# gbordelon/fast_ray_tracer

Measured on AMD Instinct MI355X. Metric: Mrays/s (primary+shadow+secondary) + wall-clock/frame, 1/2/4/8 GPU, higher is better.
Workload: dtype f64

## Files before the change

fast_ray_tracer_amd/csrc/frt_engine.hip:

```cpp
#include <hip/hip_runtime.h>
#include <hipcub/hipcub.hpp>

#include <algorithm>
#include <array>
#include <atomic>
#include <condition_variable>
#include <memory>
#include <mutex>
#include <cmath>
#include <cstdio>
#include <cstdlib>
#include <cstring>
#include <string>
#include <chrono>
#include <functional>
#include <thread>
#include <vector>

#include "frt_device.h"
#include "frt_jit.h"
#include "frt_shade.hpp"
#include "frt_shade32.hpp"
#include "frt_shadow.hpp"
#include "frt_jit_rt.hpp"
// ... 411 lines not shown
            }
        }
    }
    nr.flags = flags;
    PSTAMP(3);
    const bool own = kPat && (M.map_Ka >= 0 || M.map_Kd >= 0 || M.map_Ks >= 0 || M.map_refl >= 0 || M.map_Ns >= 0);
    rec.store(node, nr, own, kPat && M.map_d >= 0);
#pragma unroll
    for (int k = 0; k < 3; ++k) rec.head.op[k * rec.head.cap + node] = c.over_point[k];
    if (rec.head.key != nullptr) rec.head.key[node] = key;
    PSTAMP(4);
    for (int k = 0; k < 3; ++k) op[k] = c.over_point[k];
    };
    if (uniform_ok) {
        const int leaf_u = uniform(hr.node);
        if (__ballot(hr.node != leaf_u) == 0ull) {
            if (B.stats) wave_count(line + 18, (int)(threadIdx.x & 63) == __builtin_ctzll(__ballot(true)));
            prepare_hit(uniform_view(S), leaf_u);
            return true;
        }
    }
    prepare_hit(S, hr.node);
    return true;
}

__device__ __forceinline__ void tile_box(int64_t node, int64_t n, bool hit, const double* op, float* __restrict__ tbox,
                                         int tile_log2, float* __restrict__ stbox, int sub_log2) {
    float lo[3], hi[3];
#pragma unroll
    for (int a = 0; a < 3; ++a) {
        lo[a] = hit ? __double2float_rd(op[a]) : __builtin_huge_valf();
        hi[a] = hit ? __double2float_ru(op[a]) : -__builtin_huge_valf();
    }
    for (int off = 1; off < (1 << tile_log2); off <<= 1) {
        if (stbox != nullptr && off == (1 << sub_log2) && node < n && (node & (off - 1)) == 0) {
            float* b = stbox + 6 * (node >> sub_log2);
#pragma unroll
            for (int a = 0; a < 3; ++a) {
                b[a] = lo[a];
                b[a + 3] = hi[a];
            }
        }
#pragma unroll
        for (int a = 0; a < 3; ++a) {
            lo[a] = fminf(lo[a], __shfl_xor(lo[a], off, 64));
            hi[a] = fmaxf(hi[a], __shfl_xor(hi[a], off, 64));
        }
    }
    if (node < n && (node & ((1 << tile_log2) - 1)) == 0) {
        float* b = tbox + 6 * (node >> tile_log2);
#pragma unroll
        for (int a = 0; a < 3; ++a) {
            b[a] = lo[a];
            b[a + 3] = hi[a];
        }
    }
}

template <bool kPat>
__global__ void __launch_bounds__(kBlock) __attribute__((amdgpu_waves_per_eu(kPat ? 1 : FRT_PREPARE_WAVES, 8)))
k_prepare(DevScene S, Batch B, const QueuedRay* __restrict__ q, int64_t n, const HitRec* __restrict__ hits,
          const double* __restrict__ hn12,
          NodeCols rec, QueuedRay* __restrict__ next_q, unsigned long long* counters,
          unsigned* err, float* __restrict__ tbox, int tile_log2, float* __restrict__ stbox, int sub_log2,
          int32_t* __restrict__ counts, unsigned long long* __restrict__ spawn_masks, int uniform_ok) {
    const int64_t node = (int64_t)blockIdx.x * blockDim.x + threadIdx.x;
    double op[3] = {0.0, 0.0, 0.0};
    bool hit = false;
    if (node < n && counts != nullptr)
        for (int l = 0; l < S.num_lights; ++l) counts[node * S.num_lights + l] = 0;
    int spawned = 0;
    if (node < n)
        hit = prepare_node<kPat>(S, B, q, n, hits, hn12, rec, next_q, counters, err, node, op,
                                 spawn_masks != nullptr ? &spawned : nullptr, uniform_ok);
    if (spawn_masks != nullptr) {
        const unsigned long long mr = __ballot(spawned & 1), mt = __ballot((spawned >> 1) & 1);
        const int64_t g = node >> 6, G = (n + 63) >> 6;
        if ((threadIdx.x & 63) == 0 && g < G) {
            spawn_masks[g] = mr;
            spawn_masks[G + g] = mt;
        }
    }
    if (tbox != nullptr) tile_box(node, n, hit, op, tbox, tile_log2, stbox, sub_log2);
}

#ifdef FRT_SHADOW_WAVES
#define FRT_SHADOW_ATTR __attribute__((amdgpu_waves_per_eu(FRT_SHADOW_WAVES, 8)))
#else
#define FRT_SHADOW_ATTR
#endif
template <int kFeat>
__global__ void __launch_bounds__(kTraceBlock) FRT_SHADOW_ATTR k_shadow(DevScene S, Batch B, const HeadCols shead, int64_t n,
                                                        const int32_t* __restrict__ j_light,
                                                        const int32_t* __restrict__ j_point, int32_t samples_per_node,
                                                        int32_t* __restrict__ counts, unsigned* err) {
    ShadowLane L;
    shadow_lane(S, B, shead, n, j_light, j_point, samples_per_node, (int64_t)blockIdx.x * blockDim.x + threadIdx.x, L);
    unsigned e = 0;
    double unused;
    const bool lit = walk<true, kFeat>(S, L.r, L.distance, L.live, unused, frt_walk_smem, e) == 0 && L.live;
    if (e) atomicOr(err, e);
    shadow_count(S, L, lit, counts);
}

template <int kFeat>
__global__ void __launch_bounds__(kTraceBlock) k_shadow_redo(DevScene S, Batch B, const HeadCols shead, int64_t n,
                                                             const int32_t* __restrict__ j_light,
                                                             const int32_t* __restrict__ j_point, int32_t samples_per_node,
                                                             int32_t* __restrict__ counts, unsigned* err,
                                                             const int64_t* __restrict__ redo,
                                                             const unsigned* __restrict__ redo_count, unsigned redo_cap) {
    const unsigned cnt = min(*redo_count, redo_cap);
    const int64_t wave = ((int64_t)blockIdx.x * blockDim.x + threadIdx.x) >> 6;
    const int64_t nwaves = ((int64_t)gridDim.x * blockDim.x) >> 6;
    unsigned e = 0;
    for (int64_t base = wave * 64; base < (int64_t)cnt; base += nwaves * 64) {
        const int64_t k = base + (threadIdx.x & 63);
        ShadowLane L;
        shadow_lane(S, B, shead, n, j_light, j_point, samples_per_node, k < (int64_t)cnt ? redo[k] : -1, L);
        double unused;
        const bool lit = walk<true, kFeat>(S, L.r, L.distance, L.live, unused, frt_walk_smem, e) == 0 && L.live;
        if (lit) atomicAdd(counts + L.node * S.num_lights + L.light, 1);
    }
    if (e) atomicOr(err, e);
}

#ifndef FRT_SHADE_FACTOR
#define FRT_SHADE_FACTOR 1
#endif
__device__ __forceinline__ double dot3_shade(const double* a, const double* b) {
    return __builtin_fma(a[0], b[0], __builtin_fma(a[1], b[1], a[2] * b[2]));
}
__device__ __forceinline__ void camera_eyev(const DevScene& S, const Batch& B, int64_t i, double* eyev) {
    Ray r;
    uint64_t key;
    unsigned ce = 0;
    camera_ray(S, B, i, r, key, ce);
    for (int k = 0; k < 3; ++k) eyev[k] = r.d[k] * -1.0;
}

__global__ void __launch_bounds__(kBlock) k_view_rays(DevScene S, Batch B, const frt_camera* __restrict__ cams,
                                                      int32_t nviews, int64_t view_pixels, int64_t n,
                                                      QueuedRay* __restrict__ q, unsigned* err) {
    const int64_t i = (int64_t)blockIdx.x * blockDim.x + threadIdx.x;
    if (i >= n) return;
    const int64_t pix = B.pixel_begin + i / B.spp;
    const int view = (int)min((int64_t)(nviews - 1), pix / view_pixels);
    Batch Bv = B;
    Bv.pixel_begin = pix - (int64_t)view * view_pixels - i / B.spp;
    Bv.cam_fast = 0;
    unsigned e = 0;
    auto emit = [&](const frt_camera& cam) {
        DevScene Sv = S;
        Sv.cam = cam;
        Sv.cam_origin_set = 0;
        QueuedRay qr;
        Ray r;
        camera_ray(Sv, Bv, i, r, qr.key, e);
        for (int k = 0; k < 3; ++k) {
            qr.o[k] = r.o[k];
            qr.d[k] = r.d[k];
        }
        qr.parent = -1;
        qr.slot = 0;
        q[i] = qr;
    };
// ... 1364 lines not shown
    if (fgather != nullptr)
        for (int k = 0; k < 3; ++k) a[k] += fgather[3 * i + k];
    for (int k = 0; k < 3; ++k) a[k] += gi_extra[6 * i + 3 + k];
    const double len = a[0] + a[1] + a[2];
    if (len > 1.7320508075688772) {
        for (int k = 0; k < 3; ++k) a[k] *= 1.0 / len;
        for (int k = 0; k < 3; ++k) a[k] *= 1.7320508075688772;
    }
    tri_store(surface, i, a);
}

}


constexpr size_t kJitStatWords = 16384;

template <typename T>
struct PinnedBuf {
    T* p = nullptr;
    size_t n = 0;
    PinnedBuf() = default;
    PinnedBuf(const PinnedBuf&) = delete;
    PinnedBuf& operator=(const PinnedBuf&) = delete;
    ~PinnedBuf() {
        if (p) (void)hipHostFree(p);
    }
    bool resize(size_t m) {
        if (m > n) {
            if (p) (void)hipHostFree(p);
            p = nullptr;
            n = 0;
            if (hipHostMalloc((void**)&p, m * sizeof(T), hipHostMallocDefault) != hipSuccess) {
                p = nullptr;
                return false;
            }
            n = m;
        }
        std::memset(p, 0, n * sizeof(T));
        return true;
    }
    T* data() { return p; }
    const T* data() const { return p; }
    size_t size() const { return n; }
    T& operator[](size_t i) { return p[i]; }
    const T& operator[](size_t i) const { return p[i]; }
};

struct frt_scene_handle {
    int device = 0;
    UploadKnobs up;
    FrameKnobs fk;
    frt::DevScene S{};
    std::vector<void*> owned;
    std::vector<double> host_table;
    hipStream_t stream = nullptr;
    int32_t* j_light = nullptr;
    int32_t* j_point = nullptr;
    int32_t samples_per_node = 0;
    size_t lds_bytes = 0;
    void* jit_shadow = nullptr;
    void* jit_beam = nullptr;
    void* jit_tile = nullptr;
    void* jit_list = nullptr;
    int tile = 0;
    uint64_t scene_key = 0;
    void* jit_sub = nullptr;
    int sub = 0;
    int sub_ps = 0;
    const int32_t* light_psamp2 = nullptr;
    const float* light_sbox = nullptr;
    uint32_t* slist = nullptr;
    int64_t slist_cap = 0;
    uint64_t sub_pairs = 0, sub_mixed = 0;
    void* jit_subtile = nullptr;
    void* jit_trace = nullptr;
    int32_t* tredo = nullptr;
    int64_t tredo_cap = 0;
    int subtile = 0;
    float* stbox = nullptr;
    int64_t stbox_cap = 0;
    uint32_t* s2list = nullptr;
    int64_t s2list_cap = 0;
    uint64_t subtile_pairs = 0, subtile_mixed = 0;
    float* tbox = nullptr;
    int64_t tbox_cap = 0;
    uint32_t* tlist = nullptr;
    int64_t tlist_cap = 0;
    uint64_t tile_pairs = 0, tile_mixed = 0, node_pairs = 0, node_mixed = 0;
    bool jit_beam_on = true;
    const int32_t* light_psamp = nullptr;
    const float* light_aabb = nullptr;
    uint32_t* mixed = nullptr;
    int64_t mixed_cap = 0;
    unsigned* mcount = nullptr;
    uint64_t sync_epoch = 0;
    PinnedBuf<unsigned> host_mcount;
    PinnedBuf<unsigned long long> host_counters;
    PinnedBuf<unsigned> host_lcount;
    int64_t* redo = nullptr;
    unsigned* redo_count = nullptr;
    unsigned redo_cap = 0;
    frt_frame_stats* cur_st = nullptr;
    uint64_t rays_walked = 0;
    uint64_t pairs_walked = 0;
    uint64_t heads_walked = 0;
    unsigned long long uniform_stats[3] = {0, 0, 0};
    uint32_t* shade_lit = nullptr;
    int64_t shade_lit_cap = 0;
    int sort_light = -1;
    int shade_stage = 0;
    uint32_t* lit_row = nullptr;
    int64_t lit_row_cap = 0;
    uint32_t* lit_flat = nullptr;
    int64_t lit_flat_cap = 0;
    frt::LitStage* lit_stage = nullptr;
    int64_t lit_stage_cap = 0;
    bool fast32 = false;
    frt::Light32 light32{nullptr, nullptr};
    uint32_t* qsort = nullptr;
    int64_t qsort_cap = 0;
    unsigned long long* spawn_masks = nullptr;
    int64_t spawn_masks_cap = 0;
    uint32_t* spawn_offs = nullptr;
    int64_t spawn_offs_cap = 0;
    unsigned char* scan_tmp = nullptr;
    int64_t scan_tmp_cap = 0;
    unsigned* shade_lcount = nullptr;
    int64_t shade_lcount_cap = 0;
    unsigned long long* jit_stats = nullptr;
    struct Level {
        frt::NodeCols rec;
        double* head_op = nullptr;
        uint64_t* head_key = nullptr;
        frt::QueuedRay* q = nullptr;
        frt::Cols<frt::Tri9> surface;
        frt::Cols<frt::Tri9> child;
        int64_t* qprefix = nullptr;
        std::vector<int64_t> hprefix = std::vector<int64_t>(frt::kQueueSegs + 1, 0);
        int32_t* counts = nullptr;
        uint32_t* spos = nullptr;
        bool staged = false;
        uint32_t* qperm = nullptr;
        int64_t qperm_cap = 0;
        bool sorted = false;
        int64_t cap = 0;
    };
    std::vector<Level> levels;
    frt::HitRec* hits = nullptr;
    int64_t hits_cap = 0;
    double* hn12 = nullptr;
    int64_t hn12_cap = 0;
    frt::Cols<frt::Tri9> sample_col;
    int64_t sample_cap = 0;
    double* out_dev = nullptr;
    int64_t out_cap = 0;
    double* feat_geom = nullptr;
    int64_t feat_geom_cap = 0;
    int32_t* feat_ids = nullptr;
    int64_t feat_ids_cap = 0;
    frt_camera* view_cams = nullptr;
    int64_t view_cams_cap = 0;
    int32_t strip_views = 0;
    bool cam_origin_ok = false;
    frt::QueuedRay* view_q = nullptr;
    int64_t view_q_cap = 0;
    unsigned long long* counters = nullptr;
// ... 743 lines not shown
    const int kind = (int)(i & 7), pick = (int)((i >> 3) % 7);
    frt::Point64 Q;
    if (kind < 2)
        across(l, eps_list[pick], Q.n);
    else
        unit(Q.n);
    if (kind == 2) {
        across(Q.n, eps_list[pick % 5], Q.e);
    } else {
        unit(Q.e);
        if (kind < 6 && frt::dot3(Q.n, Q.e) < 0.0)
            for (int k = 0; k < 3; ++k) Q.e[k] = -Q.e[k];
    }
    const double ns_list[7] = {0.0, 1.0, 2.5, 10.0, 200.0, 1000.0, 5000.0};
    Q.ns = ns_list[i % 7];
    Q.cdist = (Q.ns + 2) * 0.5 * frt::k1Pi;
    Q.ned = frt::dot3(Q.n, Q.e);
    Q.ee = frt::dot3(Q.e, Q.e);
    for (int k = 0; k < 3; ++k) Q.base[k] = c[k] - o[k];
    const frt::Point32 P = frt::point32_of(Q, __builtin_huge_valf(), true, true);
    frt::ShadeSums s32 = {0.0, 0.0, 0.0}, s64 = {0.0, 0.0, 0.0};
    frt::point_term32(P, Q, off, s32);
    frt::Point64 R = Q;
    for (int k = 0; k < 3; ++k) R.base[k] = lp[k] - o[k];
    const double zero[3] = {0.0, 0.0, 0.0};
    frt::point_term64(R, zero, true, true, s64);
    const bool fin64 = __builtin_isfinite(s64.ldn) && __builtin_isfinite(s64.b) && __builtin_isfinite(s64.fb);
    const bool fin32 = __builtin_isfinite(s32.ldn) && __builtin_isfinite(s32.b) && __builtin_isfinite(s32.fb);
    unsigned long long bad = 0;
    if (fin64 && !fin32) bad++;
    const double dl = fabs(s32.ldn - s64.ldn);
    if (fin64 && fin32 && !(dl <= 32.0 * 0x1p-24)) bad++;
    if (bad) atomicAdd(res, bad);
    auto put_max = [&](int slot, double v) {
        const unsigned long long b = (unsigned long long)__double_as_longlong(v);
        if (b > res[slot]) atomicMax(res + slot, b);
    };
    if (fin64 && fin32) {
        put_max(3, dl);
        if (s64.ldn >= 0x1p-16 && s64.b >= 0x1p-100) {
            const double rel = fabs(s32.b - s64.b) / s64.b;
            put_max(1, rel);
            if (Q.ns <= 200.0) put_max(2, rel);
            atomicAdd(res + 4, 1ull);
        }
    }
}

int64_t frt_shade32_selftest(int64_t n, uint64_t seed, double* out, int nout) {
    n = (std::max<int64_t>(n, 64) + 63) / 64 * 64;
    unsigned long long* res = nullptr;
    unsigned long long h[5] = {0, 0, 0, 0, 0};
    if (hipMalloc((void**)&res, sizeof(h)) != hipSuccess) return -1;
    bool ok = hipMemset(res, 0, sizeof(h)) == hipSuccess;
    if (ok) {
        hipLaunchKernelGGL(k_shade32_selftest, dim3((unsigned)((n + 255) / 256)), dim3(256), 0, 0, n, seed, res);
        ok = hipGetLastError() == hipSuccess && hipMemcpy(h, res, sizeof(h), hipMemcpyDeviceToHost) == hipSuccess;
    }
    hip_ignore(hipFree(res));
    if (!ok) return -1;
    for (int k = 0; k < nout && k < 4 && out != nullptr; ++k) {
        double v;
        std::memcpy(&v, &h[k + 1], sizeof(v));
        out[k] = k == 3 ? (double)h[4] : v;
    }
    return (int64_t)h[0];
}

size_t frt_frame_params_size(void) { return sizeof(frt_frame_params); }

const char* frt_last_error(void) { return g_last_error.c_str(); }

static std::atomic<long long> g_maps_stat[2];

static thread_local double t_upload_phases[8];

int frt_photon_pass_stats(int64_t* out, int n) {
    for (int i = 0; i < n && i < 2; ++i) out[i] = g_maps_stat[i].load();
    return 2;
}

size_t frt_frame_stats_size(void) { return sizeof(frt_frame_stats); }

static std::mutex g_warm_mu;
static hipStream_t g_warm_stream[64] = {};

void* frt_host_pinned_alloc(size_t bytes) {
    void* p = nullptr;
    if (bytes == 0 || hipHostMalloc(&p, bytes, hipHostMallocDefault) != hipSuccess) {
        (void)hipGetLastError();
        return nullptr;
    }
    return p;
}

void frt_host_pinned_free(void* p) {
    if (p) hip_ignore(hipHostFree(p));
}

int frt_device_warmup(int device) {
    const WarmupKnobs K = read_warmup_knobs();
    const bool trace = K.trace;
    auto t0 = std::chrono::steady_clock::now();
    auto mark = [&](const char* what) {
        if (!trace) return;
        const auto t1 = std::chrono::steady_clock::now();
        std::fprintf(stderr, "frt warmup: %s %.2f ms\n", what, std::chrono::duration<double, std::milli>(t1 - t0).count());
        t0 = t1;
    };
    if (hipSetDevice(device) != hipSuccess) {
        (void)hipGetLastError();
        return -1;
    }
    mark("hipSetDevice");
    hip_ignore(hipFree(nullptr));
    mark("context");
    void* p = nullptr;
    if (hipMalloc(&p, 1 << 20) == hipSuccess) {
        mark("hipMalloc");
        hipStream_t s = nullptr;
        if (K.mode == 1 || hipStreamCreate(&s) == hipSuccess) {
            mark("stream");
            unsigned host[64] = {0};
            hip_ignore(hipMemcpyAsync(p, host, sizeof(host), hipMemcpyHostToDevice, s));
            hip_ignore(hipStreamSynchronize(s));
            mark("H2D copy");
            hipLaunchKernelGGL(k_warm, dim3(1), dim3(64), 0, s, (unsigned*)p);
            hip_ignore(hipStreamSynchronize(s));
            mark("first kernel (code object load)");
            hip_ignore(hipMemcpyAsync(host, p, sizeof(host), hipMemcpyDeviceToHost, s));
            hip_ignore(hipStreamSynchronize(s));
            mark("D2H copy");
            if (s) {
                std::lock_guard<std::mutex> lk(g_warm_mu);
                if (device >= 0 && device < 64 && g_warm_stream[device] == nullptr) g_warm_stream[device] = s;
                else hip_ignore(hipStreamDestroy(s));
            }
        }
        hip_ignore(hipFree(p));
    }
    (void)hipGetLastError();
    return 0;
}

int frt_upload_phases(double* out, int n) {
    for (int i = 0; i < n && i < 8; ++i) out[i] = t_upload_phases[i];
    return 8;
}

int frt_scene_upload(const frt_scene* sc, int device, frt_scene_handle** out) {
    const auto up0 = std::chrono::steady_clock::now();
    auto up_last = up0;
    auto phase = [&](int i) {
        const auto t = std::chrono::steady_clock::now();
        t_upload_phases[i] += std::chrono::duration<double, std::milli>(t - up_last).count();
        up_last = t;
    };
    for (double& x : t_upload_phases) x = 0.0;
    if (sc == nullptr || out == nullptr) return fail("frt_scene_upload: null argument");
    if (sc->abi_version != FRT_ABI_VERSION) return fail("frt_scene_upload: ABI version mismatch");
    int ndev = frt_device_count();
    if (ndev <= 0) return fail("frt_scene_upload: no HIP device visible");
    if (device < 0 || device >= ndev) return fail("frt_scene_upload: device index out of range");
    FRT_HIP(hipSetDevice(device));
    frt_scene_handle* h = new frt_scene_handle();
    h->device = device;
// ... 21 lines not shown
        mix(sc->roots, sizeof(int32_t) * (size_t)sc->num_roots);
        mix(sc->xforms, sizeof(double) * 16 * (size_t)sc->num_xforms);
        mix(sc->prim_data, sizeof(double) * (size_t)sc->prim_len);
        mix(sc->materials, sizeof(frt_material) * (size_t)sc->num_materials);
        mix(sc->patterns, sizeof(frt_pattern) * (size_t)sc->num_patterns);
        mix(sc->textures, sizeof(frt_texture) * (size_t)sc->num_textures);
        mix(sc->texels, sizeof(double) * (size_t)sc->texel_len);
        mix(sc->lights, sizeof(frt_light) * (size_t)sc->num_lights);
        mix(sc->light_points, sizeof(double) * (size_t)sc->light_point_len);
        mix(&sc->config, sizeof(frt_config));
        h->scene_key = k;
    }
    phase(0);
    S.nodes = upload(h, sc->nodes, (size_t)sc->num_nodes, rc);
    S.roots = upload(h, sc->roots, (size_t)sc->num_roots, rc);
    S.xforms = upload(h, sc->xforms, (size_t)sc->num_xforms * 16, rc);
    S.prim = upload(h, sc->prim_data, (size_t)sc->prim_len, rc);
    S.materials = upload(h, sc->materials, (size_t)sc->num_materials, rc);
    S.patterns = upload(h, sc->patterns, (size_t)sc->num_patterns, rc);
    S.textures = upload(h, sc->textures, (size_t)sc->num_textures, rc);
    S.texels = upload(h, sc->texels, (size_t)sc->texel_len, rc);
    S.lights = upload(h, sc->lights, (size_t)sc->num_lights, rc);
    S.light_points = upload(h, sc->light_points, (size_t)sc->light_point_len, rc);
    S.sample_table = upload(h, sc->sample_table, (size_t)(2 * sc->camera.usteps * sc->camera.vsteps), rc);
    if (S.sample_table != nullptr)
        h->host_table.assign(sc->sample_table, sc->sample_table + 2 * sc->camera.usteps * sc->camera.vsteps);
    {
        std::vector<uint8_t> casts((size_t)std::max(1, sc->num_nodes), 0);
        for (int i = 0; i < sc->num_nodes; ++i) {
            const int m = sc->nodes[i].material;
            casts[(size_t)i] = (m >= 0 && m < sc->num_materials && sc->materials[m].casts_shadow) ? 1 : 0;
        }
        S.casts = upload(h, casts.data(), casts.size(), rc);
        std::vector<int4> xchain((size_t)std::max(1, sc->num_nodes), make_int4(0, 0, 0, 0));
        for (int i = 0; i < sc->num_nodes; ++i) {
            int ids[64], n = 0;
            for (int x = sc->nodes[i].xform >= 0 ? i : sc->nodes[i].tparent; x >= 0 && n < 64; x = sc->nodes[x].tparent)
                ids[n++] = sc->nodes[x].xform;
            if (n <= 3) xchain[(size_t)i] = make_int4(n, n > 0 ? ids[n - 1] : 0, n > 1 ? ids[n - 2] : 0, n > 2 ? ids[n - 3] : 0);
            else xchain[(size_t)i] = make_int4(-1, 0, 0, 0);
        }
        S.xchain = upload(h, xchain.data(), xchain.size(), rc);
    }
    if (rc) {
        frt_scene_release(h);
        return -1;
    }
    phase(1);
    {
        std::vector<frt::WalkNode> wn;
        build_walk_nodes(sc, wn);
        if (rc == 0 && build_meshes(h, sc, wn)) {
            frt_scene_release(h);
            return -1;
        }
        S.wn = upload(h, wn.data(), wn.size(), rc);
        if (rc == 0 && sc->config.include_direct && K.jit) {
            std::string why, log;
            phase(2);
            const std::string src = frt_jit_shadow_source(wn.data(), sc->num_nodes, sc->roots, sc->num_roots, sc->lights, sc->num_lights, K, why);
            phase(3);
            FrtJitFns fns;
            if (!src.empty() && frt_jit_compile(src, h->device, K, fns, log) != 0) {
                why = "hiprtc: " + log.substr(0, 2000);
                fns = FrtJitFns{};
            }
            if (!src.empty()) {
                double ob = 0.0, ld = 0.0;
                frt_jit_last_phases(&ob, &ld);
                t_upload_phases[4] += ob;
                t_upload_phases[5] += ld;
                up_last = std::chrono::steady_clock::now();
            }
            h->jit_shadow = fns.shadow;
            h->jit_beam = fns.beam;
            h->jit_tile = fns.tile;
            h->jit_list = fns.list;
            h->tile = fns.tile && fns.list ? K.jit_tile : 0;
            h->jit_sub = fns.sub;
            h->sub = fns.sub ? K.jit_sub : 0;
            h->jit_subtile = fns.subtile;
            h->jit_trace = sc->config.all_ni_one ? fns.trace : nullptr;
            h->subtile = fns.subtile ? K.jit_subtile : 0;
            if (h->jit_shadow) {
                h->redo_cap = 1u << 20;
                void* p = nullptr;
                if (hipMalloc(&p, h->redo_cap * sizeof(int64_t) + 64) != hipSuccess) {
                    frt_scene_release(h);
                    return fail("frt_scene_upload: redo queue allocation failed");
                }
                h->owned.push_back(p);
                h->redo = (int64_t*)p;
                h->redo_count = (unsigned*)(h->redo + h->redo_cap);
                h->jit_beam_on = K.jit_beam;
                std::vector<float> box;
                std::vector<int32_t> psamp;
                const int PS = K.jit_part;
                auto push_box = [](std::vector<float>& v, const double* pl, const double* ph) {
                    for (int a = 0; a < 3; ++a) {
                        float f = (float)pl[a];
                        if ((double)f > pl[a]) f = std::nextafter(f, -INFINITY);
                        v.push_back(f);
                    }
                    for (int a = 0; a < 3; ++a) {
                        float f = (float)ph[a];
                        if ((double)f < ph[a]) f = std::nextafter(f, INFINITY);
                        v.push_back(f);
                    }
                };
                auto sample_box = [&](const frt_light& lt, const int32_t* idx, int cnt, int r0, int r1, double* pl, double* ph) {
                    for (int a = 0; a < 3; ++a) {
                        pl[a] = INFINITY;
                        ph[a] = -INFINITY;
                    }
                    for (int r = r0; r < r1; ++r)
                        for (int k = 0; k < cnt; ++k) {
                            const int q = idx[k];
                            if (q < 0) continue;
                            const double* pt = sc->light_points + lt.points + 3 * ((int64_t)r * lt.num_samples + q);
                            for (int a = 0; a < 3; ++a) {
                                pl[a] = std::min(pl[a], pt[a]);
                                ph[a] = std::max(ph[a], pt[a]);
                            }
                        }
                };
                bool multi_row = false;
                std::vector<std::vector<int32_t>> orders((size_t)sc->num_lights);
                for (int l = 0; l < sc->num_lights; ++l) {
                    const frt_light& lt = sc->lights[l];
                    multi_row = multi_row || lt.rows > 1;
                    std::vector<int32_t>& order = orders[(size_t)l];
                    const int np = frt_jit_light_parts(lt, sc->light_points, PS, order);
                    psamp.insert(psamp.end(), order.begin(), order.end());
                    for (int r = 0; r < std::max(1, lt.rows); ++r)
                        for (int p = 0; p < np; ++p) {
                            double pl[3], ph[3];
                            sample_box(lt, order.data() + (size_t)p * PS, PS, r, r + 1, pl, ph);
                            push_box(box, pl, ph);
                        }
                }
                for (int l = 0; multi_row && l < sc->num_lights; ++l) {
                    const frt_light& lt = sc->lights[l];
                    const int np = (int)(orders[(size_t)l].size() / (size_t)PS);
                    for (int p = 0; p < np; ++p) {
                        double pl[3], ph[3];
                        sample_box(lt, orders[(size_t)l].data() + (size_t)p * PS, PS, 0, std::max(1, lt.rows), pl, ph);
                        push_box(box, pl, ph);
                    }
                }
                h->light_psamp = upload(h, psamp.data(), psamp.size(), rc);
                h->light_aabb = upload(h, box.data(), box.size(), rc);
                if (h->sub > 0) {
                    std::vector<int32_t> ps2;
                    std::vector<float> sbox;
                    const int Q = h->sub;
                    for (int l = 0; l < sc->num_lights; ++l) {
                        const frt_light& lt = sc->lights[l];
                        const int np = std::max(1, (lt.num_samples + PS - 1) / PS);
                        std::vector<int32_t> order2;
                        h->sub_ps = frt_jit_light_subparts(lt, sc->light_points, orders[(size_t)l], PS, Q, order2);
                        ps2.insert(ps2.end(), order2.begin(), order2.end());
                        for (int p = 0; p < np * Q; ++p) {
                            double pl[3], ph[3];
                            sample_box(lt, order2.data() + (size_t)p * h->sub_ps, h->sub_ps, 0, std::max(1, lt.rows), pl, ph);
                            push_box(sbox, pl, ph);
                        }
                    }
                    h->light_psamp2 = upload(h, ps2.data(), ps2.size(), rc);
                    h->light_sbox = upload(h, sbox.data(), sbox.size(), rc);
                }
                if (rc || hipMalloc((void**)&h->mcount, 4 * frt::jit::kMixSegs * frt::jit::kMixLine * sizeof(unsigned)) != hipSuccess) {
                    frt_scene_release(h);
                    return fail("frt_scene_upload: light box / pair list allocation failed");
                }
                h->owned.push_back(h->mcount);
                if (!h->host_mcount.resize((size_t)frt::jit::kMixSegs * frt::jit::kMixLine)) {
                    frt_scene_release(h);
                    return fail("frt_scene_upload: pinned host buffer allocation failed");
                }
                if (K.jit_stats) {
                    if (hipMalloc((void**)&h->jit_stats, kJitStatWords * sizeof(unsigned long long)) != hipSuccess) {
                        frt_scene_release(h);
                        return fail("frt_scene_upload: jit stats allocation failed");
                    }
                    h->owned.push_back(h->jit_stats);
                    hip_ignore(hipMemset(h->jit_stats, 0, kJitStatWords * sizeof(unsigned long long)));
                }
            } else if (K.jit_verbose) {
                std::fprintf(stderr, "frt: generic shadow walk (%s)\n", why.c_str());
            }
            if (K.jit_dump && !src.empty()) std::fprintf(stderr, "%s\n", src.c_str());
        }
    }
    {
        static const int kMaxHits[10] = {4, 2, 4, 1, 1, 2, 4, 1, 0, 0};
        const int nn = sc->num_nodes;
        std::vector<int> xf_cnt(nn, 0), comp_cnt(nn, 0), csg_top(nn, -1), list_need(nn, 0);
        int xf_depth = 0, comp_depth = 0, list_cap = 0, features = 0;
        for (int i = 0; i < nn; ++i) {
            const frt_node& nd = sc->nodes[i];
            const int par = nd.parent;
            const bool composite = nd.type == FRT_GROUP || nd.type == FRT_CSG;
            if (nd.type == FRT_CSG) features |= frt::kFeatCsg;
            if (nd.type == FRT_TOROID) features |= frt::kFeatTorus;
            csg_top[i] = par >= 0 && csg_top[par] >= 0 ? csg_top[par] : (nd.type == FRT_CSG ? i : -1);
            xf_cnt[i] = (par >= 0 ? xf_cnt[par] : 0) + (composite && nd.xform >= 0 ? 1 : 0);
            comp_cnt[i] = (par >= 0 && csg_top[par] >= 0 ? comp_cnt[par] : 0) + (composite && csg_top[i] >= 0 ? 1 : 0);
            xf_depth = std::max(xf_depth, xf_cnt[i]);
            comp_depth = std::max(comp_depth, comp_cnt[i]);
            if (!composite && csg_top[i] >= 0 && nd.type >= 0 && nd.type < 10) {
                list_need[csg_top[i]] += kMaxHits[nd.type];
                list_cap = std::max(list_cap, list_need[csg_top[i]]);
            }
        }
        S.list_cap = list_cap;
        S.comp_depth = comp_depth;
        S.xf_depth = xf_depth;
        S.features = features;
        h->lds_bytes = (size_t)frt::walk_lds_bytes(list_cap, comp_depth, xf_depth, S.mesh_stack);
        int lds_max = 64 * 1024;
        if (hipDeviceGetAttribute(&lds_max, hipDeviceAttributeMaxSharedMemoryPerBlock, device) != hipSuccess) {
            (void)hipGetLastError();
            lds_max = 64 * 1024;
        }
        if (h->lds_bytes > (size_t)lds_max) {
            frt_scene_release(h);
            return fail("frt_scene_upload: scene needs " + std::to_string(h->lds_bytes) +
                        " B of LDS per traversal block (CSG lists / nesting too large)");
        }
        if (h->lds_bytes > 64 * 1024) {
            const hipError_t e = walk_lds_opt_in(features, (int)h->lds_bytes);
            if (e != hipSuccess) {
                (void)hipGetLastError();
                frt_scene_release(h);
                return fail("frt_scene_upload: " + std::to_string(h->lds_bytes) +
                            " B of LDS per traversal block refused (" + hipGetErrorString(e) + ")");
            }
        }
    }
    S.walk_flags = K.walk_flags;
    S.num_nodes = sc->num_nodes;
    S.num_roots = sc->num_roots;
    S.num_lights = sc->num_lights;
    S.num_patterns = sc->num_patterns;
    set_scene_camera(h, sc->camera);
    S.cfg = sc->config;
    h->host_lights.assign(sc->lights, sc->lights + sc->num_lights);
    h->sort_light = -1;
    for (int l = 0; l < sc->num_lights && h->sort_light < 0 && K.shade_sort; ++l)
        if (sc->lights[l].rows > 1 && sc->lights[l].num_samples > 0) h->sort_light = l;
    h->shade_stage = h->sort_light >= 0 ? K.shade_stage : 0;
    if (S.cfg.path_length < 0 || S.cfg.path_length > frt::kMaxPathLength) {
        frt_scene_release(h);
        return fail("frt_scene_upload: path-length " + std::to_string(S.cfg.path_length) +
                    " is not supported (0.." + std::to_string(frt::kMaxPathLength) + ")");
    }
    if (S.cfg.use_gi && (S.cfg.gi_path_length >= 255 || S.cfg.photon_count <= 0)) {
        frt_scene_release(h);
        return fail("frt_scene_upload: global illumination needs photon maps (photon_count > 0) and path_length < 255");
    }

    std::vector<int32_t> jl, jp;
    for (int l = 0; l < sc->num_lights; ++l)
        for (int p = 0; p < sc->lights[l].num_samples; ++p) {
            jl.push_back(l);
            jp.push_back(p);
        }
    h->samples_per_node = (int32_t)jl.size();
    if (!jl.empty()) {
        h->j_light = (int32_t*)upload(h, jl.data(), jl.size(), rc);
        h->j_point = (int32_t*)upload(h, jp.data(), jp.size(), rc);
        if (rc) {
            frt_scene_release(h);
            return -1;
        }
    }
#if defined(FRT_WALK_STATS) || defined(FRT_WALK_PROF)
    if (hipMalloc((void**)&h->S.dbg, frt::kDbgSlots * sizeof(unsigned long long)) != hipSuccess ||
        hipMemset(h->S.dbg, 0, frt::kDbgSlots * sizeof(unsigned long long)) != hipSuccess) {
        frt_scene_release(h);
        return fail("frt_scene_upload: debug counters");
    }
#endif
    const auto ts0 = std::chrono::steady_clock::now();
    {
        std::lock_guard<std::mutex> lk(g_warm_mu);
        if (device >= 0 && device < 64 && g_warm_stream[device] != nullptr) {
            h->stream = g_warm_stream[device];
            g_warm_stream[device] = nullptr;
        }
    }
    const bool stream_ok = h->stream != nullptr || hipStreamCreate(&h->stream) == hipSuccess;
    if (K.warmup_trace)
        std::fprintf(stderr, "frt upload: hipStreamCreate %.2f ms\n",
                     std::chrono::duration<double, std::milli>(std::chrono::steady_clock::now() - ts0).count());
    if (!stream_ok || hipMalloc((void**)&h->counters, frt::kQueueSegs * frt::kCounterLine * sizeof(unsigned long long)) != hipSuccess ||
        hipMalloc((void**)&h->err, sizeof(unsigned)) != hipSuccess || hipEventCreate(&h->ev[0]) != hipSuccess ||
        hipEventCreate(&h->ev[1]) != hipSuccess) {
        frt_scene_release(h);
        return fail("frt_scene_upload: stream / counter allocation failed");
    }
    h->levels.resize((size_t)std::max(1, sc->config.path_length + 2));
    *out = h;
    phase(6);
    t_upload_phases[7] = std::chrono::duration<double, std::milli>(std::chrono::steady_clock::now() - up0).count();
    return 0;
}

void frt_scene_release(frt_scene_handle* h) {
    if (!h) return;
    hip_ignore(hipSetDevice(h->device));
    if (h->jit_stats) {
        std::vector<unsigned long long> c(kJitStatWords);
        if (hipMemcpy(c.data(), h->jit_stats, c.size() * sizeof(unsigned long long), hipMemcpyDeviceToHost) == hipSuccess) {
            unsigned long long live = 0, amb = 0, pairs = 0, mixed = 0, tpairs = 0, tmixed = 0, spairs = 0, smixed = 0,
                               upairs = 0, umixed = 0;
            for (int j = 0; j < 64; ++j) {
                live += c[32 * j];
                amb += c[32 * j + 1];
                pairs += c[32 * j + 2];
                mixed += c[32 * j + 3];
                tpairs += c[32 * j + 4];
                tmixed += c[32 * j + 5];
                spairs += c[32 * j + 6];
                smixed += c[32 * j + 7];
                upairs += c[32 * j + 8];
                umixed += c[32 * j + 9];
            }
            if (tpairs)
                std::fprintf(stderr, "frt jit stats: tile pair kernel (%d nodes per tile): live tile pairs %llu, mixed %llu (%.2f%%)\n",
                             h->tile, tpairs, tmixed, 100.0 * (double)tmixed / (double)tpairs);
            std::fprintf(stderr, "frt jit stats: pair kernel: live pairs %llu, mixed %llu (%.2f%%)\n", pairs, mixed,
                         pairs ? 100.0 * (double)mixed / (double)pairs : 0.0);
            if (spairs)
                std::fprintf(stderr, "frt jit stats: sub-part pair kernel (%d sub-parts): live sub-pairs %llu, mixed %llu (%.2f%%)\n",
                             h->sub, spairs, smixed, 100.0 * (double)smixed / (double)spairs);
            if (upairs)
                std::fprintf(stderr, "frt jit stats: sub-tile pair kernel (%d nodes per sub-tile): live sub-tile pairs %llu, mixed %llu (%.2f%%)\n",
                             h->subtile, upairs, umixed, 100.0 * (double)umixed / (double)upairs);
            std::fprintf(stderr, "frt jit stats: live shadow lanes %llu, re-walked in binary64 %llu (%.4f%%)\n", live, amb,
                         live ? 100.0 * (double)amb / (double)live : 0.0);
            std::fprintf(stderr, "frt jit stats: (node, light) pairs: all lit %llu, all shadowed %llu, mixed %llu\n",
                         h->uniform_stats[0], h->uniform_stats[1], h->uniform_stats[2]);
            for (int k = 0; k < std::min(h->S.num_nodes, 512); ++k)
                if (c[2048 + 2 * k])
                    std::fprintf(stderr, "frt jit stats: node %d: %llu waves, %llu lanes tested; composites: %llu waves, %llu lanes entered\n",
                                 k, c[2048 + 2 * k], c[2048 + 2 * k + 1], c[3072 + 2 * k], c[3072 + 2 * k + 1]);
            for (int k = std::max(h->S.num_nodes, 100); k < 2048; ++k)
                if (c[3072 + 2 * k + 1])
                    std::fprintf(stderr, "frt jit stats: beam site %d: %llu waves, %llu lanes\n", k, c[3072 + 2 * k],
                                 c[3072 + 2 * k + 1]);
            for (int k = 0; k < 2048; ++k)
                if (c[9216 + 2 * k + 1])
                    std::fprintf(stderr, "frt jit stats: tile beam site %d: %llu waves, %llu lanes\n", k, c[9216 + 2 * k],
                                 c[9216 + 2 * k + 1]);
        }
    }
    for (void* p : h->owned) hip_ignore(hipFree(p));
    for (auto& L : h->levels) {
        hip_ignore(hipFree(L.rec.core.w));
        hip_ignore(hipFree(L.head_op));
        hip_ignore(hipFree(L.head_key));
        hip_ignore(hipFree(L.q));
        hip_ignore(hipFree(L.surface.w));
        hip_ignore(hipFree(L.child.w));
        hip_ignore(hipFree(L.counts));
        hip_ignore(hipFree(L.spos));
        hip_ignore(hipFree(L.qprefix));
        hip_ignore(hipFree(L.qperm));
    }
    hip_ignore(hipFree(h->hits));
    hip_ignore(hipFree(h->hn12));
    {
        auto& G = h->gi;
        for (int m = 0; m < 2; ++m) {
            hip_ignore(hipFree(G.map_mem[m]));
            hip_ignore(hipFree(G.pq[m]));
            hip_ignore(hipFree(G.ppow[m]));
        }
        hip_ignore(hipFree(G.phits));
        hip_ignore(hipFree(G.pn12));
        hip_ignore(hipFree(G.store));
        hip_ignore(hipFree(G.gq));
        hip_ignore(hipFree(G.ghits));
        hip_ignore(hipFree(G.gcol));
        hip_ignore(hipFree(G.greq));
        hip_ignore(hipFree(G.gwork));
        hip_ignore(hipFree(G.gkeys));
        hip_ignore(hipFree(G.extra));
        hip_ignore(hipFree(G.fgather));
    }
    hip_ignore(hipFree(h->sample_col.w));
    hip_ignore(hipFree(h->out_dev));
    hip_ignore(hipFree(h->feat_geom));
    hip_ignore(hipFree(h->feat_ids));
    hip_ignore(hipFree(h->view_cams));
    hip_ignore(hipFree(h->view_q));
    hip_ignore(hipFree(h->counters));
    hip_ignore(hipFree(h->shade_lit));
    hip_ignore(hipFree(h->shade_lcount));
    hip_ignore(hipFree(h->lit_row));
    hip_ignore(hipFree(h->lit_flat));
    hip_ignore(hipFree(h->qsort));
    hip_ignore(hipFree(h->spawn_masks));
    hip_ignore(hipFree(h->spawn_offs));
    hip_ignore(hipFree(h->lit_stage));
    hip_ignore(hipFree(h->scan_tmp));
    hip_ignore(hipFree(h->mixed));
    hip_ignore(hipFree(h->tlist));
    hip_ignore(hipFree(h->slist));
    hip_ignore(hipFree(h->stbox));
    hip_ignore(hipFree(h->s2list));
    hip_ignore(hipFree(h->tredo));
    hip_ignore(hipFree(h->tbox));
    hip_ignore(hipFree(h->err));
    for (hipEvent_t e : h->ev_pool) hip_ignore(hipEventDestroy(e));
    if (h->ev[0]) hip_ignore(hipEventDestroy(h->ev[0]));
    if (h->ev[1]) hip_ignore(hipEventDestroy(h->ev[1]));
    if (h->stream) hip_ignore(hipStreamDestroy(h->stream));
    delete h;
}

static int32_t level_eye_cam(const frt_scene_handle* h, size_t d) {
    return d == 0 && !h->S.cfg.use_gi && h->fk.eye_cam && h->strip_views == 0 ? 1 : 0;
}

static bool level_keyed(const frt_scene_handle* h, size_t d) {
    bool multi = false;
    for (const auto& L : h->host_lights) multi = multi || L.rows > 1;
    if (!h->fk.head_key0) multi = false;
    return d > 0 || h->S.cfg.use_gi || h->strip_views > 0 || multi;
}

static int set_level_head(frt_scene_handle* h, size_t d) {
    auto& L = h->levels[d];
    if (L.cap <= 0) return 0;
    if (level_keyed(h, d) && L.head_key == nullptr)
        FRT_HIP(hipMalloc((void**)&L.head_key, (size_t)L.cap * sizeof(uint64_t)));
    L.rec.head.op = L.head_op;
    L.rec.head.key = level_keyed(h, d) ? L.head_key : nullptr;
    L.rec.head.mat = L.rec.core.w;
    L.rec.head.cap = L.cap;
    L.rec.head.node0 = 0;
    return 0;
}

static int ensure_level(frt_scene_handle* h, size_t d, int64_t need) {
    auto& L = h->levels[d];
    if (need <= L.cap) return 0;
    int64_t nc = std::max<int64_t>(need, L.cap * 2);
    hip_ignore(hipFree(L.rec.core.w));
    hip_ignore(hipFree(L.head_op));
    hip_ignore(hipFree(L.head_key));
    L.head_op = nullptr;
    L.head_key = nullptr;
    hip_ignore(hipFree(L.q));
    hip_ignore(hipFree(L.surface.w));
    hip_ignore(hipFree(L.child.w));
    hip_ignore(hipFree(L.counts));
    hip_ignore(hipFree(L.spos));
    L.spos = nullptr;
    L.rec = {};
    L.q = nullptr;
    L.surface = {};
    L.child = {};
    L.counts = nullptr;
    {
        void* p = nullptr;
        FRT_HIP(hipMalloc(&p, frt::NodeCols::bytes(nc)));
        L.rec.set((uint64_t*)p, nc);
        L.rec.root = d == 0 ? 1 : 0;
        L.rec.eye_cam = level_eye_cam(h, d);
    }
    FRT_HIP(hipMalloc((void**)&L.head_op, (size_t)nc * 3 * sizeof(double)));
    FRT_HIP(hipMalloc((void**)&L.q, nc * sizeof(frt::QueuedRay)));
    FRT_HIP(hipMalloc((void**)&L.surface.w, frt::Cols<frt::Tri9>::bytes(nc)));
    L.surface.cap = nc;
    FRT_HIP(hipMalloc((void**)&L.child.w, frt::Cols<frt::Tri9>::bytes(2 * nc)));
    L.child.cap = 2 * nc;
    if (!L.qprefix) FRT_HIP(hipMalloc((void**)&L.qprefix, (frt::kQueueSegs + 1) * sizeof(int64_t)));
    FRT_HIP(hipMalloc((void**)&L.counts, nc * std::max(1, h->S.num_lights) * sizeof(int32_t)));
    if (h->shade_stage) FRT_HIP(hipMalloc((void**)&L.spos, nc * sizeof(uint32_t)));
    L.cap = nc;
    return set_level_head(h, d);
}

static inline unsigned grid_for(int64_t n, int block = frt::kBlock) { return (unsigned)((n + block - 1) / block); }

static hipError_t stream_sync(frt_scene_handle* h) {
    const hipError_t e = hipStreamSynchronize(h->stream);
    if (e == hipSuccess) h->sync_epoch++;
    return e;
}

static bool shade_lazy(const frt_scene_handle* h) {
    return h->fk.shade_split && !h->S.cfg.use_gi && h->fk.shade_lazy;
}
// ... 74 lines not shown
                case 0: launch_trace_redo_f<0>(h, B, q, n, hits); break;
                case 1: launch_trace_redo_f<1>(h, B, q, n, hits); break;
                case 2: launch_trace_redo_f<2>(h, B, q, n, hits); break;
                default: launch_trace_redo_f<3>(h, B, q, n, hits); break;
                }
                if (h->fk.jit_trace_stats) {
                    unsigned c = 0;
                    hip_ignore(hipMemcpyAsync(&c, cnt, sizeof(c), hipMemcpyDeviceToHost, h->stream));
                    hip_ignore(hipStreamSynchronize(h->stream));
                    std::fprintf(stderr, "frt: frt_jit_trace level %d: %lld rays, %u to the generic walk\n", B.level,
                                 (long long)n, c);
                    const std::string& dump = h->fk.jit_trace_dump;
                    if (!dump.empty() && B.level == 0 && c > 0) {
                        std::vector<int32_t> v(std::min<size_t>(c, cap));
                        hip_ignore(hipMemcpy(v.data(), h->tredo, v.size() * sizeof(int32_t), hipMemcpyDeviceToHost));
                        if (FILE* f = std::fopen(dump.c_str(), "wb")) {
                            std::fwrite(v.data(), sizeof(int32_t), v.size(), f);
                            std::fclose(f);
                        }
                    }
                }
                return;
            }
            std::fprintf(stderr, "frt: scene-specialised closest-hit kernel launch failed; k_trace\n");
            (void)hipGetLastError();
            h->jit_trace = nullptr;
        } else {
            (void)hipGetLastError();
        }
    }
    switch (h->S.features & 3) {
    case 0: launch_trace_f<0>(h, B, q, n, hits, filter_casts, hn12); break;
    case 1: launch_trace_f<1>(h, B, q, n, hits, filter_casts, hn12); break;
    case 2: launch_trace_f<2>(h, B, q, n, hits, filter_casts, hn12); break;
    default: launch_trace_f<3>(h, B, q, n, hits, filter_casts, hn12); break;
    }
}

template <int F>
static void launch_shadow_f(frt_scene_handle* h, const frt::Batch& B, const frt::HeadCols& rec, int64_t n, int32_t* counts) {
    const int64_t work = n * h->samples_per_node;
    hipLaunchKernelGGL(frt::k_shadow<F>, dim3(grid_for(work, frt::kTraceBlock)), dim3(frt::kTraceBlock), h->lds_bytes,
                       h->stream, h->S, B, rec, n, h->j_light, h->j_point, h->samples_per_node, counts, h->err);
}

template <int F>
static void launch_shadow_redo_f(frt_scene_handle* h, const frt::Batch& B, const frt::HeadCols& rec, int64_t n,
                                 int32_t* counts) {
    hipLaunchKernelGGL(frt::k_shadow_redo<F>, dim3(64), dim3(frt::kTraceBlock), h->lds_bytes, h->stream, h->S, B, rec, n,
                       h->j_light, h->j_point, h->samples_per_node, counts, h->err, h->redo, h->redo_count, h->redo_cap);
}

static uint64_t seg_table(const PinnedBuf<unsigned>& host_mcount, uint32_t segcap, uint64_t lpe,
                          frt::jit::SegTable& seg, uint64_t& total) {
    uint64_t nblk = 0;
    total = 0;
    for (int j = 0; j < frt::jit::kMixSegs; ++j) {
        const uint64_t c = std::min<uint64_t>(host_mcount[(size_t)j * frt::jit::kMixLine], segcap);
        seg.bstart[j] = (uint32_t)nblk;
        seg.count[j] = (uint32_t)c;
        total += c;
        nblk += (c * lpe + frt::kTraceBlock - 1) / frt::kTraceBlock;
    }
    seg.bstart[frt::jit::kMixSegs] = (uint32_t)nblk;
    return nblk;
}

static void launch_shadow(frt_scene_handle* h, const frt::Batch& B, const frt::HeadCols& rec, int64_t n, int32_t* counts,
                          int64_t node0 = 0) {
    if (h->jit_shadow) {
        using frt::jit::kMixLine;
        using frt::jit::kMixSegs;
        const int PS = h->up.jit_part;
        int64_t NP = 0;
        for (const auto& L : h->host_lights) NP += std::max(1, (L.num_samples + PS - 1) / PS);
        const int64_t mp = h->fk.jit_max_pairs;
        int64_t kMaxPairs = mp ? mp : (int64_t)((1ll << 31) - 1);
        const bool beam_on = h->jit_beam_on && n * NP >= h->fk.jit_min_pairs;
        const bool tiled = beam_on && h->tile > 0 && h->jit_tile && h->jit_list && h->tbox;
        const bool subbed = tiled && h->jit_sub && h->sub > 0 && h->light_psamp2 && h->light_sbox;
        if (subbed && h->up.jit_node_beam) {
            kMaxPairs = std::min<int64_t>(kMaxPairs, (int64_t)(0xFFFFFFFFull / (uint64_t)h->sub));
        } else if (subbed) {
            int stl = 0;
            while (h->subtile > 0 && (1 << stl) < h->tile / h->subtile) ++stl;
            const uint64_t per_tile = ((uint64_t)NP * (uint64_t)h->sub) << stl;
            const int64_t tiled_max = (int64_t)(0xFFFFFFFFull / per_tile) * h->tile * NP;
            kMaxPairs = std::min<int64_t>(std::min<int64_t>(tiled_max, (int64_t)0xFFFFFFFFll),
                                          mp ? mp : INT64_MAX);
        }
        if (n * NP > kMaxPairs) {
            int64_t per = std::max<int64_t>(1, kMaxPairs / NP);
            if (h->tile > 0) per = std::max<int64_t>(h->tile, per / h->tile * h->tile);
            for (int64_t off = 0; off < n; off += per)
                launch_shadow(h, B, rec.at(off), std::min(per, n - off), counts + off * h->S.num_lights, node0 + off);
            return;
        }
        const int64_t npairs = n * NP;
        uint32_t nn = (uint32_t)n;
        uint32_t segcap = 0;
        unsigned* mc_tile = h->mcount;
        unsigned* mc_sub = h->mcount + kMixSegs * kMixLine;
        unsigned* mc_subtile = h->mcount + 2 * kMixSegs * kMixLine;
        unsigned* mc_node = h->mcount + 3 * kMixSegs * kMixLine;
        if (beam_on) hip_ignore(hipMemsetAsync(h->mcount, 0, 4 * kMixSegs * kMixLine * sizeof(unsigned), h->stream));
        uint64_t total_mixed = 0;
        const uint32_t* direct_in = nullptr;
        uint32_t direct_subq = 0, direct_nodes = 0;
        if (beam_on) {
            frt::jit::SegTable tseg{};
            uint32_t tsegcap = 0;
            uint64_t list_blocks = 0, listed = 0;
            const uint32_t* list_in = h->tlist;
            uint32_t list_segcap = 0;
            const float* list_boxes = h->light_aabb;
            int tl = 0;
            while ((1 << tl) < h->tile) ++tl;
            if (tiled) {
                const int64_t ntiles = (n + h->tile - 1) >> tl;
                uint32_t ntp = (uint32_t)(ntiles * NP);
                const int64_t tblocks = (ntiles * NP + frt::kTraceBlock - 1) / frt::kTraceBlock;
                tsegcap = (uint32_t)std::max<int64_t>(frt::kTraceBlock, ((tblocks + kMixSegs - 1) / kMixSegs) * frt::kTraceBlock);
                if (grow(&h->tlist, h->tlist_cap, 2 * (int64_t)tsegcap * kMixSegs)) {
                    (void)hipGetLastError();
                    h->jit_shadow = nullptr;
                    launch_shadow(h, B, rec, n, counts, node0);
                    return;
                }
                const float* tb = h->tbox + 6 * (node0 >> tl);
                const uint32_t* no_list = nullptr;
                uint32_t zero = 0;
                void* targs[] = {&h->S, (void*)&B, (void*)&rec, &ntp, &nn, (void*)&tb, (void*)&no_list, &tseg, &zero, &zero,
                                 &h->light_aabb, &counts, &h->tlist, &mc_tile, &tsegcap, &h->err, &h->jit_stats,
                                 &h->light_psamp2};
                hipError_t le;
                {
                    KTimer tt(h, h->cur_st, 12);
                    le = hipModuleLaunchKernel((hipFunction_t)h->jit_tile, grid_for(ntiles * NP, frt::kTraceBlock), 1, 1,
                                               frt::kTraceBlock, 1, 1, 0, h->stream, targs, nullptr);
                }
                if (le != hipSuccess) {
                    std::fprintf(stderr, "frt: scene-specialised tile kernel launch failed (%s); pairs per node\n",
                                 hipGetErrorString(le));
                    (void)hipGetLastError();
                    h->tile = 0;
                    launch_shadow(h, B, rec, n, counts, node0);
                    return;
                }
                if (hipMemcpyAsync(h->host_mcount.data(), mc_tile, h->host_mcount.size() * sizeof(unsigned),
                                   hipMemcpyDeviceToHost, h->stream) != hipSuccess ||
                    stream_sync(h) != hipSuccess)
                    return;
                list_blocks = seg_table(h->host_mcount, tsegcap, subbed ? (uint64_t)h->sub : (uint64_t)h->tile, tseg, listed);
                h->tile_pairs += ntp;
                h->tile_mixed += listed;
                list_in = h->tlist;
                list_segcap = tsegcap;
                if (subbed && listed > 0) {
                    const uint64_t sblocks = list_blocks;
                    const frt::jit::SegTable sseg = tseg;
                    const uint32_t ssegcap = (uint32_t)std::max<uint64_t>(frt::kTraceBlock,
                                                                          ((sblocks + kMixSegs - 1) / kMixSegs) * frt::kTraceBlock);
                    if (grow(&h->slist, h->slist_cap, 2 * (int64_t)ssegcap * kMixSegs)) {
                        (void)hipGetLastError();
                        h->jit_shadow = nullptr;
                        hip_ignore(hipMemsetAsync(counts, 0, (size_t)n * h->S.num_lights * sizeof(int32_t), h->stream));
                        launch_shadow(h, B, rec, n, counts, node0);
                        return;
                    }
                    hipError_t se = hipSuccess;
                    {
                        KTimer ts(h, h->cur_st, 13);
                        const uint64_t max_blocks = ((1ull << 31) - 1) / frt::kTraceBlock;
                        uint32_t zero = 0;
                        for (uint64_t b0 = 0; b0 < sblocks && se == hipSuccess; b0 += max_blocks) {
                            uint32_t b0u = (uint32_t)b0;
                            void* sargs[] = {&h->S, (void*)&B, (void*)&rec, &zero, &nn, (void*)&tb, &h->tlist, (void*)&sseg, &b0u,
                                             &tsegcap, &h->light_sbox, &counts, &h->slist, &mc_sub, (void*)&ssegcap, &h->err,
                                             &h->jit_stats, &h->light_psamp2};
                            se = hipModuleLaunchKernel((hipFunction_t)h->jit_sub, (unsigned)std::min(max_blocks, sblocks - b0), 1, 1,
                                                       frt::kTraceBlock, 1, 1, 0, h->stream, sargs, nullptr);
                        }
                    }
                    if (se != hipSuccess) {
                        std::fprintf(stderr, "frt: scene-specialised sub-part kernel launch failed (%s); no sub-parts\n",
                                     hipGetErrorString(se));
                        (void)hipGetLastError();
                        h->jit_sub = nullptr;
                        h->sub = 0;
                        hip_ignore(hipMemsetAsync(counts, 0, (size_t)n * h->S.num_lights * sizeof(int32_t), h->stream));
                        launch_shadow(h, B, rec, n, counts, node0);
                        return;
                    }
                    if (hipMemcpyAsync(h->host_mcount.data(), mc_sub, h->host_mcount.size() * sizeof(unsigned),
                                       hipMemcpyDeviceToHost, h->stream) != hipSuccess ||
                        stream_sync(h) != hipSuccess)
                        return;
                    uint64_t listed_s = 0;
                    const bool subtiled = h->jit_subtile && h->subtile > 0 && h->subtile < h->tile && h->stbox &&
                                          (B.level == 0 || h->fk.jit_subtile_deep);
                    const uint64_t nst = subtiled ? (uint64_t)(h->tile / h->subtile) : 0;
                    list_blocks = seg_table(h->host_mcount, ssegcap, subtiled ? nst : (uint64_t)h->tile, tseg, listed_s);
                    h->sub_pairs += listed * (uint64_t)h->sub;
                    h->sub_mixed += listed_s;
                    listed = listed_s;
                    list_in = h->slist;
                    list_segcap = ssegcap;
                    list_boxes = h->light_sbox;
                    if (subtiled && listed_s > 0) {
                        const uint64_t tblocks = list_blocks;
                        const frt::jit::SegTable s1seg = tseg;
                        const uint32_t s2segcap = (uint32_t)std::max<uint64_t>(
                            frt::kTraceBlock, ((tblocks + kMixSegs - 1) / kMixSegs) * frt::kTraceBlock);
                        if (grow(&h->s2list, h->s2list_cap, 2 * (int64_t)s2segcap * kMixSegs)) {
                            (void)hipGetLastError();
                            h->jit_shadow = nullptr;
                            hip_ignore(hipMemsetAsync(counts, 0, (size_t)n * h->S.num_lights * sizeof(int32_t), h->stream));
                            launch_shadow(h, B, rec, n, counts, node0);
                            return;
                        }
                        int stl = 0;
                        while ((1 << stl) < h->subtile) ++stl;
                        const float* stb = h->stbox + 6 * (node0 >> stl);
                        hipError_t ue = hipSuccess;
                        {
                            KTimer tu(h, h->cur_st, 14);
                            const uint64_t max_blocks = ((1ull << 31) - 1) / frt::kTraceBlock;
                            uint32_t zero = 0;
                            for (uint64_t b0 = 0; b0 < tblocks && ue == hipSuccess; b0 += max_blocks) {
                                uint32_t b0u = (uint32_t)b0;
                                void* uargs[] = {&h->S, (void*)&B, (void*)&rec, &zero, &nn, (void*)&stb, &h->slist, (void*)&s1seg,
                                                 &b0u, (void*)&ssegcap, &h->light_sbox, &counts, &h->s2list, &mc_subtile,
                                                 (void*)&s2segcap, &h->err, &h->jit_stats, &h->light_psamp2};
                                ue = hipModuleLaunchKernel((hipFunction_t)h->jit_subtile, (unsigned)std::min(max_blocks, tblocks - b0),
                                                           1, 1, frt::kTraceBlock, 1, 1, 0, h->stream, uargs, nullptr);
                            }
                        }
                        if (ue != hipSuccess) {
                            std::fprintf(stderr, "frt: scene-specialised sub-tile kernel launch failed (%s); no sub-tiles\n",
                                         hipGetErrorString(ue));
                            (void)hipGetLastError();
                            h->jit_subtile = nullptr;
                            h->subtile = 0;
                            hip_ignore(hipMemsetAsync(counts, 0, (size_t)n * h->S.num_lights * sizeof(int32_t), h->stream));
                            launch_shadow(h, B, rec, n, counts, node0);
                            return;
                        }
                        if (hipMemcpyAsync(h->host_mcount.data(), mc_subtile, h->host_mcount.size() * sizeof(unsigned),
                                           hipMemcpyDeviceToHost, h->stream) != hipSuccess ||
                            stream_sync(h) != hipSuccess)
                            return;
                        uint64_t listed_u = 0;
                        list_blocks = seg_table(h->host_mcount, s2segcap, (uint64_t)h->subtile, tseg, listed_u);
                        h->subtile_pairs += listed_s * nst;
                        h->subtile_mixed += listed_u;
                        listed = listed_u;
                        list_in = h->s2list;
                        list_segcap = s2segcap;
                    } else if (subtiled) {
                        list_blocks = 0;
                        listed = 0;
                    }
                } else if (subbed) {
                    list_blocks = 0;
                    listed = 0;
                }
            }
            if (subbed && !h->up.jit_node_beam && list_in != h->tlist) {
                direct_in = list_in;
                direct_subq = list_in == h->s2list ? 3u : 2u;
                direct_nodes = (uint32_t)(list_in == h->s2list ? h->subtile : h->tile);
                segcap = list_segcap;
                for (int j = 0; j < kMixSegs; ++j) total_mixed += std::min<uint64_t>(h->host_mcount[(size_t)j * kMixLine], segcap);
                h->node_pairs += total_mixed * direct_nodes;
                h->node_mixed += total_mixed * direct_nodes;
            } else {
            const int64_t pblocks = tiled ? (int64_t)list_blocks : (npairs + frt::kTraceBlock - 1) / frt::kTraceBlock;
            segcap = (uint32_t)std::max<int64_t>(frt::kTraceBlock, ((pblocks + kMixSegs - 1) / kMixSegs) * frt::kTraceBlock);
            uint32_t** nout = &h->mixed;
            int64_t& nout_cap = h->mixed_cap;
            if (grow(nout, nout_cap, 2 * (int64_t)segcap * kMixSegs)) {
                (void)hipGetLastError();
                h->jit_shadow = nullptr;
                hip_ignore(hipMemsetAsync(counts, 0, (size_t)n * h->S.num_lights * sizeof(int32_t), h->stream));
                launch_shadow(h, B, rec, n, counts, node0);
                return;
            }
            hipError_t le = hipSuccess;
            {
                KTimer tb(h, h->cur_st, 8);
                if (tiled) {
                    const uint64_t max_blocks = ((1ull << 31) - 1) / frt::kTraceBlock;
                    const float* no_box = nullptr;
                    uint32_t zero = 0;
                    for (uint64_t b0 = 0; b0 < list_blocks && le == hipSuccess; b0 += max_blocks) {
                        uint32_t b0u = (uint32_t)b0;
                        void* largs[] = {&h->S, (void*)&B, (void*)&rec, &zero, &nn, (void*)&no_box, (void*)&list_in, &tseg, &b0u,
                                         &list_segcap, (void*)&list_boxes, &counts, nout, &mc_node, &segcap, &h->err,
                                         &h->jit_stats, &h->light_psamp2};
                        le = hipModuleLaunchKernel((hipFunction_t)h->jit_list, (unsigned)std::min(max_blocks, list_blocks - b0), 1, 1,
                                                   frt::kTraceBlock, 1, 1, 0, h->stream, largs, nullptr);
                    }
                    h->node_pairs += listed * (uint64_t)(list_in == h->s2list ? h->subtile : h->tile);
                } else {
                    uint32_t np = (uint32_t)npairs;
                    const float* no_box = nullptr;
                    const uint32_t* no_list = nullptr;
                    frt::jit::SegTable no_seg{};
                    uint32_t zero = 0;
                    void* bargs[] = {&h->S, (void*)&B, (void*)&rec, &np, &nn, (void*)&no_box, (void*)&no_list, &no_seg, &zero, &zero,
                                     &h->light_aabb, &counts, nout, &mc_node, &segcap, &h->err, &h->jit_stats,
                                     &h->light_psamp2};
                    le = hipModuleLaunchKernel((hipFunction_t)h->jit_beam, grid_for(npairs, frt::kTraceBlock), 1, 1,
                                               frt::kTraceBlock, 1, 1, 0, h->stream, bargs, nullptr);
                    h->node_pairs += (uint64_t)npairs;
                }
            }
            if (le != hipSuccess) {
                std::fprintf(stderr, "frt: scene-specialised pair kernel launch failed (%s); every pair per ray\n",
                             hipGetErrorString(le));
                (void)hipGetLastError();
                h->jit_beam_on = false;
                hip_ignore(hipMemsetAsync(counts, 0, (size_t)n * h->S.num_lights * sizeof(int32_t), h->stream));
                launch_shadow(h, B, rec, n, counts, node0);
                return;
            }
            if (hipMemcpyAsync(h->host_mcount.data(), mc_node, h->host_mcount.size() * sizeof(unsigned),
                               hipMemcpyDeviceToHost, h->stream) != hipSuccess ||
                stream_sync(h) != hipSuccess)
                return;
            for (int j = 0; j < kMixSegs; ++j) total_mixed += std::min<uint64_t>(h->host_mcount[(size_t)j * kMixLine], segcap);
            h->node_mixed += total_mixed;
            }
        } else {
            segcap = (uint32_t)std::max<int64_t>(1, npairs);
            if (grow(&h->mixed, h->mixed_cap, 2 * (int64_t)segcap * kMixSegs)) {
                (void)hipGetLastError();
                h->jit_shadow = nullptr;
                launch_shadow(h, B, rec, n, counts, node0);
                return;
            }
            total_mixed = (uint64_t)npairs;
        }
        uint32_t all_pairs = beam_on ? 0u : 1u;
        uint32_t subq = direct_in ? direct_subq : subbed ? 1u : 0u;
        uint32_t lpp = direct_in ? direct_nodes * (uint32_t)h->sub_ps : subbed ? (uint32_t)h->sub_ps : (uint32_t)PS;
        const uint32_t* mixed_in = direct_in ? direct_in : h->mixed;
        uint32_t shift = 32;
        while ((1u << (shift - 32)) < lpp) ++shift;
        const uint64_t magic = (uint64_t)((((unsigned __int128)1 << shift) + lpp - 1) / lpp);
        uint32_t spn = (uint32_t)h->samples_per_node;
        const uint64_t max_pairs = std::max<uint64_t>(1, ((1ull << 31) - 1) / lpp);
        hip_ignore(hipMemsetAsync(h->redo_count, 0, sizeof(unsigned), h->stream));
        h->rays_walked += total_mixed * lpp;
        h->pairs_walked += total_mixed;
        h->heads_walked += std::min<uint64_t>(direct_in ? total_mixed * direct_nodes : total_mixed, (uint64_t)n);
        KTimer tr(h, h->cur_st, 9);
        frt::jit::SegTable seg{};
        uint64_t nblk = 0;
        for (int j = 0; j < kMixSegs; ++j) {
            const uint64_t c = all_pairs ? 0 : std::min<uint64_t>(h->host_mcount[(size_t)j * kMixLine], segcap);
            seg.bstart[j] = (uint32_t)nblk;
            seg.count[j] = (uint32_t)c;
            nblk += (c * lpp + frt::kTraceBlock - 1) / frt::kTraceBlock;
        }
        seg.bstart[kMixSegs] = (uint32_t)nblk;
        const uint64_t max_blocks = ((1ull << 31) - 1) / frt::kTraceBlock;
        const uint64_t launches = all_pairs ? (total_mixed + max_pairs - 1) / max_pairs : (nblk + max_blocks - 1) / max_blocks;
        for (uint64_t li = 0; li < launches; ++li) {
            uint32_t total = 0, m0 = 0, b0 = 0;
            uint64_t grid = 0;
            if (all_pairs) {
                const uint64_t p0 = li * max_pairs, pc = std::min<uint64_t>(max_pairs, total_mixed - p0);
                total = (uint32_t)(pc * lpp);
                m0 = (uint32_t)p0;
                grid = (total + frt::kTraceBlock - 1) / frt::kTraceBlock;
            } else {
                b0 = (uint32_t)(li * max_blocks);
                grid = std::min<uint64_t>(max_blocks, nblk - b0);
            }
            void* args[] = {&h->S, (void*)&B, (void*)&rec, &total, &m0, (void*)&mixed_in, &seg, &b0, &segcap, &all_pairs,
                            &h->light_psamp, &subq, &h->light_psamp2, &lpp, (void*)&magic,
                            &shift, &spn, &counts, &h->redo, &h->redo_count, &h->redo_cap, &h->err, &h->jit_stats, &nn};
            const hipError_t le = hipModuleLaunchKernel((hipFunction_t)h->jit_shadow, (unsigned)grid,
                                                        1, 1, frt::kTraceBlock, 1, 1, 0, h->stream, args, nullptr);
            if (le != hipSuccess) {
                std::fprintf(stderr, "frt: scene-specialised shadow kernel launch failed (%s); generic walk\n",
                             hipGetErrorString(le));
                (void)hipGetLastError();
                hip_ignore(hipMemsetAsync(counts, 0, (size_t)n * h->S.num_lights * sizeof(int32_t), h->stream));
                h->jit_shadow = nullptr;
                launch_shadow(h, B, rec, n, counts);
                return;
            }
        }
// ... 588 lines not shown
            if (v[0]) std::fprintf(stderr, " %d:%llu/%llu", i, v[0], v[1]);
        }
        std::fprintf(stderr, "\n");
    }
    std::fprintf(stderr, "walk prof (shadow, cycles):");
    const char* pn[8] = {"setup", "close", "xf_pop", "composite", "leaf_xf", "leaf_test", "leaf_post", "loop"};
    for (int k = 0; k < 8; ++k) std::fprintf(stderr, " %s=%llu", pn[k], c[frt::kDbgProf + k]);
    std::fprintf(stderr, "\nestimate prof (cycles): scan=%llu select=%llu sum=%llu band=%llu; queries over k=%llu "
                 "unlisted=%llu slow_band=%llu order_check=%llu in_range_total=%llu order_check_cycles=%llu",
                 c[frt::kDbgProf + 13], c[frt::kDbgProf + 14], c[frt::kDbgProf + 15], c[frt::kDbgProf + 16],
                 c[frt::kDbgProf + 17], c[frt::kDbgProf + 18], c[frt::kDbgProf + 19], c[frt::kDbgProf + 20],
                 c[frt::kDbgProf + 21], c[frt::kDbgProf + 22]);
    std::fprintf(stderr, " reduce_tried=%llu reduce_fallback=%llu queries=%llu candidates_read=%llu records_read=%llu",
                 c[frt::kDbgProf + 23], c[frt::kDbgProf + 24], c[frt::kDbgProf + 25], c[frt::kDbgProf + 27],
                 c[frt::kDbgProf + 28]);
    std::fprintf(stderr, "\nprepare prof (cycles):");
    const char* qn[5] = {"ray", "hits_load", "prepare", "spawn", "stores"};
    for (int k = 0; k < 5; ++k) std::fprintf(stderr, " %s=%llu", qn[k], c[frt::kDbgProf + 8 + k]);
    std::fprintf(stderr, "\n");
}
#endif

static int render_frame(frt_scene_handle* h, const frt_frame_params* P, double* dev_out, frt_frame_stats* st);

static int frame_precision(frt_scene_handle* h, const frt_frame_params* P) {
    int p = P->precision;
    if (p == FRT_PRECISION_DEFAULT) {
        const std::string& e = h->fk.precision;
        if (e.empty() || e == "parity")
            p = FRT_PRECISION_PARITY;
        else if (e == "fast32")
            p = FRT_PRECISION_FAST32;
        else
            return fail(std::string("FRT_PRECISION=") + e + " is not supported (parity or fast32)");
    }
    if (p != FRT_PRECISION_PARITY && p != FRT_PRECISION_FAST32)
        return fail("precision " + std::to_string(P->precision) + " is not supported");
    if (p == FRT_PRECISION_FAST32 && !h->fk.shade_split)
        return fail("precision fast32 is not supported with FRT_SHADE_SPLIT=0 (the unsplit k_shade is binary64 only)");
    h->fast32 = p == FRT_PRECISION_FAST32;
    return 0;
}

static int ensure_light32(frt_scene_handle* h) {
    if (h->light32.off != nullptr || h->S.num_lights == 0) return 0;
    int64_t len = 0;
    for (const frt_light& L : h->host_lights)
        len = std::max<int64_t>(len, L.points + 3 * (int64_t)L.num_samples * std::max(1, L.rows));
    if (len == 0 || h->S.light_points == nullptr) return 0;
    std::vector<double> pts((size_t)len);
    FRT_HIP(hipMemcpy(pts.data(), h->S.light_points, (size_t)len * sizeof(double), hipMemcpyDeviceToHost));
    std::vector<float> off((size_t)len + 4, 0.0f);
    std::vector<double> cent((size_t)h->S.num_lights * 3, 0.0);
    for (size_t l = 0; l < h->host_lights.size(); ++l) {
        const frt_light& L = h->host_lights[l];
        const int64_t np = (int64_t)L.num_samples * std::max(1, L.rows);
        if (np <= 0) continue;
        const double* p = pts.data() + L.points;
        double c[3] = {0.0, 0.0, 0.0};
        for (int64_t q = 0; q < np; ++q)
            for (int k = 0; k < 3; ++k) c[k] += p[3 * q + k];
        for (int k = 0; k < 3; ++k) cent[3 * l + (size_t)k] = c[k] /= (double)np;
        for (int64_t q = 0; q < np; ++q)
            for (int k = 0; k < 3; ++k) off[(size_t)(L.points + 3 * q + k)] = (float)(p[3 * q + k] - c[k]);
    }
    int rc = 0;
    const float* doff = upload(h, off.data(), off.size(), rc);
    const double* dcent = upload(h, cent.data(), cent.size(), rc);
    if (rc) return rc;
    h->light32.cent = dcent;
    h->light32.off = doff;
    return 0;
}

static int render_impl(frt_scene_handle* h, const frt_frame_params* P, double* dev_out, frt_frame_stats* st) {
    h->fk = read_frame_knobs();
    frame_camera_consts(h);
    h->cur_st = st;
    h->rays_walked = 0;
    h->pairs_walked = 0;
    h->heads_walked = 0;
    h->tile_pairs = h->tile_mixed = h->node_pairs = h->node_mixed = h->sub_pairs = h->sub_mixed = 0;
    h->subtile_pairs = h->subtile_mixed = 0;
    const int rc = render_frame(h, P, dev_out, st);
    if (rc) h->gi.built = false;
    return rc;
}

static int render_strip(frt_scene_handle* h, const frt_camera* cams, int32_t nviews, const frt_frame_params* P,
                        double* dev_out, frt_frame_stats* st) {
    FRT_HIP(hipSetDevice(h->device));
    if (grow(&h->view_cams, h->view_cams_cap, nviews)) return -1;
    FRT_HIP(hipMemcpy(h->view_cams, cams, (size_t)nviews * sizeof(frt_camera), hipMemcpyHostToDevice));
    const frt_camera own = h->S.cam;
    h->S.cam = cams[0];
    h->strip_views = nviews;
    const int rc = render_impl(h, P, dev_out, st);
    h->strip_views = 0;
    h->S.cam = own;
    if (!h->levels.empty()) h->levels[0].rec.eye_cam = level_eye_cam(h, 0);
    return rc;
}

static int shade_level(frt_scene_handle* h, const frt::Batch& B, int d, int64_t n, frt_frame_stats* st);
static int64_t close_level(frt_scene_handle* h, const frt::Batch& B, int d, int64_t n, bool dense, frt_frame_stats* st);
static void frame_stats(frt_scene_handle* h, frt_frame_stats* st, unsigned err);

static int render_frame(frt_scene_handle* h, const frt_frame_params* P, double* dev_out, frt_frame_stats* st) {
    using namespace frt;
    FRT_HIP(hipSetDevice(h->device));
    if (frame_precision(h, P)) return -1;
    if (h->fast32 && ensure_light32(h)) return -1;
    const int64_t hs = h->S.cam.hsize;
    const int64_t stride = P->row_stride > 0 ? P->row_stride : 1;
    int64_t nrows = 0;
    for (int64_t r = P->row_begin; r < P->row_end; r += stride) nrows++;
    const int32_t nviews = h->strip_views;
    const int64_t npix = nrows * hs * std::max(1, nviews);
    if (!h->levels.empty()) h->levels[0].rec.eye_cam = level_eye_cam(h, 0);
    if (!h->levels.empty() && set_level_head(h, 0)) return -1;
    const int32_t spp = (int32_t)(h->S.cam.usteps * h->S.cam.vsteps);
    if (spp <= 0) return fail("render: usteps*vsteps must be positive");
    int64_t batch = P->batch_samples > 0 ? P->batch_samples : h->fk.batch_samples;
    int64_t pix_per_batch = std::max<int64_t>(1, batch / spp);
    const int path = h->S.cfg.path_length;
    if (st) {
        std::memset(st, 0, sizeof(*st));
        (void)hipEventRecord(h->ev[0], h->stream);
    }
    FRT_HIP(hipMemsetAsync(h->err, 0, sizeof(unsigned), h->stream));
    FRT_HIP(hipMemsetAsync(h->counters, 0, frt::kQueueSegs * frt::kCounterLine * sizeof(unsigned long long), h->stream));
    if (h->S.cfg.use_gi && (!h->gi.built || h->gi.seed != P->seed)) {
        hipEvent_t p0 = nullptr, p1 = nullptr;
        if (st) {
            hip_ignore(hipEventCreate(&p0));
            hip_ignore(hipEventCreate(&p1));
            hip_ignore(hipEventRecord(p0, h->stream));
        }
        const int rc = build_photon_maps(h, P->seed);
        if (st) {
            hip_ignore(hipEventRecord(p1, h->stream));
            hip_ignore(hipEventSynchronize(p1));
            float ms = 0.f;
            hip_ignore(hipEventElapsedTime(&ms, p0, p1));
            st->photon_ms = ms;
            st->photon_pass = 1;
            hip_ignore(hipEventDestroy(p0));
            hip_ignore(hipEventDestroy(p1));
        }
        if (rc) return rc;
    }
    if (st) {
        st->photons[0] = h->gi.photons[0];
        st->photons[1] = h->gi.photons[1];
    }
    if (!h->host_counters.resize((size_t)kQueueSegs * kCounterLine) ||
        !h->host_lcount.resize((size_t)kShadeSegs * jit::kMixLine))
        return fail("render: pinned host buffer allocation failed");
    auto& host_counters = h->host_counters;
    for (int64_t p0 = 0; p0 < npix; p0 += pix_per_batch) {
        const int64_t bp = std::min<int64_t>(pix_per_batch, npix - p0);
        const int64_t ns = bp * spp;
        if (ns > h->sample_cap) {
            hip_ignore(hipFree(h->sample_col.w));
            h->sample_col = {};
            h->sample_cap = 0;
            FRT_HIP(hipMalloc((void**)&h->sample_col.w, frt::Cols<frt::Tri9>::bytes(ns)));
            h->sample_col.cap = h->sample_cap = ns;
        }
        if (ensure_level(h, 0, ns)) return -1;
        if (nviews > 0 && grow(&h->view_q, h->view_q_cap, ns)) return -1;
        Batch B{};
        B.sample_begin = 0;
        const int64_t first_row = P->row_begin + ((p0 / hs) % std::max<int64_t>(1, nrows)) * stride;
        B.sample_begin = (first_row * hs + p0 % hs) * spp;
        B.pixel_begin = p0;
        B.num_samples = ns;
        B.row_begin = P->row_begin;
        B.row_stride = stride;
        B.seed = P->seed;
        B.spp = spp;
        B.stats = st != nullptr ? 1 : 0;
        batch_camera_index(h, B, bp);
        std::vector<int64_t> count(path + 2, 0);
        count[0] = ns;
        FRT_HIP(hipMemset2DAsync(h->counters, kCounterLine * sizeof(unsigned long long), 0, 16 * sizeof(unsigned long long),
                                 kQueueSegs, h->stream));
        for (int d = 0; d <= path; ++d) {
            const int64_t n = count[d];
            if (n == 0) break;
            B.level = d;
            B.remaining = path - d;
            auto& L = h->levels[d];
            if (ensure_level(h, d + 1, 2 * n + (int64_t)kQueueSegs * 2 * kBlock)) return -1;
            auto& N = h->levels[d + 1];
            B.qprefix = d > 0 ? L.qprefix : nullptr;
            B.qperm = d > 0 && L.sorted ? L.qperm : nullptr;
            B.qsegcap = L.cap / kQueueSegs;
            B.next_segcap = N.cap / kQueueSegs;
            if (h->S.num_lights < 1)
                FRT_HIP(hipMemsetAsync(L.counts, 0, (size_t)n * sizeof(int32_t), h->stream));
            if (grow(&h->hits, h->hits_cap, n)) return -1;
            if (!h->S.cfg.all_ni_one && grow(&h->hn12, h->hn12_cap, 2 * n)) return -1;
            double* hn12 = h->S.cfg.all_ni_one ? nullptr : h->hn12;
            const QueuedRay* q = d == 0 ? (nviews > 0 ? h->view_q : nullptr) : L.q;
            bool dense = false;
            {
                KTimer t(h, st, d == 0 ? 5 : 0);
                if (d == 0 && nviews > 0) {
                    hipLaunchKernelGGL(k_view_rays, dim3(grid_for(n)), dim3(kBlock), 0, h->stream, h->S, B,
                                       (const frt_camera*)h->view_cams, nviews, nrows * hs, n, h->view_q, h->err);
                    FRT_HIP(hipGetLastError());
                }
                launch_trace(h, B, q, n, h->hits, 0, hn12, true);
                FRT_HIP(hipGetLastError());
            }
            {
                KTimer t(h, st, 6);
                const bool tiles = h->tile > 0 && h->jit_shadow && h->jit_beam_on && h->S.cfg.include_direct &&
                                   h->samples_per_node > 0;
                int tl = 0;
                while (tiles && (1 << tl) < h->tile) ++tl;
                if (tiles && grow(&h->tbox, h->tbox_cap, 6 * ((n >> tl) + 1))) return -1;
                const bool subtiles = tiles && h->subtile > 0 && h->subtile < h->tile;
                int stl = 0;
                while (subtiles && (1 << stl) < h->subtile) ++stl;
                if (subtiles && grow(&h->stbox, h->stbox_cap, 6 * ((n >> stl) + 1))) return -1;
                dense = h->up.queue_sort == 2 && d < path && 2 * n <= (int64_t)UINT32_MAX && N.cap >= 2 * n;
                const int64_t G = (n + 63) >> 6;
                if (dense && (grow(&h->spawn_masks, h->spawn_masks_cap, 2 * G) ||
                              grow(&h->spawn_offs, h->spawn_offs_cap, 2 * G + 1) || grow(&N.qperm, N.qperm_cap, 2 * n)))
                    return -1;
                hipLaunchKernelGGL(h->S.num_patterns > 0 ? k_prepare<true> : k_prepare<false>, dim3(grid_for(n)),
                                   dim3(kBlock), 0, h->stream, h->S, B, q, n, h->hits, hn12,
                                   L.rec, N.q, h->counters, h->err, tiles ? h->tbox : nullptr, tl,
                                   subtiles ? h->stbox : nullptr, stl, L.counts, dense ? h->spawn_masks : nullptr,
                                   h->up.prepare_uniform ? 1 : 0);
                FRT_HIP(hipGetLastError());
                if (dense) {
                    hipcub::CountingInputIterator<int64_t> idx(0);
                    hipcub::TransformInputIterator<uint32_t, MaskPopc, hipcub::CountingInputIterator<int64_t>> popc(
                        idx, MaskPopc{h->spawn_masks, 2 * G});
                    size_t tmp_bytes = 0;
                    FRT_HIP(hipcub::DeviceScan::ExclusiveSum(nullptr, tmp_bytes, popc, h->spawn_offs, (int)(2 * G + 1),
                                                             h->stream));
                    if (grow(&h->scan_tmp, h->scan_tmp_cap, (int64_t)tmp_bytes + 16)) return -1;
                    FRT_HIP(hipcub::DeviceScan::ExclusiveSum((void*)h->scan_tmp, tmp_bytes, popc, h->spawn_offs,
                                                             (int)(2 * G + 1), h->stream));
                    hipLaunchKernelGGL(k_spawn_expand, dim3(grid_for(2 * G)), dim3(kBlock), 0, h->stream, h->spawn_masks,
                                       h->spawn_offs, n, G, N.qperm, h->counters);
                    FRT_HIP(hipGetLastError());
                }
            }
            FRT_HIP(hipMemcpyAsync(host_counters.data(), h->counters, host_counters.size() * sizeof(unsigned long long),
                                   hipMemcpyDeviceToHost, h->stream));
            const uint64_t counters_epoch = h->sync_epoch;
            if (h->S.cfg.include_direct && h->samples_per_node > 0) {
                KTimer t(h, st, 1);
                launch_shadow(h, B, L.rec.head, n, L.counts);
                FRT_HIP(hipGetLastError());
            }
            if (h->jit_stats && h->S.num_lights > 0) {
                std::vector<int32_t> hc((size_t)n * h->S.num_lights);
                std::vector<uint64_t> hh((size_t)n);
                FRT_HIP(hipMemcpyAsync(hc.data(), L.counts, hc.size() * sizeof(int32_t), hipMemcpyDeviceToHost, h->stream));
                FRT_HIP(hipMemcpyAsync(hh.data(), L.rec.core.w, hh.size() * sizeof(uint64_t), hipMemcpyDeviceToHost, h->stream));
                FRT_HIP(hipStreamSynchronize(h->stream));
                for (int64_t i = 0; i < n; ++i) {
                    if ((int32_t)(uint32_t)hh[(size_t)i] < 0) continue;
                    for (int l = 0; l < h->S.num_lights; ++l) {
                        const int32_t c = hc[(size_t)(i * h->S.num_lights + l)];
                        h->uniform_stats[c == 0 ? 1 : (c == h->host_lights[(size_t)l].num_samples ? 0 : 2)]++;
                    }
                }
            }
            if (shade_level(h, B, d, n, st)) return -1;
            if (h->S.cfg.use_gi) {
                KTimer t(h, st, 7);
                if (shade_gi(h, B, L, n, st)) return -1;
            }
            if (h->sync_epoch == counters_epoch) FRT_HIP(stream_sync(h));
            const int64_t next = close_level(h, B, d, n, dense, st);
            if (next < 0) return -1;
            count[d + 1] = next;
        }
        const bool fuse = spp <= kFuseBlock && h->fk.fuse_resolve;
        const bool lazy = shade_lazy(h);
        for (int d = path; d >= 0; --d) {
            const int64_t n = count[d];
            if (n == 0) continue;
            if (d == 0 && fuse) {
                KTimer t(h, st, 4);
                const int32_t ppb = kFuseBlock / spp;
                hipLaunchKernelGGL(k_combine_resolve, dim3((unsigned)((bp + ppb - 1) / ppb)), dim3(kFuseBlock), 0, h->stream,
                                   h->S, lazy ? h->levels[0].counts : nullptr, h->levels[0].rec, n, h->levels[0].surface, h->levels[0].child, spp, ppb, bp,
                                   h->S.materials, h->S.cfg.include_specular, dev_out + 4 * p0,
                                   h->levels[0].staged ? (const uint32_t*)h->levels[0].spos : nullptr);
                FRT_HIP(hipGetLastError());
                continue;
            }
            KTimer t(h, st, 3);
            const Cols<Tri9> parent_child = d > 0 ? h->levels[d - 1].child : Cols<Tri9>{};
            hipLaunchKernelGGL(k_combine, dim3(grid_for(n)), dim3(kBlock), 0, h->stream, h->S,
                               lazy ? h->levels[d].counts : nullptr, h->levels[d].rec, n,
                               h->levels[d].surface, h->levels[d].child, parent_child, h->sample_col, spp,
                               h->S.materials, h->S.cfg.include_specular,
                               h->levels[d].staged ? (const uint32_t*)h->levels[d].spos : nullptr);
            FRT_HIP(hipGetLastError());
        }
        if (!fuse) {
            KTimer t(h, st, 4);
            hipLaunchKernelGGL(k_resolve, dim3((unsigned)((bp + 63) / 64)), dim3(kResolveBlock), 0, h->stream, h->sample_col, bp, spp,
                               dev_out + 4 * p0);
            FRT_HIP(hipGetLastError());
        }
    }
    FRT_HIP(hipMemcpyAsync(host_counters.data(), h->counters, host_counters.size() * sizeof(unsigned long long),
                           hipMemcpyDeviceToHost, h->stream));
    unsigned err = 0;
    FRT_HIP(hipMemcpyAsync(&err, h->err, sizeof(unsigned), hipMemcpyDeviceToHost, h->stream));
    if (st) (void)hipEventRecord(h->ev[1], h->stream);
// ... 107 lines not shown
    for (int j = 0; j < kQueueSegs && !dense; ++j) {
        N.hprefix[j] = next;
        int64_t c = (int64_t)host_counters[(size_t)j * kCounterLine + d + 1];
        if (c > B.next_segcap) {
            overflow = true;
            c = B.next_segcap;
        }
        next += c;
    }
    if (dense) next = (int64_t)host_counters[20];
    N.hprefix[kQueueSegs] = next;
    if (overflow) {
        unsigned e = kErrQueueOverflow;
        FRT_HIP(hipMemcpyAsync(h->err, &e, sizeof(unsigned), hipMemcpyHostToDevice, h->stream));
    }
    if (next > 0 && d < path && !dense)
        FRT_HIP(hipMemcpyAsync(N.qprefix, N.hprefix.data(), (kQueueSegs + 1) * sizeof(int64_t), hipMemcpyHostToDevice,
                               h->stream));
    int pbits = 1;
    while (pbits < 32 && (1ll << pbits) < n) ++pbits;
    N.sorted = dense || (h->up.queue_sort == 1 && d < path && next >= 4096 && !overflow && pbits < 32 &&
                         N.cap <= (int64_t)UINT32_MAX);
    if (N.sorted && !dense) {
        KTimer t(h, st, 6);
        if (grow(&h->qsort, h->qsort_cap, 3 * next) || grow(&N.qperm, N.qperm_cap, next)) return -1;
        uint32_t *keys = h->qsort, *keys2 = h->qsort + next, *slots = h->qsort + 2 * next;
        Batch Bn = B;
        Bn.qprefix = N.qprefix;
        Bn.qsegcap = N.cap / kQueueSegs;
        Bn.qperm = nullptr;
        const int shift = std::min(h->up.queue_sort_shift, pbits - 1);
        hipLaunchKernelGGL(k_queue_keys, dim3(grid_for(next)), dim3(kBlock), 0, h->stream, Bn, N.q, next, pbits,
                           shift, keys, slots);
        FRT_HIP(hipGetLastError());
        size_t tmp_bytes = 0;
        FRT_HIP(hipcub::DeviceRadixSort::SortPairs(nullptr, tmp_bytes, keys, keys2, slots, N.qperm, (int)next, 0,
                                                   pbits - shift + 1, h->stream));
        if (grow(&h->scan_tmp, h->scan_tmp_cap, (int64_t)tmp_bytes + 16)) return -1;
        FRT_HIP(hipcub::DeviceRadixSort::SortPairs((void*)h->scan_tmp, tmp_bytes, keys, keys2, slots, N.qperm,
                                                   (int)next, 0, pbits - shift + 1, h->stream));
    }
    if (st) {
        if (d > 0) st->secondary_rays += (uint64_t)n;
        else st->primary_rays += (uint64_t)n;
    }
    return d < path ? next : 0;
}

static void frame_stats(frt_scene_handle* h, frt_frame_stats* st, unsigned err) {
    using namespace frt;
    const auto& host_counters = h->host_counters;
    float ms = 0.f;
    (void)hipEventElapsedTime(&ms, h->ev[0], h->ev[1]);
    st->render_ms = ms;
    uint64_t pruned = 0, hits = 0, uniform_waves = 0;
    for (int j = 0; j < kQueueSegs; ++j) {
        pruned += host_counters[(size_t)j * kCounterLine + 16];
        hits += host_counters[(size_t)j * kCounterLine + 17];
        uniform_waves += host_counters[(size_t)j * kCounterLine + 18];
    }
    st->prepare_uniform_waves = uniform_waves;
    st->pruned_secondary = pruned;
    st->hits = hits;
    st->shadow_rays = h->S.cfg.include_direct ? hits * (uint64_t)h->samples_per_node : 0;
    bool multi = false;
    for (const auto& L : h->host_lights) multi = multi || L.rows > 1;
    const double kHead = multi ? 40.0 : 32.0;
    st->shadow_kernel_bytes = !(h->S.cfg.include_direct && h->samples_per_node > 0) ? 0.0
                              : h->jit_shadow != nullptr ? (double)h->pairs_walked * 8.0 + (double)h->heads_walked * (kHead + 4.0) +
                                                               (multi ? 24.0 * (double)h->rays_walked : 0.0)
                                                         : (double)hits * (kHead + 4.0 * h->S.num_lights);
    st->errors = err;
    st->shadow_jit = h->jit_shadow != nullptr ? 1 : 0;
    st->shadow_rays_walked = h->jit_shadow != nullptr ? h->rays_walked : st->shadow_rays;
    st->shadow_tile_pairs = h->tile_pairs;
    st->shadow_tile_mixed = h->tile_mixed;
    st->shadow_pairs = h->node_pairs;
    st->shadow_pairs_mixed = h->node_mixed;
    st->shadow_sub_pairs = h->sub_pairs;
    st->shadow_sub_mixed = h->sub_mixed;
    st->shadow_subtile_pairs = h->subtile_pairs;
    st->shadow_subtile_mixed = h->subtile_mixed;
    collect_timings(h, st);
}

static int feature_frame(frt_scene_handle* h, const frt_frame_params* P, const frt_feature_buffers* dev,
                         frt_frame_stats* st) {
    using namespace frt;
    FRT_HIP(hipSetDevice(h->device));
    const int64_t hs = h->S.cam.hsize;
    const int64_t stride = P->row_stride > 0 ? P->row_stride : 1;
    int64_t nrows = 0;
    for (int64_t r = P->row_begin; r < P->row_end; r += stride) nrows++;
    const int32_t nviews = h->strip_views;
    const int64_t npix = nrows * hs * std::max(1, nviews);
    if (!h->levels.empty()) h->levels[0].rec.eye_cam = level_eye_cam(h, 0);
    if (!h->levels.empty() && set_level_head(h, 0)) return -1;
    const int32_t spp = (int32_t)(h->S.cam.usteps * h->S.cam.vsteps);
    if (spp <= 0) return fail("render: usteps*vsteps must be positive");
    if (h->levels.size() < 2) return fail("render: the handle has no level state");
    const int64_t batch = P->batch_samples > 0 ? P->batch_samples : h->fk.batch_samples;
    const int64_t pix_per_batch = std::max<int64_t>(1, batch / spp);
    if (st) {
        std::memset(st, 0, sizeof(*st));
        (void)hipEventRecord(h->ev[0], h->stream);
    }
    FRT_HIP(hipMemsetAsync(h->err, 0, sizeof(unsigned), h->stream));
    FRT_HIP(hipMemsetAsync(h->counters, 0, frt::kQueueSegs * frt::kCounterLine * sizeof(unsigned long long), h->stream));
    for (int64_t p0 = 0; p0 < npix; p0 += pix_per_batch) {
        const int64_t bp = std::min<int64_t>(pix_per_batch, npix - p0);
        const int64_t ns = bp * spp;
        if (ensure_level(h, 0, ns)) return -1;
        if (nviews > 0 && grow(&h->view_q, h->view_q_cap, ns)) return -1;
        Batch B{};
        const int64_t first_row = P->row_begin + ((p0 / hs) % std::max<int64_t>(1, nrows)) * stride;
        B.sample_begin = (first_row * hs + p0 % hs) * spp;
        B.pixel_begin = p0;
        B.num_samples = ns;
        B.row_begin = P->row_begin;
        B.row_stride = stride;
        B.seed = P->seed;
        B.spp = spp;
        B.stats = st != nullptr ? 1 : 0;
        batch_camera_index(h, B, bp);
        B.level = 0;
        B.remaining = 0;
        if (ensure_level(h, 1, (int64_t)kQueueSegs * 2 * kBlock)) return -1;
        auto& L = h->levels[0];
        auto& N = h->levels[1];
        B.qprefix = nullptr;
        B.qperm = nullptr;
        B.qsegcap = L.cap / kQueueSegs;
        B.next_segcap = N.cap / kQueueSegs;
        if (grow(&h->hits, h->hits_cap, ns)) return -1;
        if (!h->S.cfg.all_ni_one && grow(&h->hn12, h->hn12_cap, 2 * ns)) return -1;
        double* hn12 = h->S.cfg.all_ni_one ? nullptr : h->hn12;
        const QueuedRay* q = nviews > 0 ? h->view_q : nullptr;
        {
            KTimer t(h, st, 5);
            if (nviews > 0) {
                hipLaunchKernelGGL(k_view_rays, dim3(grid_for(ns)), dim3(kBlock), 0, h->stream, h->S, B,
                                   (const frt_camera*)h->view_cams, nviews, nrows * hs, ns, h->view_q, h->err);
                FRT_HIP(hipGetLastError());
            }
            launch_trace(h, B, q, ns, h->hits, 0, hn12, true);
            FRT_HIP(hipGetLastError());
        }
        {
            KTimer t(h, st, 6);
            hipLaunchKernelGGL(h->S.num_patterns > 0 ? k_prepare<true> : k_prepare<false>, dim3(grid_for(ns)),
                               dim3(kBlock), 0, h->stream, h->S, B, q, ns, h->hits, hn12, L.rec, N.q, h->counters,
                               h->err, (float*)nullptr, 0, (float*)nullptr, 0, (int32_t*)nullptr,
                               (unsigned long long*)nullptr, h->up.prepare_uniform ? 1 : 0);
            FRT_HIP(hipGetLastError());
        }
        {
            KTimer t(h, st, 8 + 10);
            const int32_t ppb = spp <= kFeatBlock ? kFeatBlock / spp : 1;
            hipLaunchKernelGGL(k_feature_resolve, dim3((unsigned)((bp + ppb - 1) / ppb)), dim3(kFeatBlock), 0,
                               h->stream, L.rec, (const HitRec*)h->hits, ns, spp, ppb, bp, h->S.materials,
                               dev->geom ? dev->geom + 8 * p0 : nullptr, dev->ids ? dev->ids + 2 * p0 : nullptr);
            FRT_HIP(hipGetLastError());
        }
    }
    unsigned err = 0;
    FRT_HIP(hipMemcpyAsync(&err, h->err, sizeof(unsigned), hipMemcpyDeviceToHost, h->stream));
// ... 260 lines not shown
```

fast_ray_tracer_amd/csrc/frt_jit.h:

```cpp
#pragma once

#include <stdint.h>

#include <string>
#include <vector>

#include "frt_knobs.hpp"

namespace frt {
struct WalkNode;
}
struct frt_light;

std::vector<int> frt_jit_sub_sizes(int c, int Q);
int frt_jit_sub_ps(int PS, int Q);
int frt_jit_light_subparts(const frt_light& L, const double* light_points, const std::vector<int32_t>& order, int PS,
                           int Q, std::vector<int32_t>& order2);
int frt_jit_light_parts(const frt_light& L, const double* light_points, int PS, std::vector<int32_t>& order);

std::string frt_jit_shadow_source(const frt::WalkNode* wn, int num_nodes, const int32_t* roots, int num_roots,
                                  const frt_light* lights, int num_lights, const UploadKnobs& K, std::string& why);

struct FrtJitFns {
    void* shadow = nullptr;
    void* beam = nullptr;
    void* tile = nullptr;
    void* list = nullptr;
    void* sub = nullptr;
    void* subtile = nullptr;
    void* trace = nullptr;
};
int frt_jit_compile(const std::string& src, int device, const UploadKnobs& K, FrtJitFns& fns, std::string& log);

void frt_jit_last_phases(double* obtain_ms, double* load_ms);

int frt_jit_compile_only(const std::string& src, const std::string& arch, const UploadKnobs& K, std::string& log);
```

fast_ray_tracer_amd/csrc/frt_jit.hip:

```cpp
#include <hip/hip_runtime.h>
#include <hip/hiprtc.h>

#include <unistd.h>
#include <sys/stat.h>

#include <atomic>
#include <chrono>
#include <cmath>
#include <condition_variable>
#include <cstdio>
#include <cstdlib>
#include <cstring>
#include <functional>
#include <map>
#include <memory>
#include <mutex>
#include <set>
#include <thread>
#include <sstream>
#include <string>
#include <vector>

#include "frt_device.h"
#include "frt_jit.h"
// ... 1084 lines not shown

static void walk32(Gen& g, const int32_t* roots, int num_roots) {
    std::ostringstream& o = g.o;
    for (int ri = 0; ri < num_roots; ++ri) {
        o << "        // ---- world shape " << ri << " (node " << roots[ri] << ")\n";
        o << "        if (__ballot(alive)) {\n";
        if (g.gate_start)
            o << "            bool any_entry = START_ANY && START >= " << roots[ri] << "u && START < " << g.wn[roots[ri]].skip
              << "u;\n";
        else
            o << "            bool any_entry = false;\n";
        g.slots.clear();
        g.top32(roots[ri], "true", "", ri == num_roots - 1, "            ");
        if (g.beam)
            o << "            if (ms && result != 1) {\n                amb = true;\n                alive = false;\n            }\n";
        o << "            if (alive && any_entry) alive = false;  // the first world shape with entries ends the walk\n";
        o << "        }\n";
    }
}

std::string frt_jit_shadow_source(const frt::WalkNode* wn, int num_nodes, const int32_t* roots, int num_roots,
                                  const frt_light* lights, int num_lights, const UploadKnobs& K, std::string& why) {
    if (num_nodes > kMaxNodes) {
        why = "scene has more than " + std::to_string(kMaxNodes) + " nodes";
        return "";
    }
    if (num_lights < 1 || num_lights > kMaxLights) {
        why = "scene has " + std::to_string(num_lights) + " lights (the scene-specialised kernel takes 1.." +
              std::to_string(kMaxLights) + ")";
        return "";
    }
    Gen g;
    g.wn = wn;
    g.nn = num_nodes;
    g.stats = K.jit_stats;
    g.inside_opt = K.jit_inside;
    g.u32 = K.jit_u32 != 0;
    for (int ri = 0; ri < num_roots; ++ri)
        if (!g.check(roots[ri])) {
            why = g.why;
            return "";
        }
    LightTabs T;
    T.lights = lights;
    T.n = num_lights;
    T.start.assign((size_t)num_lights + 1, 0);
    T.rowbase.assign((size_t)num_lights + 1, 0);
    for (int l = 0; l < num_lights; ++l) {
        T.start[(size_t)l + 1] = T.start[(size_t)l] + lights[l].num_samples;
        T.rowbase[(size_t)l + 1] = T.rowbase[(size_t)l] + std::max(1, lights[l].rows);
        T.multi_row = T.multi_row || lights[l].rows > 1;
    }
    T.parts.assign((size_t)num_lights, 0);
    T.partbase.assign((size_t)num_lights + 1, 0);
    T.boxbase.assign((size_t)num_lights + 1, 0);
    for (int l = 0; l < num_lights; ++l) {
        T.parts[(size_t)l] = std::max<int64_t>(1, (lights[l].num_samples + K.jit_part - 1) / K.jit_part);
        T.partbase[(size_t)l + 1] = T.partbase[(size_t)l] + T.parts[(size_t)l];
        T.boxbase[(size_t)l + 1] = T.boxbase[(size_t)l] + T.parts[(size_t)l] * std::max(1, lights[l].rows);
    }
    T.np = T.partbase[(size_t)num_lights];
    const std::string NP = std::to_string(T.np) + "u";
    const std::string NL = std::to_string(num_lights) + "u";
    std::ostringstream& o = g.o;
    header(o);

    const int TS = K.jit_tile;
    int TSL = 0;
    while ((1 << TSL) < TS) ++TSL;
    const bool resume = K.jit_resume;
    if (resume && K.jit_flags) g.assign_flags();
    const bool stats_on = g.stats;
    const int u32_mode = K.jit_u32;
    const int order_mode = K.jit_order;
    const int SQ = TS > 0 ? K.jit_sub : 0;
    int SQL = 0;
    while ((1 << SQL) < SQ) ++SQL;
    const bool st_on = !T.multi_row || K.jit_subtile_set;
    const int ST = SQ > 0 && st_on && K.jit_subtile < TS ? K.jit_subtile : 0;
    const int NST = ST ? TS / ST : 0;
    int STL = 0, NSTL = 0;
    while (ST && (1 << STL) < ST) ++STL;
    while (NST && (1 << NSTL) < NST) ++NSTL;
    const int PS = K.jit_part;
    const int PS2 = SQ ? frt_jit_sub_ps(PS, SQ) : 0;
    const int NM = K.jit_node_major ? K.jit_node_major : T.multi_row ? 4 : 1;
    std::string subn;
    for (int l = 0; SQ && l < num_lights; ++l)
        for (int64_t p = 0; p < T.parts[(size_t)l]; ++p) {
            const int c = p + 1 < T.parts[(size_t)l] ? PS : lights[l].num_samples - (int)p * PS;
            for (int x : frt_jit_sub_sizes(std::max(c, 0), SQ)) subn += (subn.empty() ? "" : ", ") + std::to_string(x);
        }
    auto pair_kernel = [&](int mode) {
        const char* name = mode == 0 ? "frt_jit_beam" : mode == 1 ? "frt_jit_tile" : mode == 2 ? "frt_jit_beam_list"
                         : mode == 3 ? "frt_jit_sub" : "frt_jit_subtile";
        const bool boxed = mode == 1 || mode == 3 || mode == 4;
        o << "extern \"C\" __global__ void __launch_bounds__(kTraceBlock)" << waves_attr(K.jit_beam_waves) << "\n"
          << name << "(DevScene S, Batch B, const HeadCols shead, uint32_t nlanes, uint32_t nnodes,\n"
             "             const float* __restrict__ tbox, const uint32_t* __restrict__ tlist, jit::SegTable seg,\n"
             "             uint32_t b0, uint32_t tsegcap,\n"
             "             const float* __restrict__ laabb, int32_t* __restrict__ counts, uint32_t* __restrict__ mixed,\n"
             "             unsigned* __restrict__ mcount, uint32_t segcap, unsigned* __restrict__ err,\n"
             "             unsigned long long* __restrict__ jstats, const int32_t* __restrict__ psamp2) {\n"
             "    const uint32_t tid = blockIdx.x * blockDim.x + threadIdx.x;\n";
        for (int k = 0; k < num_nodes; ++k) g.node32(k, "    ");
        o << "    uint32_t node = 0, gp = 0, pp = 0, tile = 0;\n"
             "    bool live = false;\n"
             "    uint32_t START = 0, FLAGS = 0;  // (frt_jit_beam_list: the tile's resume point and flags)\n"
             "    bool START_ANY = false;\n"
          << (boxed ? "    jit::BeamBox32 W;\n" : "    jit::Beam32 W;\n");
        if (mode == 0) {
            o << "    bool in = tid < nlanes;\n"
                 "    if (in) {\n"
                 "        node = tid / " << NP << ";\n"
                 "        gp = tid - node * " << NP << ";\n"
                 "    }\n";
        } else if (mode == 1) {
            o << "    bool in = tid < nlanes;\n"
                 "    if (in) {\n"
                 "        tile = tid / " << NP << ";\n"
                 "        gp = tid - tile * " << NP << ";\n"
                 "    }\n";
        } else if (mode == 3) {
            o << "    constexpr int32_t SUBN[] = {" << subn << "};\n"
                 "    bool in = false;\n"
                 "    uint32_t q = 0;\n"
                 "    {\n"
                 "        const uint32_t gb = b0 + blockIdx.x;\n"
                 "        const int sg = jit::seg_of_block(seg, gb);\n"
                 "        const uint32_t u = (gb - seg.bstart[sg]) * blockDim.x + threadIdx.x;\n"
                 "        const uint32_t mi = u >> " << SQL << ";\n"
                 "        q = u & " << (SQ - 1) << "u;\n"
                 "        if (mi < seg.count[sg]) {\n"
                 "            const size_t slot = (size_t)sg * tsegcap + mi;\n"
                 "            const uint32_t entry = tlist[slot];\n"
                 "            const uint32_t rsv = tlist[(size_t)jit::kMixSegs * tsegcap + slot];\n"
                 "            START = rsv & " << ((1u << kStartBits) - 1) << "u;\n"
                 "            FLAGS = rsv & " << (0x7fffffffu & ~((1u << kStartBits) - 1)) << "u;\n"
                 "            START_ANY = (rsv >> 31) != 0;\n"
                 "            tile = entry / " << NP << ";\n"
                 "            gp = entry - tile * " << NP << ";\n"
                 "            in = (tile << " << TSL << ") < nnodes && SUBN[gp * " << SQ << "u + q] > 0;\n"
                 "        }\n"
                 "    }\n";
        } else {
            const int LL = mode == 4 ? NSTL : ST ? STL : TSL;
            if (SQ) o << "    constexpr int32_t SUBN[] = {" << subn << "};\n";
            o << "    bool in = false;\n"
                 "    uint32_t q = 0, st = 0;\n"
                 "    {\n"
                 "        const uint32_t gb = b0 + blockIdx.x;\n"
                 "        const int sg = jit::seg_of_block(seg, gb);\n"
                 "        const uint32_t u = (gb - seg.bstart[sg]) * blockDim.x + threadIdx.x;\n"
                 "        const uint32_t mi = u >> " << LL << ";\n"
                 "        if (mi < seg.count[sg]) {\n"
                 "            const size_t slot = (size_t)sg * tsegcap + mi;\n"
                 "            const uint32_t entry = tlist[slot];\n"
                 "            const uint32_t rsv = tlist[(size_t)jit::kMixSegs * tsegcap + slot];\n"
                 "            START = rsv & " << ((1u << kStartBits) - 1) << "u;\n"
                 "            FLAGS = rsv & " << (0x7fffffffu & ~((1u << kStartBits) - 1)) << "u;\n"
                 "            START_ANY = (rsv >> 31) != 0;\n"
                 "            // (SQ: tile sub-pairs (tile pair) * SQ + q; mode 2 after the sub-tile kernel: times NST plus\n"
                 "            // the sub-tile; mode 4: its lanes' sub-tiles)\n"
                 "            const uint32_t e2 = entry >> " << (mode == 2 ? NSTL : 0) << ";\n"
                 "            st = " << (mode == 4 ? "u & " + std::to_string(std::max(NST - 1, 0)) + "u"
                                       : "entry & " + std::to_string(mode == 2 ? std::max(NST - 1, 0) : 0) + "u") << ";\n"
                 "            const uint32_t tp = e2 >> " << SQL << ";\n"
                 "            q = e2 & " << std::max(SQ - 1, 0) << "u;\n"
                 "            tile = tp / " << NP << ";\n"
                 "            gp = tp - tile * " << NP << ";\n";
            if (mode == 4)
                o << "            node = (tile << " << TSL << ") + (st << " << STL << ");  // (the sub-tile's first)\n";
            else if (ST)
                o << "            node = (tile << " << TSL << ") + (st << " << STL << ") + (u & " << (ST - 1) << "u);\n";
            else
                o << "            node = (tile << " << TSL << ") + (u & " << (TS - 1) << "u);\n";
            o << "            in = node < nnodes;\n"
                 "        }\n"
                 "    }\n";
        }
        T.light_of_part(o, "gp", "    ");
        o << "    pp = gp - " << T.partbase_of() << ";\n"
             "    if (in) {\n";
        if (boxed) {
            if (mode != 1)
                o << "        const float* bx = laabb + 6 * ((size_t)gp * " << SQ << "u + q);\n";
            else
                o << "        const float* bx = laabb + 6 * (" << (T.multi_row ? T.boxbase[(size_t)num_lights] : 0)
                  << "LL + (int64_t)gp);\n";
            if (mode == 4)
                o << "        live = jit::beam_box32(tbox + 6 * ((size_t)tile * " << NST << "u + st), bx, bx + 3, W);  // (false: no live node)\n";
            else
                o << "        live = jit::beam_box32(tbox + 6 * (size_t)tile, bx, bx + 3, W);  // (false: no live node in the tile)\n";
        } else {
            o << "        live = shead.hit(node);\n"
                 "        if (live) {\n"
                 "            double OPN[3];\n"
                 "            shead.over_point(node, OPN);\n";
            if (T.multi_row)
                o << "            const int row = light_row_n(" << T.rows() << ", B.seed, head_key(S, B, shead, node), lt, 0);\n";
            else
                o << "            const int row = 0;\n";
            if (mode == 2 && SQ && T.multi_row) {
                o << "            float bl[3] = {__builtin_huge_valf(), __builtin_huge_valf(), __builtin_huge_valf()};\n"
                     "            float bh[3] = {-__builtin_huge_valf(), -__builtin_huge_valf(), -__builtin_huge_valf()};\n"
                     "            const double* rp = S.light_points + " << T.points() << " + 3 * ((int64_t)row * " << T.ns()
                  << ");\n"
                     "            for (uint32_t k = 0; k < " << PS2 << "u; ++k) {\n"
                     "                const int32_t js = psamp2[((size_t)gp * " << SQ << "u + q) * " << PS2 << "u + k];\n"
                     "                if (js < 0) break;\n"
                     "                for (int a = 0; a < 3; ++a) {\n"
                     "                    bl[a] = fminf(bl[a], __double2float_rd(rp[3 * js + a]));\n"
                     "                    bh[a] = fmaxf(bh[a], __double2float_ru(rp[3 * js + a]));\n"
                     "                }\n"
                     "            }\n"
                     "            jit::beam32(OPN, bl, bh, W);\n";
            } else {
                if (mode == 2 && SQ)
                    o << "            const float* bx = laabb + 6 * ((size_t)gp * " << SQ << "u + q);\n";
                else
                    o << "            const float* bx = laabb + 6 * (" << T.boxbase_of() << " + (int64_t)row * " << T.nparts()
                      << " + pp);\n";
                o << "            jit::beam32(OPN, bx, bx + 3, W);\n";
            }
            o << "        }\n";
        }
        o << "    }\n"
             "    bool alive = live;\n"
             "    bool amb = false;  // a pair the beam cannot decide: mixed\n"
             "    bool ms = false;  // a sphere that may block some of the rays was passed (sphere_beam32 == 2)\n"
             "    int result = 0;\n"
             "    uint32_t RS = START;  // the next kernel's resume point for this pair (Gen::track_start)\n"
             "    bool RS_ANY = START_ANY;\n"
             "    {  // the interval walk on the beam (s = t / |D|: DIST = 1)\n"
             "        const jit::Iv DIST{1.0f - 1e-7f, 1.0f + 1e-7f};\n";
        g.beam = true;
        g.order_opt = order_mode == 2 || (order_mode == 1 && boxed);
        g.u32 = u32_mode >= 1;
        g.beam_stats = stats_on;
        g.stats = false;
        g.track_start = resume;
        g.gate_start = (mode == 2 || mode == 3 || mode == 4) && resume;
        g.JS = boxed ? "jstats + 1024 + 6144" : "jstats + 1024";
        walk32(g, roots, num_roots);
        g.JS = "jstats + 1024";
        g.beam = false;
        g.order_opt = false;
        g.track_start = false;
        g.gate_start = false;
        g.stats = stats_on;
        o << "    }\n";
        const std::string cnt = "(int32_t)min(" + std::to_string(PS) + "u, " + T.ns() + " - pp * " +
                                std::to_string(PS) + "u)";
        const std::string rsv = "RS | FLAGS | (RS_ANY ? 0x80000000u : 0u)";
        if (mode == 1 && K.jit_run_counts) {
            o << "    // the part's samples are unshadowed from every node of the tile (summed over the wave's lanes of the tile)\n"
                 "    jit::add_run_counts(shead, counts, " << NL << ", live && !amb && result == 0, tile << " << TSL << ", "
              << TS << "u, (uint32_t)lt, " << cnt << ", nnodes);\n"
                 "    jit::mix_append(live && amb, tile * " << NP << " + gp, " << rsv << ", mixed, mcount, segcap, err);\n"
                 "    if (jstats != nullptr) {  // diagnostics (FRT_JIT_STATS): tile pairs / mixed tile pairs\n"
                 "        unsigned long long* line = jstats + 32 * (blockIdx.x % 64);\n"
                 "        wave_count(line + 4, live);\n"
                 "        wave_count(line + 5, live && amb);\n"
                 "    }\n"
                 "}\n\n";
        } else if (mode == 3 && K.jit_run_counts) {
            o << "    // the sub-part's samples are unshadowed from every node of the tile (summed over the tile's lanes)\n"
                 "    jit::add_run_counts(shead, counts, " << NL << ", live && !amb && result == 0, tile << " << TSL << ", "
              << TS << "u, (uint32_t)lt, in ? SUBN[gp * " << SQ << "u + q] : 0, nnodes);\n"
                 "    jit::mix_append(live && amb, (tile * " << NP << " + gp) * " << SQ << "u + q, " << rsv
              << ", mixed, mcount, segcap, err);\n"
                 "    if (jstats != nullptr) {  // diagnostics (FRT_JIT_STATS): sub-part pairs / mixed ones\n"
                 "        unsigned long long* line = jstats + 32 * (blockIdx.x % 64);\n"
                 "        wave_count(line + 6, live);\n"
                 "        wave_count(line + 7, live && amb);\n"
                 "    }\n"
                 "}\n\n";
        } else if (mode == 4 && K.jit_run_counts) {
            o << "    // the sub-part's samples are unshadowed from every node of the sub-tile (summed over its lanes)\n"
                 "    jit::add_run_counts(shead, counts, " << NL << ", live && !amb && result == 0, node, " << ST
              << "u, (uint32_t)lt, in ? SUBN[gp * " << SQ << "u + q] : 0, nnodes);\n"
                 "    jit::mix_append(live && amb, (((tile * " << NP << " + gp) * " << SQ << "u + q) << " << NSTL << ") + st, "
              << rsv << ", mixed, mcount, segcap, err);\n"
                 "    if (jstats != nullptr) {  // diagnostics (FRT_JIT_STATS): sub-tile pairs / mixed ones\n"
                 "        unsigned long long* line = jstats + 32 * (blockIdx.x % 64);\n"
                 "        wave_count(line + 8, live);\n"
                 "        wave_count(line + 9, live && amb);\n"
                 "    }\n"
                 "}\n\n";
        } else if (mode == 1) {
            o << "    if (live && !amb && result == 0) {  // the part's samples are unshadowed from every node of the tile\n"
                 "        for (uint32_t n = 0; n < " << TS << "u; ++n) {\n"
                 "            const uint32_t nd = (tile << " << TSL << ") + n;\n"
                 "            if (nd < nnodes && shead.hit(nd)) atomicAdd(counts + nd * " << NL << " + (uint32_t)lt, " << cnt << ");\n"
                 "        }\n"
                 "    }\n"
                 "    jit::mix_append(live && amb, tile * " << NP << " + gp, " << rsv << ", mixed, mcount, segcap, err);\n"
                 "    if (jstats != nullptr) {  // diagnostics (FRT_JIT_STATS): tile pairs / mixed tile pairs\n"
                 "        unsigned long long* line = jstats + 32 * (blockIdx.x % 64);\n"
                 "        wave_count(line + 4, live);\n"
                 "        wave_count(line + 5, live && amb);\n"
                 "    }\n"
                 "}\n\n";
        } else if (mode == 3) {
            o << "    if (live && !amb && result == 0) {  // the sub-part's samples are unshadowed from every node of the tile\n"
                 "        for (uint32_t n = 0; n < " << TS << "u; ++n) {\n"
                 "            const uint32_t nd = (tile << " << TSL << ") + n;\n"
                 "            if (nd < nnodes && shead.hit(nd)) atomicAdd(counts + nd * " << NL
              << " + (uint32_t)lt, SUBN[gp * " << SQ << "u + q]);\n"
                 "        }\n"
                 "    }\n"
                 "    jit::mix_append(live && amb, (tile * " << NP << " + gp) * " << SQ << "u + q, " << rsv
              << ", mixed, mcount, segcap, err);\n"
                 "    if (jstats != nullptr) {  // diagnostics (FRT_JIT_STATS): sub-part pairs / mixed ones\n"
                 "        unsigned long long* line = jstats + 32 * (blockIdx.x % 64);\n"
                 "        wave_count(line + 6, live);\n"
                 "        wave_count(line + 7, live && amb);\n"
                 "    }\n"
                 "}\n\n";
        } else if (mode == 4) {
            o << "    if (live && !amb && result == 0) {  // the sub-part's samples are unshadowed from every node of the sub-tile\n"
                 "        for (uint32_t n = 0; n < " << ST << "u; ++n) {\n"
                 "            const uint32_t nd = node + n;\n"
                 "            if (nd < nnodes && shead.hit(nd)) atomicAdd(counts + nd * " << NL
              << " + (uint32_t)lt, SUBN[gp * " << SQ << "u + q]);\n"
                 "        }\n"
                 "    }\n"
                 "    jit::mix_append(live && amb, (((tile * " << NP << " + gp) * " << SQ << "u + q) << " << NSTL << ") + st, "
              << rsv << ", mixed, mcount, segcap, err);\n"
                 "    if (jstats != nullptr) {  // diagnostics (FRT_JIT_STATS): sub-tile pairs / mixed ones\n"
                 "        unsigned long long* line = jstats + 32 * (blockIdx.x % 64);\n"
                 "        wave_count(line + 8, live);\n"
                 "        wave_count(line + 9, live && amb);\n"
                 "    }\n"
                 "}\n\n";
        } else if (mode == 2 && SQ) {
            o << "    if (live && !amb && result == 0)  // the sub-part's samples are all unshadowed\n"
                 "        atomicAdd(counts + node * " << NL << " + (uint32_t)lt, SUBN[gp * " << SQ << "u + q]);\n"
                 "    jit::mix_append(live && amb, (node * " << NP << " + gp) * " << SQ << "u + q, " << rsv
              << ", mixed, mcount, segcap, err);\n"
                 "    if (jstats != nullptr) {  // diagnostics (FRT_JIT_STATS): pairs / mixed pairs\n"
                 "        unsigned long long* line = jstats + 32 * (blockIdx.x % 64);\n"
                 "        wave_count(line + 2, live);\n"
                 "        wave_count(line + 3, live && amb);\n"
                 "    }\n"
                 "}\n\n";
        } else {
            o << "    if (live && !amb && result == 0)  // the part's samples are all unshadowed\n"
                 "        atomicAdd(counts + node * " << NL << " + (uint32_t)lt, " << cnt << ");\n"
                 "    jit::mix_append(live && amb, node * " << NP << " + gp, " << rsv << ", mixed, mcount, segcap, err);\n"
                 "    if (jstats != nullptr) {  // diagnostics (FRT_JIT_STATS): pairs / mixed pairs\n"
                 "        unsigned long long* line = jstats + 32 * (blockIdx.x % 64);\n"
                 "        wave_count(line + 2, live);\n"
                 "        wave_count(line + 3, live && amb);\n"
                 "    }\n"
                 "}\n\n";
        }
    };
    pair_kernel(0);
    if (TS > 0) {
        pair_kernel(1);
        pair_kernel(2);
    }
    if (SQ > 0) pair_kernel(3);
    if (ST > 0) pair_kernel(4);
    g.u32 = u32_mode >= 2;

    o << "extern \"C\" __global__ void __launch_bounds__(kTraceBlock)" << waves_attr(K.jit_waves) << "\n"
         "frt_jit_shadow(DevScene S, Batch B, const HeadCols shead, uint32_t total, uint32_t m0,\n"
         "               const uint32_t* __restrict__ mixed, jit::SegTable seg, uint32_t b0, uint32_t segcap,\n"
         "               uint32_t all_pairs, const int32_t* __restrict__ psamp, uint32_t subq,\n"
         "               const int32_t* __restrict__ psamp2,\n"
         "               uint32_t lpp, uint64_t magic, uint32_t shift, uint32_t spn,\n"
         "               int32_t* __restrict__ counts, int64_t* __restrict__ redo, unsigned* __restrict__ redo_count,\n"
         "               unsigned redo_cap, unsigned* __restrict__ err, unsigned long long* __restrict__ jstats,\n"
         "               uint32_t nnodes) {\n"
         "    const uint32_t tid = blockIdx.x * blockDim.x + threadIdx.x;\n";
    for (int k = 0; k < num_nodes; ++k) g.node32(k, "    ");
    o << "    jit::Lane32 L;\n"
         "    uint32_t START = 0;  // first node whose subtree this lane walks (the pair kernel's resume point)\n"
         "    bool START_ANY = false;\n"
         "    uint32_t FLAGS = 0;  // boxes every ray of the lane's pair enters (Gen::fbit)\n"
         "    L.valid = L.live = false;\n"
         "    L.node = 0;\n"
         "    L.light = 0;\n"
         "    L.lp = L.op = nullptr;\n"
         "    L.ocap = 0;\n"
         "    double LP[3] = {0.0, 0.0, 0.0}, OP[3] = {0.0, 0.0, 0.0};\n"
         "    uint32_t jall = 0;  // the sample's index among the node's spn samples (k_shadow_redo's lane)\n"
         "    uint32_t j = 0;  // the lane's sample within its part\n"
         "    {\n"
         "        // every pair in order (all_pairs: no pair kernel ran; lanes tid of pairs m0 + tid / lpp) or the\n"
         "        // mixed ones (the block's segment of the list, jit::SegTable)\n"
         "        uint32_t u = tid;\n"
         "        int sg = 0;\n"
         "        if (!all_pairs) {\n"
         "            const uint32_t gb = b0 + blockIdx.x;\n"
         "            sg = jit::seg_of_block(seg, gb);\n"
         "            u = (gb - seg.bstart[sg]) * blockDim.x + threadIdx.x;\n"
         "        }\n"
         "        uint32_t mi = (uint32_t)(((uint64_t)u * magic) >> shift);  // u / lpp\n"
         "        j = u - mi * lpp;\n";
    if (NM > 1)
        o << "        if (subq >= 2 && !all_pairs) {\n"
             "            // node-major lanes (a multi-row light): groups of " << NM << " consecutive list entries, lane w of a\n"
             "            // group = (entry w % kg, node lane w / kg), so a node's samples of the group's entries sit side by\n"
             "            // side and read its own light row together (kg: the group's entries, fewer in the last group)\n"
             "            const uint32_t cnt = seg.count[sg], grp = " << NM << "u * lpp, gi = u / grp, w = u - gi * grp;\n"
             "            const uint32_t base = gi * " << NM << "u;\n"
             "            const uint32_t kg = cnt > base ? min(" << NM << "u, cnt - base) : " << NM << "u;\n"
             "            const uint32_t jn = w / kg;\n"
             "            mi = u < cnt * lpp ? base + (w - jn * kg) : cnt;\n"
             "            j = jn;\n"
             "        }\n";
    o << "        const size_t slot = (size_t)sg * segcap + mi;\n"
         "        if (all_pairs ? tid < total : mi < seg.count[sg]) {\n"
         "            const uint32_t pair = all_pairs ? m0 + mi : mixed[slot];\n"
         "            const uint32_t rsv = all_pairs ? 0u : mixed[(size_t)jit::kMixSegs * segcap + slot];  // resume point\n"
         "            START = rsv & " << ((1u << kStartBits) - 1) << "u;\n"
         "            FLAGS = rsv & " << (0x7fffffffu & ~((1u << kStartBits) - 1)) << "u;\n"
         "            START_ANY = (rsv >> 31) != 0;\n"
         "            // subq 0: (node, part) pairs; 1: sub-part pairs (node pair) * SQ + q (frt_jit_beam_list after\n"
         "            // frt_jit_sub); 2 / 3: the entries frt_jit_sub / frt_jit_subtile leave, walked here without the node\n"
         "            // pair kernel: a tile's (sub-tile's) nodes times the sub-part's samples, the node's samples consecutive\n"
         "            uint32_t gp = 0, q = 0;\n"
         "            if (subq >= 2) {\n"
         "                const uint32_t nn = j / " << std::max(PS2, 1) << "u;\n"
         "                j -= nn * " << std::max(PS2, 1) << "u;\n"
         "                const uint32_t e2 = subq == 3 ? pair >> " << NSTL << " : pair;\n"
         "                const uint32_t tp = e2 >> " << SQL << ";\n"
         "                q = e2 & " << std::max(SQ - 1, 0) << "u;\n"
         "                const uint32_t tile = tp / " << NP << ";\n"
         "                gp = tp - tile * " << NP << ";\n"
         "                L.node = (tile << " << TSL << ") + (subq == 3 ? (pair & " << std::max(NST - 1, 0) << "u) << " << STL
      << " : 0u) + nn;\n"
         "            } else {\n"
         "                const uint32_t npair = subq ? pair >> " << SQL << " : pair;\n"
         "                L.node = npair / " << NP << ";\n"
         "                gp = npair - L.node * " << NP << ";\n"
         "                q = pair & " << std::max(SQ - 1, 0) << "u;\n"
         "            }\n";
    T.light_of_part(o, "gp", "            ");
    o << "            const int32_t jp = subq ? psamp2[(gp * " << std::max(SQ, 1) << "u + q) * " << std::max(PS2, 1)
      << "u + j] : psamp[gp * " << PS << "u + j];  // the light's sample (-1: none)\n"
         "            const uint32_t js = (uint32_t)max(jp, 0);\n"
         "            const bool in_range = L.node < nnodes;  // (a tile's nodes past the batch's last)\n"
         "            L.light = lt;\n"
         "            L.valid = jp >= 0 && in_range;\n"
         "            jall = " << T.first() << " + js;\n"
         "            // the node's head words, loaded side by side ahead of the test of its hit (they sit in columns of their\n"
         "            // own: behind the test their misses would queue up after the material word's)\n"
         "            const uint32_t nd = in_range ? L.node : 0u;\n"
         "            const bool hit = shead.hit(nd);\n"
         "            shead.over_point(nd, OP);\n";
    if (T.multi_row) o << "            const uint64_t key = head_key(S, B, shead, nd);\n";
    o << "            if (L.valid && hit) {\n"
         "                L.live = true;\n";
    if (T.multi_row)
        o << "                const int row = light_row_n(" << T.rows() << ", B.seed, key, lt, 0);\n";
    else
        o << "                const int row = 0;\n";
    o << "                L.lp = S.light_points + " << T.points() << " + 3 * ((int64_t)row * " << T.ns() << " + js);\n"
         "                L.op = shead.op;\n"
         "                L.ocap = shead.cap;\n"
         "                for (int a = 0; a < 3; ++a) LP[a] = L.lp[a];\n"
         "            }\n"
         "        }\n"
         "    }\n"
         "    bool alive = L.live;\n"
         "    bool handed = false;\n"
         "    int shadowed = 0;\n"
         "    bool amb = false;  // a lane whose binary32 walk met an undecidable comparison\n"
         "    {  // binary32 interval walk\n"
         "        int result = 0;\n"
         "        jit::World32 W;\n"
         "        jit::Iv DIST{0.0f, 0.0f};\n"
         "        Ray R64 = Ray{{0, 0, 0}, {0, 0, 1}};  // the binary64 ray, once a leaf needs it\n"
         "        double D64 = 0.0;\n"
         "        bool have64 = false;\n";
    const int nowalk = K.jit_dbg_nowalk;
    if (nowalk == 1) o << "        alive = false;\n";
    o << "        if (alive && !jit::ray32v(LP, OP, W, DIST)) {  // no binary32 bounds for this ray: binary64 walk\n"
         "            amb = true;\n"
         "            alive = false;\n"
         "        }\n";
    if (nowalk == 2) o << "        if (__builtin_amdgcn_readfirstlane(__float_as_int(W.P[0] + W.Q[2] + DIST.hi)) == 1) atomicOr(err, 0u);\n"
                          "        alive = false;\n";
    g.gate_start = resume;
    walk32(g, roots, num_roots);
    g.gate_start = false;
    o << "        shadowed = result;\n    }\n";
    o << "    if (__ballot(amb)) {  // the reference's binary64 arithmetic for those lanes\n"
         "        Ray R0 = Ray{{0, 0, 0}, {0, 0, 1}};\n"
         "        double dist = 0.0;\n"
         "        if (amb) jit::ray64(L, R0, dist);\n"
         "        if (amb && !jit::finite_ray(R0, dist)) {  // to the generic walk (k_shadow_redo)\n"
         "            amb = false;\n"
         "            handed = true;\n"
         "            const unsigned at = atomicAdd(redo_count, 1u);\n"
         "            if (at < redo_cap) redo[at] = (int64_t)L.node * spn + jall;\n"
         "            else atomicOr(err, kErrQueueOverflow);\n"
         "        }\n"
         "        bool alive = amb;\n"
         "        int result = 0;\n";
    for (int ri = 0; ri < num_roots; ++ri) {
        o << "        // ---- world shape " << ri << " (node " << roots[ri] << ")\n";
        o << "        if (__ballot(alive)) {\n";
        o << "            bool any_entry = false;\n";
        g.top(roots[ri], "true", "R0", ri == num_roots - 1, "            ");
        o << "            if (alive && any_entry) alive = false;\n";
        o << "        }\n";
    }
    o << "        if (amb) shadowed = result;\n    }\n";
    o << "    if (jstats != nullptr) {  // diagnostics (FRT_JIT_STATS): live lanes / lanes re-walked in binary64\n"
         "        unsigned long long* line = jstats + 32 * (blockIdx.x % 64);\n"
         "        wave_count(line, L.live);\n"
         "        wave_count(line + 1, amb);\n"
// ... 161 lines not shown
    const auto t0 = std::chrono::steady_clock::now();
    t_obtain_ms = t_load_ms = 0.0;
    hipDeviceProp_t prop;
    std::string arch = "gfx950";
    if (hipGetDeviceProperties(&prop, device) == hipSuccess) {
        const std::string a = prop.gcnArchName;
        arch = a.substr(0, a.find(':'));
    }
    std::string key = arch;
    for (const char* o : kJitOpts) key += std::string(" ") + o;
    key += '\n';
    key += src;
    std::shared_ptr<CodeObject> co;
    bool producer = false;
    {
        std::lock_guard<std::mutex> lk(g_mu);
        auto it = g_cache.find(std::make_pair(device, key));
        if (it != g_cache.end()) {
            g_stat[4]++;
            fns = it->second.fns;
            return 0;
        }
        auto& slot = g_code[key];
        if (!slot) {
            slot = std::make_shared<CodeObject>();
            producer = true;
        }
        co = slot;
    }
    if (producer) {
        std::vector<char> code;
        std::string clog;
        const std::string& dir = K.jit_cache_dir;
        const DiskKey dk = disk_key(key);
        int st = 1;
        bool from_disk = false;
        if (allow_disk && disk_load(dir, dk, code)) {
            g_stat[1]++;
            from_disk = true;
        } else if (compile_code(src, arch, K, code, clog) == 0) {
            disk_store(dir, dk, code);
        } else {
            st = -1;
        }
        {
            std::lock_guard<std::mutex> lk(co->mu);
            co->code.swap(code);
            co->log = clog;
            co->from_disk = from_disk;
            co->state = st;
        }
        co->cv.notify_all();
        if (st < 0) {
            std::lock_guard<std::mutex> lk(g_mu);
            g_code.erase(key);
        }
    } else {
        std::unique_lock<std::mutex> lk(co->mu);
        co->cv.wait(lk, [&] { return co->state != 0; });
    }
    if (co->state < 0) {
        log = co->log;
        return -1;
    }
    t_obtain_ms = ms_since(t0);
    const auto t1 = std::chrono::steady_clock::now();
    std::lock_guard<std::mutex> lk(g_mu);
    auto it = g_cache.find(std::make_pair(device, key));
    if (it != g_cache.end()) {
        fns = it->second.fns;
        return 0;
    }
    CacheEntry ce;
    if (hipSetDevice(device) != hipSuccess || hipModuleLoadData(&ce.mod, co->code.data()) != hipSuccess) {
        (void)hipGetLastError();
        log = "hipModuleLoadData failed";
        if (co->from_disk) {
            std::remove(disk_path(K.jit_cache_dir, disk_key(key)).c_str());
            if (g_code.count(key) && g_code[key] == co) g_code.erase(key);
            return -2;
        }
        return -1;
    }
    hipFunction_t f = nullptr, fb = nullptr, ft = nullptr, fl = nullptr, fs = nullptr, fst = nullptr, ftr = nullptr;
    if (hipModuleGetFunction(&f, ce.mod, "frt_jit_shadow") != hipSuccess ||
        hipModuleGetFunction(&fb, ce.mod, "frt_jit_beam") != hipSuccess) {
        log = "hipModuleGetFunction failed";
        return -1;
    }
    if (src.find("frt_jit_tile(") != std::string::npos &&
        (hipModuleGetFunction(&ft, ce.mod, "frt_jit_tile") != hipSuccess ||
         hipModuleGetFunction(&fl, ce.mod, "frt_jit_beam_list") != hipSuccess)) {
        log = "hipModuleGetFunction failed (tile kernels)";
        return -1;
    }
    t_load_ms = ms_since(t1);
    if (src.find("frt_jit_sub(") != std::string::npos && hipModuleGetFunction(&fs, ce.mod, "frt_jit_sub") != hipSuccess) {
        log = "hipModuleGetFunction failed (sub-part kernel)";
        return -1;
    }
    if (src.find("frt_jit_subtile(") != std::string::npos &&
        hipModuleGetFunction(&fst, ce.mod, "frt_jit_subtile") != hipSuccess) {
        log = "hipModuleGetFunction failed (sub-tile kernel)";
        return -1;
    }
    if (src.find("frt_jit_trace(") != std::string::npos && hipModuleGetFunction(&ftr, ce.mod, "frt_jit_trace") != hipSuccess) {
        log = "hipModuleGetFunction failed (closest-hit kernel)";
        return -1;
    }
    ce.fns.sub = (void*)fs;
    ce.fns.subtile = (void*)fst;
    ce.fns.trace = (void*)ftr;
    ce.fns.shadow = (void*)f;
    ce.fns.beam = (void*)fb;
    ce.fns.tile = (void*)ft;
    ce.fns.list = (void*)fl;
    g_stat[3]++;
    g_cache[std::make_pair(device, key)] = ce;
    fns = ce.fns;
    return 0;
}

extern "C" int frt_jit_cache_stats(int64_t* out, int n) {
    for (int i = 0; i < n && i < 5; ++i) out[i] = g_stat[i].load();
    return 5;
}
```

fast_ray_tracer_amd/csrc/frt_knobs.hpp:

```cpp
#pragma once

#include <stdint.h>

#include <algorithm>
#include <cstdlib>
#include <cstring>
#include <string>

namespace frt_knobs {
inline const char* raw(const char* name) { return std::getenv(name); }
inline bool present(const char* name) { return raw(name) != nullptr; }
inline bool unless_str0(const char* name) {
    const char* e = raw(name);
    return !(e && std::strcmp(e, "0") == 0);
}
inline bool unless_int0(const char* name) {
    const char* e = raw(name);
    return !(e && std::atoi(e) == 0);
}
inline int int_or(const char* name, int def) {
    const char* e = raw(name);
    return e ? std::atoi(e) : def;
}
inline long long ll_or(const char* name, long long def) {
    const char* e = raw(name);
    return e ? std::atoll(e) : def;
}
inline int pow2_upto64(int x) {
    int p = 0;
    while (p < 6 && (2 << p) <= x) ++p;
    return x >= 2 ? 1 << p : 0;
}
inline int waves(const char* name) {
    const int n = int_or(name, 0);
    return n >= 1 && n <= 8 ? n : 0;
}
}

struct UploadKnobs {
    bool jit = true;
    bool jit_beam = true;
    bool jit_node_beam = false;
    bool jit_stats = false;
    bool jit_verbose = false;
    bool jit_dump = false;
    bool jit_trace = true;
    bool mesh = true;
    bool shade_sort = true;
    int shade_stage = 2;
    int queue_sort = 2;
    int queue_sort_shift = 0;
    bool prepare_uniform = true;
    int walk_flags = 0;

    int jit_part = 16;
    int jit_tile = 64;
    int jit_subtile = 16;
    bool jit_subtile_set = false;
    int jit_sub = 16;
    bool jit_inside = true;
    int jit_u32 = 1;
    int jit_order = 1;
    bool jit_resume = true;
    bool jit_flags = true;
    int jit_node_major = 0;
    bool jit_run_counts = true;
    int jit_dbg_nowalk = 0;
    bool jit_trace_dbg = false;
    long long jit_trace_dbg_ray = 0;
    int jit_waves = 0, jit_beam_waves = 0, jit_trace_waves = 0;

    std::string jit_cache_dir;
    std::string jit_co;

    bool warmup_trace = false;
};

inline UploadKnobs read_upload_knobs() {
    using namespace frt_knobs;
    UploadKnobs k;
    k.jit = unless_str0("FRT_JIT");
    k.jit_beam = unless_str0("FRT_JIT_BEAM");
    k.jit_node_beam = int_or("FRT_JIT_NODE_BEAM", 0) != 0;
    k.jit_stats = present("FRT_JIT_STATS");
    k.jit_verbose = present("FRT_JIT_VERBOSE");
    k.jit_dump = present("FRT_JIT_DUMP");
    k.jit_trace = unless_int0("FRT_JIT_TRACE");
    k.mesh = unless_str0("FRT_MESH");
    k.shade_sort = unless_int0("FRT_SHADE_SORT");
    k.shade_stage = int_or("FRT_SHADE_STAGE", 2);
    k.queue_sort = int_or("FRT_QUEUE_SORT", 2);
    k.queue_sort_shift = std::max(0, std::min(16, int_or("FRT_QUEUE_SORT_SHIFT", 0)));
    k.prepare_uniform = unless_int0("FRT_PREPARE_UNIFORM");
    k.walk_flags = int_or("FRT_WALK_FLAGS", 0);
    const int part = int_or("FRT_JIT_PART", 0);
    k.jit_part = part >= 1 && part <= 1024 ? part : 16;
    k.jit_tile = pow2_upto64(int_or("FRT_JIT_TILE", 64));
    k.jit_subtile = pow2_upto64(int_or("FRT_JIT_SUBTILE", 16));
    k.jit_subtile_set = present("FRT_JIT_SUBTILE");
    const int sub = int_or("FRT_JIT_SUB", 16);
    k.jit_sub = sub == 2 || sub == 4 || sub == 8 || sub == 16 || sub == 32 ? sub : 0;
    k.jit_inside = unless_int0("FRT_JIT_INSIDE");
    k.jit_u32 = int_or("FRT_JIT_U32", 1);
    k.jit_order = int_or("FRT_JIT_ORDER", 1);
    k.jit_resume = unless_int0("FRT_JIT_RESUME");
    k.jit_flags = unless_int0("FRT_JIT_FLAGS");
    if (present("FRT_JIT_NODE_MAJOR")) {
        const int nm = int_or("FRT_JIT_NODE_MAJOR", 0);
        k.jit_node_major = nm >= 1 && nm <= 64 && (nm & (nm - 1)) == 0 ? nm : 1;
    }
    k.jit_run_counts = unless_int0("FRT_JIT_RUN_COUNTS");
    k.jit_dbg_nowalk = int_or("FRT_JIT_DBG_NOWALK", 0);
    k.jit_trace_dbg = present("FRT_JIT_TRACE_DBG");
    k.jit_trace_dbg_ray = ll_or("FRT_JIT_TRACE_DBG", 0);
    k.jit_waves = waves("FRT_JIT_WAVES");
    k.jit_beam_waves = waves("FRT_JIT_BEAM_WAVES");
    k.jit_trace_waves = waves("FRT_JIT_TRACE_WAVES");
    if (unless_str0("FRT_JIT_CACHE")) {
        if (const char* d = raw("FRT_JIT_CACHE_DIR")) k.jit_cache_dir = d;
        else if (const char* x = raw("XDG_CACHE_HOME")) k.jit_cache_dir = std::string(x) + "/frt_jit";
        else if (const char* home = raw("HOME")) k.jit_cache_dir = std::string(home) + "/.cache/frt_jit";
    }
    if (const char* co = raw("FRT_JIT_CO")) k.jit_co = co;
    k.warmup_trace = present("FRT_WARMUP_TRACE");
    return k;
}

struct FrameKnobs {
    std::string precision;
    int64_t batch_samples = (int64_t)1 << 23;
    bool eye_cam = true;
    bool head_key0 = true;
    bool cam_fast = true;
    bool shade_split = true;
    bool shade_lazy = true;
    bool fuse_resolve = true;
    int64_t jit_max_pairs = 0;
    int64_t jit_min_pairs = (int64_t)1 << 18;
    bool jit_subtile_deep = true;
    bool jit_trace = true;
    bool jit_trace_stats = false;
    std::string jit_trace_dump;
    int64_t gather_chunk = (int64_t)1 << 24;
    bool gather_jit = true;
    bool gather_queue = true;
    int gather_sort = -1;
    bool share_photons = true;
    bool gi_timing = false;
    double pm_cell_div = 3.0;
    int pm_max_cells_log2 = 0;
};

inline FrameKnobs read_frame_knobs() {
    using namespace frt_knobs;
    FrameKnobs k;
    if (const char* e = raw("FRT_PRECISION")) k.precision = e;
    const long long batch = ll_or("FRT_BATCH_SAMPLES", 0);
    if (batch > 0) k.batch_samples = (int64_t)batch;
    k.eye_cam = unless_int0("FRT_EYE_CAM");
    k.head_key0 = unless_int0("FRT_HEAD_KEY0");
    k.cam_fast = unless_int0("FRT_CAM_FAST");
    k.shade_split = unless_str0("FRT_SHADE_SPLIT");
    k.shade_lazy = unless_str0("FRT_SHADE_LAZY");
    k.fuse_resolve = unless_str0("FRT_FUSE_RESOLVE");
    const long long mp = ll_or("FRT_JIT_MAX_PAIRS", 0);
    k.jit_max_pairs = mp >= 1 && mp < (1ll << 31) ? (int64_t)mp : 0;
    k.jit_min_pairs = (int64_t)ll_or("FRT_JIT_MIN_PAIRS", 1ll << 18);
    k.jit_subtile_deep = unless_int0("FRT_JIT_SUBTILE_DEEP");
    k.jit_trace = unless_int0("FRT_JIT_TRACE");
    k.jit_trace_stats = present("FRT_JIT_TRACE_STATS");
    if (const char* d = raw("FRT_JIT_TRACE_DUMP")) k.jit_trace_dump = d;
    const long long chunk = ll_or("FRT_GATHER_CHUNK", 0);
    if (chunk >= 1024) k.gather_chunk = (int64_t)chunk;
    k.gather_jit = unless_int0("FRT_GATHER_JIT");
    k.gather_queue = unless_str0("FRT_GATHER_QUEUE");
    k.gather_sort = int_or("FRT_GATHER_SORT", -1);
    k.share_photons = unless_int0("FRT_SHARE_PHOTONS");
    k.gi_timing = present("FRT_GI_TIMING");
    if (const char* e = raw("FRT_PM_CELL_DIV")) {
        const double v = std::atof(e);
        if (v >= 1.0 && v <= 16.0) k.pm_cell_div = v;
    }
    const int cells = int_or("FRT_PM_MAX_CELLS_LOG2", 0);
    k.pm_max_cells_log2 = cells >= 10 && cells <= 30 ? cells : 0;
    return k;
}

struct WarmupKnobs {
    bool trace = false;
    int mode = 0;
};

inline WarmupKnobs read_warmup_knobs() {
    WarmupKnobs k;
    k.trace = frt_knobs::present("FRT_WARMUP_TRACE");
    k.mode = frt_knobs::int_or("FRT_WARMUP_MODE", 0);
    return k;
}
```

fast_ray_tracer_amd/runtime.py:

```python
from __future__ import annotations

import ctypes
import os
import weakref
import threading

import numpy as np

from . import build

_lock = threading.Lock()
_host = None


class FrameParams(ctypes.Structure):
    _fields_ = [("row_begin", ctypes.c_int64), ("row_end", ctypes.c_int64), ("row_stride", ctypes.c_int64),
                ("seed", ctypes.c_uint64), ("batch_samples", ctypes.c_int64),
                ("count_reference_rays", ctypes.c_int32), ("precision", ctypes.c_int32)]


PRECISION = {None: 0, "parity": 1, "fast32": 2}


class FrameStats(ctypes.Structure):
    _fields_ = [("primary_rays", ctypes.c_uint64), ("secondary_rays", ctypes.c_uint64),
                ("shadow_rays", ctypes.c_uint64), ("pruned_secondary", ctypes.c_uint64),
                ("hits", ctypes.c_uint64), ("errors", ctypes.c_uint64), ("render_ms", ctypes.c_double),
                ("kernel_ms", ctypes.c_double * 8), ("kernel_launches", ctypes.c_uint64 * 8),
                ("shadow_kernel_bytes", ctypes.c_double), ("gather_rays", ctypes.c_uint64),
                ("photons", ctypes.c_uint64 * 2), ("photon_ms", ctypes.c_double),
                ("shadow_jit", ctypes.c_int32), ("photon_pass", ctypes.c_int32),
                ("sub_ms", ctypes.c_double * 16), ("sub_launches", ctypes.c_uint64 * 16),
                ("shadow_rays_walked", ctypes.c_uint64), ("shadow_tile_pairs", ctypes.c_uint64),
                ("shadow_tile_mixed", ctypes.c_uint64), ("shadow_pairs", ctypes.c_uint64),
                ("shadow_pairs_mixed", ctypes.c_uint64), ("shadow_sub_pairs", ctypes.c_uint64),
                ("shadow_sub_mixed", ctypes.c_uint64), ("shadow_subtile_pairs", ctypes.c_uint64),
                ("shadow_subtile_mixed", ctypes.c_uint64), ("lit_nodes", ctypes.c_uint64),
                ("prepare_uniform_waves", ctypes.c_uint64)]

    def as_dict(self) -> dict:
        names = ["trace", "shadow", "shade", "combine", "resolve", "trace_primary", "prepare", "gi"]
        subs = ["frt_jit_beam", "frt_jit_shadow", "k_gather_est", "k_gather_hit", "frt_jit_tile", "frt_jit_sub",
                "frt_jit_subtile", "k_shade_lit", "k_lit_sort", "k_shade_lit32", "k_feature_resolve"]
        return {
            "primary_rays": int(self.primary_rays), "secondary_rays": int(self.secondary_rays),
            "shadow_rays": int(self.shadow_rays), "pruned_secondary": int(self.pruned_secondary),
            "hits": int(self.hits), "errors": int(self.errors), "render_ms": float(self.render_ms),
            "shadow_kernel_bytes": float(self.shadow_kernel_bytes),
            "gather_rays": int(self.gather_rays), "photons": [int(self.photons[0]), int(self.photons[1])],
            "photon_ms": float(self.photon_ms), "shadow_jit": int(self.shadow_jit),
            "photon_pass": int(self.photon_pass),
            "kernel_ms": {names[i]: float(self.kernel_ms[i]) for i in range(8) if self.kernel_launches[i]},
            "kernel_launches": {names[i]: int(self.kernel_launches[i]) for i in range(8) if self.kernel_launches[i]},
            "sub_ms": {subs[i]: float(self.sub_ms[i]) for i in range(len(subs)) if self.sub_launches[i]},
            "sub_launches": {subs[i]: int(self.sub_launches[i]) for i in range(len(subs)) if self.sub_launches[i]},
            "shadow_rays_walked": int(self.shadow_rays_walked),
            "shadow_tile_pairs": int(self.shadow_tile_pairs), "shadow_tile_mixed": int(self.shadow_tile_mixed),
            "shadow_pairs": int(self.shadow_pairs), "shadow_pairs_mixed": int(self.shadow_pairs_mixed),
            "shadow_sub_pairs": int(self.shadow_sub_pairs), "shadow_sub_mixed": int(self.shadow_sub_mixed),
            "shadow_subtile_pairs": int(self.shadow_subtile_pairs),
            "shadow_subtile_mixed": int(self.shadow_subtile_mixed), "lit_nodes": int(self.lit_nodes),
            "prepare_uniform_waves": int(self.prepare_uniform_waves),
        }


class FeatureBuffers(ctypes.Structure):
    _fields_ = [("geom", ctypes.c_void_p), ("ids", ctypes.c_void_p)]


FEATURE_GEOM_WORDS = 8


def _feature_dict(geom: np.ndarray, ids: np.ndarray) -> dict:
    return {"depth": geom[..., 0], "normal": geom[..., 1:4], "albedo": geom[..., 4:7], "coverage": geom[..., 7],
            "node": ids[..., 0], "material": ids[..., 1]}


class EncodeStats(ctypes.Structure):
    _fields_ = [("values", ctypes.c_uint64), ("undecided", ctypes.c_uint64), ("backend", ctypes.c_int32),
                ("decline", ctypes.c_int32), ("mode", ctypes.c_int32), ("device", ctypes.c_int32),
                ("rgb_max", ctypes.c_double * 3), ("srgb_max", ctypes.c_double * 3), ("upload_ms", ctypes.c_double),
                ("kernel_ms", ctypes.c_double), ("readback_ms", ctypes.c_double), ("patch_ms", ctypes.c_double),
                ("host_ms", ctypes.c_double)]

    def as_dict(self) -> dict:
        return {"values": int(self.values), "undecided": int(self.undecided),
                "backend": ENCODE_BACKENDS[self.backend], "decline": ENCODE_DECLINES[self.decline],
                "mode": ENCODE_MODES[self.mode], "device": int(self.device), "rgb_max": list(self.rgb_max),
                "srgb_max": list(self.srgb_max), "upload_ms": float(self.upload_ms),
                "kernel_ms": float(self.kernel_ms), "readback_ms": float(self.readback_ms),
                "patch_ms": float(self.patch_ms), "host_ms": float(self.host_ms)}


ENCODE_MODES = ("ppm_scaled", "ppm_clamped", "png")
ENCODE_BACKENDS = ("host", "device", "auto")
ENCODE_DECLINES = (None, "zero_max", "non_finite", "over_cap", "no_device", "too_large")


DENOISE_BACKENDS = ("host", "device", "auto")
DENOISE_MAX_ITERATIONS = 8


class DenoiseParams(ctypes.Structure):
    _fields_ = [("iterations", ctypes.c_int32), ("normal_squarings", ctypes.c_int32), ("demodulate", ctypes.c_int32),
                ("match_material", ctypes.c_int32), ("sigma_color", ctypes.c_double), ("sigma_depth", ctypes.c_double),
                ("albedo_eps", ctypes.c_double)]

    def __init__(self, **fields):
        super().__init__()
        host_lib().frt_denoise_defaults(ctypes.byref(self))
        for k, v in fields.items():
            if k not in dict(self._fields_):
                raise TypeError("frt: DenoiseParams has no field %r" % (k,))
            setattr(self, k, v)

    def as_dict(self) -> dict:
        return {k: getattr(self, k) for k, _ in self._fields_}


class DenoiseStats(ctypes.Structure):
    _fields_ = [("pixels", ctypes.c_uint64), ("valid_pixels", ctypes.c_uint64), ("iterations", ctypes.c_int32),
                ("backend", ctypes.c_int32), ("device", ctypes.c_int32), ("reserved", ctypes.c_int32),
                ("upload_ms", ctypes.c_double), ("pack_ms", ctypes.c_double), ("atrous_ms", ctypes.c_double),
                ("atrous_iter_ms", ctypes.c_double * DENOISE_MAX_ITERATIONS), ("readback_ms", ctypes.c_double),
                ("host_ms", ctypes.c_double)]

    def as_dict(self) -> dict:
        return {"pixels": int(self.pixels), "valid_pixels": int(self.valid_pixels),
                "iterations": int(self.iterations), "backend": DENOISE_BACKENDS[self.backend],
                "device": int(self.device), "upload_ms": float(self.upload_ms), "pack_ms": float(self.pack_ms),
                "atrous_ms": float(self.atrous_ms),
                "atrous_iter_ms": [float(self.atrous_iter_ms[i]) for i in range(self.iterations)],
                "readback_ms": float(self.readback_ms), "host_ms": float(self.host_ms)}


def host_lib(auto_build: bool = False) -> ctypes.CDLL:
    global _host
    with _lock:
        if _host is not None:
            return _host
        if auto_build:
            build.build_host()
        if not os.path.exists(build.HOST_LIB) or not os.path.exists(build.DEVICE_LIB):
            raise RuntimeError("frt native libraries are not built: run __graft_entry__.build() "
                               "(expected %s and %s)" % (build.HOST_LIB, build.DEVICE_LIB))
        lib = ctypes.CDLL(build.HOST_LIB, mode=ctypes.RTLD_GLOBAL)
        vp = ctypes.c_void_p
        lib.frt_captured.restype = ctypes.c_int
        for fn in ("frt_captured_camera", "frt_captured_world"):
            getattr(lib, fn).restype = vp
        for fn in ("frt_captured_usteps", "frt_captured_vsteps"):
            getattr(lib, fn).restype = ctypes.c_size_t
        lib.frt_captured_jitter.restype = ctypes.c_int
        lib.frt_camera_hsize.restype = ctypes.c_size_t
        lib.frt_camera_hsize.argtypes = [vp]
        lib.frt_camera_vsize.restype = ctypes.c_size_t
        lib.frt_camera_vsize.argtypes = [vp]
        lib.frt_host_prepare.restype = vp
        lib.frt_host_prepare.argtypes = [vp, vp, ctypes.c_size_t, ctypes.c_size_t, ctypes.c_bool, ctypes.c_int]
        lib.frt_host_last_error.restype = ctypes.c_char_p
        lib.frt_host_set_camera.restype = ctypes.c_int
        lib.frt_host_set_camera.argtypes = [vp, vp, ctypes.c_size_t, ctypes.c_size_t, ctypes.c_bool]
        lib.frt_camera_look_at.restype = vp
        lib.frt_camera_look_at.argtypes = [ctypes.POINTER(ctypes.c_double)] * 3 + [
            ctypes.c_size_t, ctypes.c_size_t, ctypes.c_double, ctypes.c_double, vp]
        for fn in ("frt_camera_fov", "frt_camera_distance", "frt_camera_aperture_size"):
            getattr(lib, fn).restype = ctypes.c_double
            getattr(lib, fn).argtypes = [vp]
        lib.frt_camera_set_aperture_size.restype = None
        lib.frt_camera_set_aperture_size.argtypes = [vp, ctypes.c_double]
        lib.frt_camera_free.restype = None
        lib.frt_camera_free.argtypes = [vp]
        lib.frt_device_count.restype = ctypes.c_int
        lib.frt_last_error.restype = ctypes.c_char_p
        lib.frt_render_rows.restype = ctypes.c_int
        lib.frt_render_rows.argtypes = [vp, ctypes.POINTER(FrameParams), vp, ctypes.POINTER(FrameStats)]
        lib.frt_render_rows_device.restype = ctypes.c_int
        lib.frt_render_rows_device.argtypes = [vp, ctypes.POINTER(FrameParams), vp, ctypes.POINTER(FrameStats)]
        lib.frt_scene_release.argtypes = [vp]
        lib.frt_encode_ppm.restype = ctypes.c_size_t
        lib.frt_encode_ppm.argtypes = [vp, ctypes.c_size_t, ctypes.c_size_t, ctypes.c_int, vp, ctypes.c_size_t]
        lib.frt_encode16.restype = ctypes.c_int
        lib.frt_encode16.argtypes = [vp, ctypes.c_int, ctypes.c_size_t, ctypes.c_size_t, ctypes.c_int, ctypes.c_int,
                                     ctypes.c_int, vp, ctypes.POINTER(EncodeStats)]
        lib.frt_encode_last.restype = None
        lib.frt_encode_last.argtypes = [ctypes.POINTER(EncodeStats)]
        lib.frt_encode_stats_size.restype = ctypes.c_size_t
        if lib.frt_encode_stats_size() != ctypes.sizeof(EncodeStats):
            raise RuntimeError("frt: frt_encode_stats is %d bytes in %s, runtime.py EncodeStats %d: rebuild"
                               % (lib.frt_encode_stats_size(), build.HOST_LIB, ctypes.sizeof(EncodeStats)))
        lib.frt_srgb_max_full.restype = None
        lib.frt_srgb_max_full.argtypes = [vp, ctypes.c_size_t, ctypes.c_size_t, ctypes.POINTER(ctypes.c_double)]
        lib.frt_encode_selftest.restype = ctypes.c_int64
        lib.frt_encode_selftest.argtypes = [ctypes.c_int64, ctypes.c_uint64, ctypes.POINTER(ctypes.c_double),
                                            ctypes.c_int]
        lib.write_ppm_file.restype = ctypes.c_int
        lib.write_ppm_file.argtypes = [vp, ctypes.c_bool, ctypes.c_char_p]
        lib.write_png.restype = ctypes.c_int
        lib.write_png.argtypes = [vp, ctypes.c_char_p]
        lib.frt_frame_stats_size.restype = ctypes.c_size_t
        if lib.frt_frame_stats_size() != ctypes.sizeof(FrameStats):
            raise RuntimeError("frt: frt_frame_stats is %d bytes in %s, runtime.py FrameStats %d: rebuild"
                               % (lib.frt_frame_stats_size(), build.DEVICE_LIB, ctypes.sizeof(FrameStats)))
        lib.frt_frame_params_size.restype = ctypes.c_size_t
        if lib.frt_frame_params_size() != ctypes.sizeof(FrameParams):
            raise RuntimeError("frt: frt_frame_params is %d bytes in %s, runtime.py FrameParams %d: rebuild"
                               % (lib.frt_frame_params_size(), build.DEVICE_LIB, ctypes.sizeof(FrameParams)))
        lib.frt_feature_geom_words.restype = ctypes.c_size_t
        if lib.frt_feature_geom_words() != FEATURE_GEOM_WORDS:
            raise RuntimeError("frt: frt_feature_buffers.geom has %d doubles per pixel in %s, runtime.py %d: rebuild"
                               % (lib.frt_feature_geom_words(), build.DEVICE_LIB, FEATURE_GEOM_WORDS))
        fb, fp, fs = ctypes.POINTER(FeatureBuffers), ctypes.POINTER(FrameParams), ctypes.POINTER(FrameStats)
        for fn in ("frt_render_features_device", "frt_render_features_host"):
            getattr(lib, fn).restype = ctypes.c_int
            getattr(lib, fn).argtypes = [vp, fp, fb, fs]
        for fn in ("frt_render_feature_views_device", "frt_render_feature_views_host"):
            getattr(lib, fn).restype = ctypes.c_int
            getattr(lib, fn).argtypes = [vp, vp, ctypes.c_int32, fp, fb, fs]
        for fn, mirror in (("frt_denoise_params_size", DenoiseParams), ("frt_denoise_stats_size", DenoiseStats)):
            getattr(lib, fn).restype = ctypes.c_size_t
            if getattr(lib, fn)() != ctypes.sizeof(mirror):
                raise RuntimeError("frt: %s() is %d bytes in %s, runtime.py %s %d: rebuild"
                                   % (fn, getattr(lib, fn)(), build.DEVICE_LIB, mirror.__name__,
                                      ctypes.sizeof(mirror)))
        dp, ds, i64 = ctypes.POINTER(DenoiseParams), ctypes.POINTER(DenoiseStats), ctypes.c_int64
        lib.frt_denoise_defaults.restype = None
        lib.frt_denoise_defaults.argtypes = [dp]
        lib.frt_denoise_host.restype = ctypes.c_int
        lib.frt_denoise_host.argtypes = [vp, vp, vp, i64, i64, i64, dp, vp, ds]
        lib.frt_denoise_device.restype = ctypes.c_int
        lib.frt_denoise_device.argtypes = [vp, vp, vp, ctypes.c_int, i64, i64, i64, dp, ctypes.c_int, vp, ds]
        lib.frt_denoise.restype = ctypes.c_int
        lib.frt_denoise.argtypes = [vp, vp, vp, ctypes.c_int, i64, i64, i64, dp, ctypes.c_int, ctypes.c_int, vp, ds]
        lib.frt_denoise_error.restype = ctypes.c_char_p
        lib.frt_denoise_release.restype = None
        _host = lib
        return lib


class Scene:

    def __init__(self, scene_so: str, asset_root: str | None = None):
        lib = host_lib()
        self._so = ctypes.CDLL(scene_so, mode=ctypes.RTLD_GLOBAL)
        self._so.frt_scene_main.restype = ctypes.c_int
        cwd = os.getcwd()
        lib.frt_reset_libc_rng()
        try:
            if asset_root:
                os.chdir(asset_root)
            rc = self._so.frt_scene_main()
        finally:
            os.chdir(cwd)
        if rc != 0 or not lib.frt_captured():
            raise RuntimeError("scene main() did not reach render_multi (rc=%d): %s" % (rc, scene_so))
        self.camera = lib.frt_captured_camera()
        self.world = lib.frt_captured_world()
        self.usteps = int(lib.frt_captured_usteps())
        self.vsteps = int(lib.frt_captured_vsteps())
        self.jitter = bool(lib.frt_captured_jitter())
        st = (ctypes.c_ushort * 3)()
        lib.frt_captured_drand48(st)
# ... 44 lines not shown
        self.vsteps = int(vsteps)
        self.jitter = bool(jitter)
        self.drand48_state = tuple(drand48_state)
        self.width = int(lib.frt_camera_hsize(camera))
        self.height = int(lib.frt_camera_vsize(camera))
        self.name = name

    @property
    def spp(self) -> int:
        return self.usteps * self.vsteps


class GpuRenderer:

    def __init__(self, scene: Scene, device: int = 0):
        self.lib = host_lib()
        if self.lib.frt_device_count() <= 0:
            raise RuntimeError("frt: no HIP device visible; the GPU path has no CPU fallback")
        release_render_multi()
        self.scene = scene
        self.frame = scene
        self.device = device
        h = self.lib.frt_host_prepare(scene.camera, scene.world, scene.usteps, scene.vsteps, scene.jitter, device)
        if not h:
            raise RuntimeError("frt: scene upload failed: " + self.lib.frt_host_last_error().decode())
        self.handle = h

    def set_camera(self, view) -> None:
        if view.world != self.scene.world:
            raise ValueError("frt: set_camera needs a view of this renderer's world (Scene.view / Scene.view_of)")
        if self.lib.frt_host_set_camera(self.handle, view.camera, view.usteps, view.vsteps, view.jitter) != 0:
            raise RuntimeError("frt: set_camera failed: " + self.lib.frt_host_last_error().decode())
        self.frame = view

    def _strip_cams(self, who: str, views, allow_empty: bool = False):
        views = list(views)
        if not views and not allow_empty:
            raise ValueError("frt: %s needs at least one view" % who)
        if any(v.world != self.scene.world for v in views):
            raise ValueError("frt: %s needs views of this renderer's world (Scene.view / Scene.view_of)" % who)
        lib = self.lib
        lib.frt_camera_size.restype = ctypes.c_size_t
        lib.frt_flatten_camera.restype = ctypes.c_int
        lib.frt_flatten_camera.argtypes = [ctypes.c_void_p, ctypes.c_size_t, ctypes.c_size_t, ctypes.c_bool,
                                           ctypes.c_void_p, ctypes.POINTER(ctypes.c_void_p)]
        size = lib.frt_camera_size()
        cams = ctypes.create_string_buffer(size * max(1, len(views)))
        for k, v in enumerate(views):
            table = ctypes.c_void_p()
            rc = lib.frt_flatten_camera(v.camera, v.usteps, v.vsteps, v.jitter, ctypes.addressof(cams) + k * size,
                                        ctypes.byref(table))
            lib.frt_camera_free(table)
            if rc:
                raise RuntimeError("frt: out of host memory for a view's sample table")
        return views, cams

    def render_views(self, views, row_begin: int = 0, row_end: int | None = None, row_stride: int = 1,
                     seed: int = 0x5EED, batch_samples: int = 0, stats: bool = False, precision: str | None = None):
        views, cams = self._strip_cams("render_views", views)
        lib = self.lib
        lib.frt_render_views_host.restype = ctypes.c_int
        lib.frt_render_views_host.argtypes = [ctypes.c_void_p, ctypes.c_void_p, ctypes.c_int32,
                                              ctypes.POINTER(FrameParams), ctypes.c_void_p, ctypes.POINTER(FrameStats)]
        first, own = views[0], self.frame
        borrow = (first.usteps, first.vsteps) != (own.usteps, own.vsteps)
        if borrow:
            self.set_camera(first)
        try:
            p = self._params(row_begin, first.height if row_end is None else row_end, row_stride, seed, batch_samples,
                             precision)
            n = self.rows_in(p.row_begin, p.row_end, row_stride)
            out = np.zeros((len(views), n, first.width, 4), dtype=np.float64)
            st = FrameStats()
            rc = lib.frt_render_views_host(self.handle, cams, len(views), ctypes.byref(p),
                                           out.ctypes.data_as(ctypes.c_void_p), ctypes.byref(st) if stats else None)
            err = lib.frt_last_error().decode() if rc != 0 else ""
        finally:
            if borrow:
                self.set_camera(own)
        if rc != 0:
            raise RuntimeError("frt render_views failed: " + err)
        return (out, st) if stats else out

    def close(self) -> None:
        if getattr(self, "handle", None):
            self.lib.frt_scene_release(self.handle)
            self.handle = None

    def __del__(self):
        try:
            self.close()
        except Exception:
            pass

    def _params(self, row_begin, row_end, row_stride, seed, batch_samples, precision=None):
        p = FrameParams()
        if not isinstance(precision, int) and precision not in PRECISION:
            raise ValueError("frt: precision %r is not supported (\"parity\", \"fast32\" or None)" % (precision,))
        p.precision = precision if isinstance(precision, int) else PRECISION[precision]
        p.row_begin = row_begin
        p.row_end = self.frame.height if row_end is None else row_end
        p.row_stride = row_stride
        p.seed = seed
        p.batch_samples = batch_samples
        return p

    @staticmethod
    def rows_in(row_begin, row_end, row_stride) -> int:
        return len(range(row_begin, row_end, row_stride))

    def render(self, row_begin: int = 0, row_end: int | None = None, row_stride: int = 1, seed: int = 0x5EED,
               batch_samples: int = 0, stats: bool = False, precision: str | None = None):
        p = self._params(row_begin, row_end, row_stride, seed, batch_samples, precision)
        n = self.rows_in(p.row_begin, p.row_end, row_stride)
        out = np.zeros((n, self.frame.width, 4), dtype=np.float64)
        st = FrameStats()
        rc = self.lib.frt_render_rows(self.handle, ctypes.byref(p), out.ctypes.data_as(ctypes.c_void_p),
                                      ctypes.byref(st) if stats else None)
        if rc != 0:
            raise RuntimeError("frt render failed: " + self.lib.frt_last_error().decode())
        return (out, st) if stats else out

    def render_into(self, device_ptr: int, row_begin: int = 0, row_end: int | None = None, row_stride: int = 1,
                    seed: int = 0x5EED, batch_samples: int = 0, stats: bool = False, precision: str | None = None):
        p = self._params(row_begin, row_end, row_stride, seed, batch_samples, precision)
        st = FrameStats()
        rc = self.lib.frt_render_rows_device(self.handle, ctypes.byref(p), ctypes.c_void_p(device_ptr),
                                             ctypes.byref(st) if stats else None)
        if rc != 0:
            raise RuntimeError("frt render failed: " + self.lib.frt_last_error().decode())
        return st if stats else None

    def render_features(self, row_begin: int = 0, row_end: int | None = None, row_stride: int = 1,
                        seed: int = 0x5EED, batch_samples: int = 0, stats: bool = False):
        p = self._params(row_begin, row_end, row_stride, seed, batch_samples)
        n = self.rows_in(p.row_begin, p.row_end, row_stride)
        geom = np.zeros((n, self.frame.width, FEATURE_GEOM_WORDS), dtype=np.float64)
        ids = np.zeros((n, self.frame.width, 2), dtype=np.int32)
        bufs = FeatureBuffers(geom.ctypes.data, ids.ctypes.data)
        st = FrameStats()
        rc = self.lib.frt_render_features_host(self.handle, ctypes.byref(p), ctypes.byref(bufs),
                                               ctypes.byref(st) if stats else None)
        if rc != 0:
            raise RuntimeError("frt render_features failed: " + self.lib.frt_last_error().decode())
        out = _feature_dict(geom, ids)
        return (out, st) if stats else out

    def render_features_into(self, geom_ptr: int | None, ids_ptr: int | None, row_begin: int = 0,
                             row_end: int | None = None, row_stride: int = 1, seed: int = 0x5EED,
                             batch_samples: int = 0, stats: bool = False):
        p = self._params(row_begin, row_end, row_stride, seed, batch_samples)
        bufs = FeatureBuffers(geom_ptr or None, ids_ptr or None)
        st = FrameStats()
        rc = self.lib.frt_render_features_device(self.handle, ctypes.byref(p), ctypes.byref(bufs),
                                                 ctypes.byref(st) if stats else None)
        if rc != 0:
            raise RuntimeError("frt render_features failed: " + self.lib.frt_last_error().decode())
        return st if stats else None

    def render_feature_views(self, views, row_begin: int = 0, row_end: int | None = None, row_stride: int = 1,
                             seed: int = 0x5EED, batch_samples: int = 0, stats: bool = False):
        views, cams = self._strip_cams("render_feature_views", views, allow_empty=True)
        first, own = views[0] if views else self.frame, self.frame
        borrow = (first.usteps, first.vsteps) != (own.usteps, own.vsteps)
        if borrow:
            self.set_camera(first)
# ... 381 lines not shown
```

include/frt_device.h:

```cpp
#ifndef FRT_DEVICE_H
#define FRT_DEVICE_H

#ifndef __HIPCC_RTC__
#include <stddef.h>
#include <stdint.h>
#endif

#ifdef __cplusplus
extern "C" {
#endif

#define FRT_ABI_VERSION 3u

enum frt_node_type {
    FRT_CONE = 0,
    FRT_CUBE = 1,
    FRT_CYLINDER = 2,
    FRT_PLANE = 3,
    FRT_SMOOTH_TRIANGLE = 4,
    FRT_SPHERE = 5,
    FRT_TOROID = 6,
    FRT_TRIANGLE = 7,
    FRT_CSG = 8,
    FRT_GROUP = 9
// ... 86 lines not shown
    int32_t gi_path_length;
    int32_t trace_caustic_map;
    int32_t trace_global_map;
    int64_t photon_count;
    double irradiance_radius;
    double cone_filter_k;
} frt_config;

typedef struct frt_scene {
    uint32_t abi_version;
    int32_t num_nodes;
    const frt_node *nodes;
    int32_t num_roots;
    int32_t pad0;
    const int32_t *roots;
    int32_t num_xforms;
    int32_t pad1;
    const double *xforms;
    int64_t prim_len;
    const double *prim_data;
    int32_t num_materials;
    int32_t num_patterns;
    const frt_material *materials;
    const frt_pattern *patterns;
    int32_t num_textures;
    int32_t pad2;
    const frt_texture *textures;
    int64_t texel_len;
    const double *texels;
    int32_t num_lights;
    int32_t pad3;
    const frt_light *lights;
    int64_t light_point_len;
    const double *light_points;
    frt_camera camera;
    const double *sample_table;
    frt_config config;
} frt_scene;

typedef struct frt_scene_handle frt_scene_handle;

typedef struct frt_frame_params {
    int64_t row_begin, row_end;
    int64_t row_stride;
    uint64_t seed;
    int64_t batch_samples;
    int32_t count_reference_rays;
    int32_t precision;
} frt_frame_params;

enum frt_precision { FRT_PRECISION_DEFAULT = 0, FRT_PRECISION_PARITY = 1, FRT_PRECISION_FAST32 = 2 };

typedef struct frt_frame_stats {
    uint64_t primary_rays;
    uint64_t secondary_rays;
    uint64_t shadow_rays;
    uint64_t pruned_secondary;
    uint64_t hits;
    uint64_t errors;
    double render_ms;
    double kernel_ms[8];
    uint64_t kernel_launches[8];
    double shadow_kernel_bytes;
    uint64_t gather_rays;
    uint64_t photons[2];
    double photon_ms;
    int32_t shadow_jit;
    int32_t photon_pass;
    double sub_ms[16];
    uint64_t sub_launches[16];
    uint64_t shadow_rays_walked;
    uint64_t shadow_tile_pairs;
    uint64_t shadow_tile_mixed;
    uint64_t shadow_pairs;
    uint64_t shadow_pairs_mixed;
    uint64_t shadow_sub_pairs;
    uint64_t shadow_sub_mixed;
    uint64_t shadow_subtile_pairs;
    uint64_t shadow_subtile_mixed;
    uint64_t lit_nodes;
    uint64_t prepare_uniform_waves;
} frt_frame_stats;

int frt_device_count(void);

int frt_device_warmup(int device);

void *frt_host_pinned_alloc(size_t bytes);
void frt_host_pinned_free(void *p);

size_t frt_frame_stats_size(void);

size_t frt_frame_params_size(void);

const char *frt_last_error(void);

int frt_scene_upload(const frt_scene *scene, int device, frt_scene_handle **out);

int frt_scene_set_camera(frt_scene_handle *h, const frt_camera *cam, const double *sample_table);

int frt_render_rows(frt_scene_handle *h, const frt_frame_params *params, double *host_rgba,
                    frt_frame_stats *stats);

int frt_render_rows_device(frt_scene_handle *h, const frt_frame_params *params, double *device_rgba,
                           frt_frame_stats *stats);

int frt_render_views_host(frt_scene_handle *h, const frt_camera *cams, int32_t nviews, const frt_frame_params *params,
                          double *host_rgba, frt_frame_stats *stats);
int frt_render_views_device(frt_scene_handle *h, const frt_camera *cams, int32_t nviews,
                            const frt_frame_params *params, double *device_rgba, frt_frame_stats *stats);

typedef struct frt_feature_buffers {
    double *geom;
    int32_t *ids;
} frt_feature_buffers;

int frt_render_features_device(frt_scene_handle *h, const frt_frame_params *params, const frt_feature_buffers *dev,
                               frt_frame_stats *stats);
int frt_render_features_host(frt_scene_handle *h, const frt_frame_params *params, const frt_feature_buffers *host,
                             frt_frame_stats *stats);
int frt_render_feature_views_device(frt_scene_handle *h, const frt_camera *cams, int32_t nviews,
                                    const frt_frame_params *params, const frt_feature_buffers *dev,
                                    frt_frame_stats *stats);
int frt_render_feature_views_host(frt_scene_handle *h, const frt_camera *cams, int32_t nviews,
                                  const frt_frame_params *params, const frt_feature_buffers *host,
                                  frt_frame_stats *stats);

size_t frt_feature_geom_words(void);

void frt_scene_release(frt_scene_handle *h);

int frt_jit_check(const frt_scene *scene, char *log, size_t log_cap, char *src, size_t src_cap);

int frt_mesh_check(const frt_scene *scene, int64_t *out, int n);

int64_t frt_math_selftest(int64_t n, uint64_t seed);

int64_t frt_shade32_selftest(int64_t n, uint64_t seed, double *out, int nout);

int frt_jit_cache_stats(int64_t *out, int n);

int frt_upload_phases(double *out, int n);

int frt_photon_pass_stats(int64_t *out, int n);

int frt_pm_balance(const double *pos, int64_t n, int32_t *heap_of, int8_t *plane);
int frt_pm_estimate(int device, const double *pos, const double *power, const uint8_t *theta_phi, int64_t n,
                    const double *queries, int64_t nq, double radius, int32_t k, double cone_k,
                    double *irrad, int64_t *found);

enum frt_encode_mode {
    FRT_ENCODE_PPM_SCALED = 0,
    FRT_ENCODE_PPM_CLAMPED = 1,
    FRT_ENCODE_PNG = 2
};

enum frt_encode_backend { FRT_ENCODE_HOST = 0, FRT_ENCODE_DEVICE = 1, FRT_ENCODE_AUTO = 2 };

enum frt_encode_decline {
    FRT_ENCODE_TAKEN = 0,
    FRT_ENCODE_ZERO_MAX = 1,
    FRT_ENCODE_NON_FINITE = 2,
    FRT_ENCODE_OVER_CAP = 3,
    FRT_ENCODE_NO_DEVICE = 4,
    FRT_ENCODE_TOO_LARGE = 5
};

#define FRT_ENCODE_MARGIN 0x1p-40

typedef struct frt_encode_stats {
    uint64_t values;
    uint64_t undecided;
    int32_t backend;
    int32_t decline;
    int32_t mode;
    int32_t device;
// ... 76 lines not shown
```

Baseline: 532,900.

## Add super-tile level to hierarchical shadow beam culling with split kernel

Adds a coarser super-tile stage to the JIT shadow culling hierarchy. Tile-level light-pair tests now run on super-tile boxes (built by a new k_sup_boxes kernel), and a new split kernel refines the surviving mixed super-tile/sub-part pairs down to individual tiles before the existing sub-tile and node list stages. The aim is fewer coarse pair tests and better early culling of shadow rays. In exchange it adds an extra kernel launch, a host round-trip sync to read the mixed counts, more pair-index encoding logic, and new stats plumbing.

```diff
diff --git a/fast_ray_tracer_amd/csrc/frt_engine.hip b/fast_ray_tracer_amd/csrc/frt_engine.hip
--- a/fast_ray_tracer_amd/csrc/frt_engine.hip
+++ b/fast_ray_tracer_amd/csrc/frt_engine.hip
@@ -517,6 +517,29 @@
         }
     }
     if (tbox != nullptr) tile_box(node, n, hit, op, tbox, tile_log2, stbox, sub_log2);
+}
+
+__global__ void __launch_bounds__(kBlock)
+k_sup_boxes(const float* __restrict__ tbox, int64_t ntiles, int nt_log2, float* __restrict__ supbox, int64_t nsup) {
+    const int64_t s = (int64_t)blockIdx.x * blockDim.x + threadIdx.x;
+    if (s >= nsup) return;
+    float lo[3] = {__builtin_huge_valf(), __builtin_huge_valf(), __builtin_huge_valf()};
+    float hi[3] = {-__builtin_huge_valf(), -__builtin_huge_valf(), -__builtin_huge_valf()};
+    const int64_t t0 = s << nt_log2, t1 = min(t0 + ((int64_t)1 << nt_log2), ntiles);
+    for (int64_t t = t0; t < t1; ++t) {
+        const float* b = tbox + 6 * t;
+#pragma unroll
+        for (int a = 0; a < 3; ++a) {
+            lo[a] = fminf(lo[a], b[a]);
+            hi[a] = fmaxf(hi[a], b[a + 3]);
+        }
+    }
+    float* o = supbox + 6 * s;
+#pragma unroll
+    for (int a = 0; a < 3; ++a) {
+        o[a] = lo[a];
+        o[a + 3] = hi[a];
+    }
 }
 
 #ifdef FRT_SHADOW_WAVES
@@ -2047,6 +2070,14 @@
     uint32_t* s2list = nullptr;
     int64_t s2list_cap = 0;
     uint64_t subtile_pairs = 0, subtile_mixed = 0;
+    void* jit_split = nullptr;
+    int sup = 0;
+    bool sup_on = false;
+    float* supbox = nullptr;
+    int64_t supbox_cap = 0;
+    uint32_t* xlist = nullptr;
+    int64_t xlist_cap = 0;
+    frt_shadow_stage_stats stages{};
     float* tbox = nullptr;
     int64_t tbox_cap = 0;
     uint32_t* tlist = nullptr;
@@ -2956,6 +2987,21 @@
 
 size_t frt_frame_stats_size(void) { return sizeof(frt_frame_stats); }
 
+size_t frt_shadow_stages(const frt_scene_handle* h, frt_shadow_stage_stats* out) {
+    if (h != nullptr && out != nullptr) {
+        *out = h->stages;
+        out->supertile = h->sup_on ? (uint64_t)h->sup : 0;
+        out->tile_pairs = h->tile_pairs;
+        out->tile_mixed = h->tile_mixed;
+        out->sub_pairs = h->sub_pairs;
+        out->sub_mixed = h->sub_mixed;
+        out->subtile_pairs = h->subtile_pairs;
+        out->subtile_mixed = h->subtile_mixed;
+        out->rays_walked = h->rays_walked;
+    }
+    return sizeof(frt_shadow_stage_stats);
+}
+
 static std::mutex g_warm_mu;
 static hipStream_t g_warm_stream[64] = {};
 
@@ -3143,6 +3189,9 @@
             h->jit_subtile = fns.subtile;
             h->jit_trace = sc->config.all_ni_one ? fns.trace : nullptr;
             h->subtile = fns.subtile ? K.jit_subtile : 0;
+            h->jit_split = fns.split;
+            h->sup = fns.split && h->tile > 0 && h->sub > 0 ? frt_jit_supertile(K) : 0;
+            h->sup_on = h->sup > 0;
             if (h->jit_shadow) {
                 h->redo_cap = 1u << 20;
                 void* p = nullptr;
@@ -3230,7 +3279,7 @@
                     h->light_psamp2 = upload(h, ps2.data(), ps2.size(), rc);
                     h->light_sbox = upload(h, sbox.data(), sbox.size(), rc);
                 }
-                if (rc || hipMalloc((void**)&h->mcount, 4 * frt::jit::kMixSegs * frt::jit::kMixLine * sizeof(unsigned)) != hipSuccess) {
+                if (rc || hipMalloc((void**)&h->mcount, 5 * frt::jit::kMixSegs * frt::jit::kMixLine * sizeof(unsigned)) != hipSuccess) {
                     frt_scene_release(h);
                     return fail("frt_scene_upload: light box / pair list allocation failed");
                 }
@@ -3396,6 +3445,14 @@
             if (spairs)
                 std::fprintf(stderr, "frt jit stats: sub-part pair kernel (%d sub-parts): live sub-pairs %llu, mixed %llu (%.2f%%)\n",
                              h->sub, spairs, smixed, 100.0 * (double)smixed / (double)spairs);
+            unsigned long long xpairs = 0, xmixed = 0;
+            for (int j = 0; j < 64; ++j) {
+                xpairs += c[32 * j + 10];
+                xmixed += c[32 * j + 11];
+            }
+            if (xpairs)
+                std::fprintf(stderr, "frt jit stats: split kernel (%d nodes per super-tile): live tile sub-pairs %llu, mixed %llu (%.2f%%)\n",
+                             h->sup, xpairs, xmixed, 100.0 * (double)xmixed / (double)xpairs);
             if (upairs)
                 std::fprintf(stderr, "frt jit stats: sub-tile pair kernel (%d nodes per sub-tile): live sub-tile pairs %llu, mixed %llu (%.2f%%)\n",
                              h->subtile, upairs, umixed, 100.0 * (double)umixed / (double)upairs);
@@ -3474,6 +3531,8 @@
     hip_ignore(hipFree(h->s2list));
     hip_ignore(hipFree(h->tredo));
     hip_ignore(hipFree(h->tbox));
+    hip_ignore(hipFree(h->supbox));
+    hip_ignore(hipFree(h->xlist));
     hip_ignore(hipFree(h->err));
     for (hipEvent_t e : h->ev_pool) hip_ignore(hipEventDestroy(e));
     if (h->ev[0]) hip_ignore(hipEventDestroy(h->ev[0]));
@@ -3714,16 +3773,19 @@
         if (subbed && h->up.jit_node_beam) {
             kMaxPairs = std::min<int64_t>(kMaxPairs, (int64_t)(0xFFFFFFFFull / (uint64_t)h->sub));
         } else if (subbed) {
+            const int run = h->sup > h->tile ? h->sup : h->tile;
+            const int fine = h->subtile > 0 && h->subtile < h->tile ? h->subtile : h->tile;
             int stl = 0;
-            while (h->subtile > 0 && (1 << stl) < h->tile / h->subtile) ++stl;
+            while ((fine << stl) < run) ++stl;
             const uint64_t per_tile = ((uint64_t)NP * (uint64_t)h->sub) << stl;
-            const int64_t tiled_max = (int64_t)(0xFFFFFFFFull / per_tile) * h->tile * NP;
+            const int64_t tiled_max = (int64_t)(0xFFFFFFFFull / per_tile) * run * NP;
             kMaxPairs = std::min<int64_t>(std::min<int64_t>(tiled_max, (int64_t)0xFFFFFFFFll),
                                           mp ? mp : INT64_MAX);
         }
         if (n * NP > kMaxPairs) {
             int64_t per = std::max<int64_t>(1, kMaxPairs / NP);
-            if (h->tile > 0) per = std::max<int64_t>(h->tile, per / h->tile * h->tile);
+            const int64_t unit = h->sup > h->tile ? h->sup : h->tile;
+            if (unit > 0) per = std::max<int64_t>(unit, per / unit * unit);
             for (int64_t off = 0; off < n; off += per)
                 launch_shadow(h, B, rec.at(off), std::min(per, n - off), counts + off * h->S.num_lights, node0 + off);
             return;
@@ -3735,7 +3797,8 @@
         unsigned* mc_sub = h->mcount + kMixSegs * kMixLine;
         unsigned* mc_subtile = h->mcount + 2 * kMixSegs * kMixLine;
         unsigned* mc_node = h->mcount + 3 * kMixSegs * kMixLine;
-        if (beam_on) hip_ignore(hipMemsetAsync(h->mcount, 0, 4 * kMixSegs * kMixLine * sizeof(unsigned), h->stream));
+        unsigned* mc_split = h->mcount + 4 * kMixSegs * kMixLine;
+        if (beam_on) hip_ignore(hipMemsetAsync(h->mcount, 0, 5 * kMixSegs * kMixLine * sizeof(unsigned), h->stream));
         uint64_t total_mixed = 0;
         const uint32_t* direct_in = nullptr;
         uint32_t direct_subq = 0, direct_nodes = 0;
@@ -3748,8 +3811,13 @@
             const float* list_boxes = h->light_aabb;
             int tl = 0;
             while ((1 << tl) < h->tile) ++tl;
+            const bool use_sup = subbed && h->sup > h->tile && h->sup_on && h->jit_split && h->supbox &&
+                                 (B.level == 0 || h->fk.jit_supertile_deep);
+            int rl = tl;
+            while (use_sup && (1 << rl) < h->sup) ++rl;
+            uint32_t runl = (uint32_t)rl;
             if (tiled) {
-                const int64_t ntiles = (n + h->tile - 1) >> tl;
+                const int64_t ntiles = (n + ((int64_t)1 << rl) - 1) >> rl;
                 uint32_t ntp = (uint32_t)(ntiles * NP);
                 const int64_t tblocks = (ntiles * NP + frt::kTraceBlock - 1) / frt::kTraceBlock;
                 tsegcap = (uint32_t)std::max<int64_t>(frt::kTraceBlock, ((tblocks + kMixSegs - 1) / kMixSegs) * frt::kTraceBlock);
@@ -3759,12 +3827,12 @@
                     launch_shadow(h, B, rec, n, counts, node0);
                     return;
                 }
-                const float* tb = h->tbox + 6 * (node0 >> tl);
+                const float* tb = use_sup ? h->supbox + 6 * (node0 >> rl) : h->tbox + 6 * (node0 >> tl);
                 const uint32_t* no_list = nullptr;
                 uint32_t zero = 0;
                 void* targs[] = {&h->S, (void*)&B, (void*)&rec, &ntp, &nn, (void*)&tb, (void*)&no_list, &tseg, &zero, &zero,
                                  &h->light_aabb, &counts, &h->tlist, &mc_tile, &tsegcap, &h->err, &h->jit_stats,
-                                 &h->light_psamp2};
+                                 &h->light_psamp2, &runl};
                 hipError_t le;
                 {
                     KTimer tt(h, h->cur_st, 12);
@@ -3809,7 +3877,7 @@
                             uint32_t b0u = (uint32_t)b0;
                             void* sargs[] = {&h->S, (void*)&B, (void*)&rec, &zero, &nn, (void*)&tb, &h->tlist, (void*)&sseg, &b0u,
                                              &tsegcap, &h->light_sbox, &counts, &h->slist, &mc_sub, (void*)&ssegcap, &h->err,
-                                             &h->jit_stats, &h->light_psamp2};
+                                             &h->jit_stats, &h->light_psamp2, &runl};
                             se = hipModuleLaunchKernel((hipFunction_t)h->jit_sub, (unsigned)std::min(max_blocks, sblocks - b0), 1, 1,
                                                        frt::kTraceBlock, 1, 1, 0, h->stream, sargs, nullptr);
                         }
@@ -3832,13 +3900,65 @@
                     const bool subtiled = h->jit_subtile && h->subtile > 0 && h->subtile < h->tile && h->stbox &&
                                           (B.level == 0 || h->fk.jit_subtile_deep);
                     const uint64_t nst = subtiled ? (uint64_t)(h->tile / h->subtile) : 0;
-                    list_blocks = seg_table(h->host_mcount, ssegcap, subtiled ? nst : (uint64_t)h->tile, tseg, listed_s);
+                    const uint64_t after = subtiled ? nst : (uint64_t)h->tile;
+                    const uint64_t nt = use_sup ? (uint64_t)(h->sup / h->tile) : 0;
+                    list_blocks = seg_table(h->host_mcount, ssegcap, use_sup ? nt : after, tseg, listed_s);
                     h->sub_pairs += listed * (uint64_t)h->sub;
                     h->sub_mixed += listed_s;
                     listed = listed_s;
                     list_in = h->slist;
                     list_segcap = ssegcap;
                     list_boxes = h->light_sbox;
+                    if (use_sup && listed_s > 0) {
+                        const uint64_t xblocks = list_blocks;
+                        const frt::jit::SegTable xseg = tseg;
+                        const uint32_t xsegcap = (uint32_t)std::max<uint64_t>(
+                            frt::kTraceBlock, ((xblocks + kMixSegs - 1) / kMixSegs) * frt::kTraceBlock);
+                        if (grow(&h->xlist, h->xlist_cap, 2 * (int64_t)xsegcap * kMixSegs)) {
+                            (void)hipGetLastError();
+                            h->jit_shadow = nullptr;
+                            hip_ignore(hipMemsetAsync(counts, 0, (size_t)n * h->S.num_lights * sizeof(int32_t), h->stream));
+                            launch_shadow(h, B, rec, n, counts, node0);
+                            return;
+                        }
+                        const float* tileb = h->tbox + 6 * (node0 >> tl);
+                        hipError_t xe = hipSuccess;
+                        {
+                            KTimer tx(h, h->cur_st, 19);
+                            const uint64_t max_blocks = ((1ull << 31) - 1) / frt::kTraceBlock;
+                            uint32_t zero = 0;
+                            for (uint64_t b0 = 0; b0 < xblocks && xe == hipSuccess; b0 += max_blocks) {
+                                uint32_t b0u = (uint32_t)b0;
+                                void* xargs[] = {&h->S, (void*)&B, (void*)&rec, &zero, &nn, (void*)&tileb, &h->slist, (void*)&xseg,
+                                                 &b0u, (void*)&ssegcap, &h->light_sbox, &counts, &h->xlist, &mc_split,
+                                                 (void*)&xsegcap, &h->err, &h->jit_stats, &h->light_psamp2, &runl};
+                                xe = hipModuleLaunchKernel((hipFunction_t)h->jit_split, (unsigned)std::min(max_blocks, xblocks - b0),
+                                                           1, 1, frt::kTraceBlock, 1, 1, 0, h->stream, xargs, nullptr);
+                            }
+                        }
+                        if (xe != hipSuccess) {
+                            std::fprintf(stderr, "frt: scene-specialised split kernel launch failed (%s); no super-tiles\n",
+                                         hipGetErrorString(xe));
+                            (void)hipGetLastError();
+                            h->sup_on = false;
+                            hip_ignore(hipMemsetAsync(counts, 0, (size_t)n * h->S.num_lights * sizeof(int32_t), h->stream));
+                            launch_shadow(h, B, rec, n, counts, node0);
+                            return;
+                        }
+                        if (hipMemcpyAsync(h->host_mcount.data(), mc_split, h->host_mcount.size() * sizeof(unsigned),
+                                           hipMemcpyDeviceToHost, h->stream) != hipSuccess ||
+                            stream_sync(h) != hipSuccess)
+                            return;
+                        uint64_t listed_x = 0;
+                        list_blocks = seg_table(h->host_mcount, xsegcap, after, tseg, listed_x);
+                        h->stages.split_pairs += listed_s * nt;
+                        h->stages.split_mixed += listed_x;
+                        listed = listed_s = listed_x;
+                        list_in = h->xlist;
+                        list_segcap = xsegcap;
+                    }
+                    const uint32_t* const ts_list = list_in;
+                    const uint32_t ts_segcap = list_segcap;
                     if (subtiled && listed_s > 0) {
                         const uint64_t tblocks = list_blocks;
                         const frt::jit::SegTable s1seg = tseg;
@@ -3861,9 +3981,9 @@
                             uint32_t zero = 0;
                             for (uint64_t b0 = 0; b0 < tblocks && ue == hipSuccess; b0 += max_blocks) {
                                 uint32_t b0u = (uint32_t)b0;
-                                void* uargs[] = {&h->S, (void*)&B, (void*)&rec, &zero, &nn, (void*)&stb, &h->slist, (void*)&s1seg,
-                                                 &b0u, (void*)&ssegcap, &h->light_sbox, &counts, &h->s2list, &mc_subtile,
-                                                 (void*)&s2segcap, &h->err, &h->jit_stats, &h->light_psamp2};
+                                void* uargs[] = {&h->S, (void*)&B, (void*)&rec, &zero, &nn, (void*)&stb, (void*)&ts_list, (void*)&s1seg,
+                                                 &b0u, (void*)&ts_segcap, &h->light_sbox, &counts, &h->s2list, &mc_subtile,
+                                                 (void*)&s2segcap, &h->err, &h->jit_stats, &h->light_psamp2, &runl};
                                 ue = hipModuleLaunchKernel((hipFunction_t)h->jit_subtile, (unsigned)std::min(max_blocks, tblocks - b0),
                                                            1, 1, frt::kTraceBlock, 1, 1, 0, h->stream, uargs, nullptr);
                             }
@@ -3929,7 +4049,7 @@
                         uint32_t b0u = (uint32_t)b0;
                         void* largs[] = {&h->S, (void*)&B, (void*)&rec, &zero, &nn, (void*)&no_box, (void*)&list_in, &tseg, &b0u,
                                          &list_segcap, (void*)&list_boxes, &counts, nout, &mc_node, &segcap, &h->err,
-                                         &h->jit_stats, &h->light_psamp2};
+                                         &h->jit_stats, &h->light_psamp2, &runl};
                         le = hipModuleLaunchKernel((hipFunction_t)h->jit_list, (unsigned)std::min(max_blocks, list_blocks - b0), 1, 1,
                                                    frt::kTraceBlock, 1, 1, 0, h->stream, largs, nullptr);
                     }
@@ -3942,7 +4062,7 @@
                     uint32_t zero = 0;
                     void* bargs[] = {&h->S, (void*)&B, (void*)&rec, &np, &nn, (void*)&no_box, (void*)&no_list, &no_seg, &zero, &zero,
                                      &h->light_aabb, &counts, nout, &mc_node, &segcap, &h->err, &h->jit_stats,
-                                     &h->light_psamp2};
+                                     &h->light_psamp2, &runl};
                     le = hipModuleLaunchKernel((hipFunction_t)h->jit_beam, grid_for(npairs, frt::kTraceBlock), 1, 1,
                                                frt::kTraceBlock, 1, 1, 0, h->stream, bargs, nullptr);
                     h->node_pairs += (uint64_t)npairs;
@@ -4697,6 +4817,7 @@
     h->heads_walked = 0;
     h->tile_pairs = h->tile_mixed = h->node_pairs = h->node_mixed = h->sub_pairs = h->sub_mixed = 0;
     h->subtile_pairs = h->subtile_mixed = 0;
+    h->stages = frt_shadow_stage_stats{};
     const int rc = render_frame(h, P, dev_out, st);
     if (rc) h->gi.built = false;
     return rc;
@@ -4852,6 +4973,15 @@
                                    subtiles ? h->stbox : nullptr, stl, L.counts, dense ? h->spawn_masks : nullptr,
                                    h->up.prepare_uniform ? 1 : 0);
                 FRT_HIP(hipGetLastError());
+                if (tiles && h->sup > h->tile && h->sup_on && (d == 0 || h->fk.jit_supertile_deep)) {
+                    int sl = 0;
+                    while ((1 << sl) < h->sup) ++sl;
+                    const int64_t ntiles = (n + h->tile - 1) >> tl, nsup = (n + h->sup - 1) >> sl;
+                    if (grow(&h->supbox, h->supbox_cap, 6 * (nsup + 1))) return -1;
+                    hipLaunchKernelGGL(k_sup_boxes, dim3(grid_for(nsup)), dim3(kBlock), 0, h->stream, h->tbox, ntiles,
+                                       sl - tl, h->supbox, nsup);
+                    FRT_HIP(hipGetLastError());
+                }
                 if (dense) {
                     hipcub::CountingInputIterator<int64_t> idx(0);
                     hipcub::TransformInputIterator<uint32_t, MaskPopc, hipcub::CountingInputIterator<int64_t>> popc(
@@ -5125,6 +5255,8 @@
     st->shadow_subtile_pairs = h->subtile_pairs;
     st->shadow_subtile_mixed = h->subtile_mixed;
     collect_timings(h, st);
+    h->stages.split_ms = st->sub_ms[11];
+    h->stages.split_launches = st->sub_launches[11];
 }
 
 static int feature_frame(frt_scene_handle* h, const frt_frame_params* P, const frt_feature_buffers* dev,
diff --git a/fast_ray_tracer_amd/csrc/frt_jit.h b/fast_ray_tracer_amd/csrc/frt_jit.h
--- a/fast_ray_tracer_amd/csrc/frt_jit.h
+++ b/fast_ray_tracer_amd/csrc/frt_jit.h
@@ -16,6 +16,9 @@
 int frt_jit_sub_ps(int PS, int Q);
 int frt_jit_light_subparts(const frt_light& L, const double* light_points, const std::vector<int32_t>& order, int PS,
                            int Q, std::vector<int32_t>& order2);
+inline int frt_jit_supertile(const UploadKnobs& K) {
+    return K.jit_tile > 0 && K.jit_sub > 0 && K.jit_supertile > K.jit_tile ? K.jit_supertile : 0;
+}
 int frt_jit_light_parts(const frt_light& L, const double* light_points, int PS, std::vector<int32_t>& order);
 
 std::string frt_jit_shadow_source(const frt::WalkNode* wn, int num_nodes, const int32_t* roots, int num_roots,
@@ -28,6 +31,7 @@
     void* list = nullptr;
     void* sub = nullptr;
     void* subtile = nullptr;
+    void* split = nullptr;
     void* trace = nullptr;
 };
 int frt_jit_compile(const std::string& src, int device, const UploadKnobs& K, FrtJitFns& fns, std::string& log);
diff --git a/fast_ray_tracer_amd/csrc/frt_jit.hip b/fast_ray_tracer_amd/csrc/frt_jit.hip
--- a/fast_ray_tracer_amd/csrc/frt_jit.hip
+++ b/fast_ray_tracer_amd/csrc/frt_jit.hip
@@ -1190,6 +1190,11 @@
     int STL = 0, NSTL = 0;
     while (ST && (1 << STL) < ST) ++STL;
     while (NST && (1 << NSTL) < NST) ++NSTL;
+    const int SUP = frt_jit_supertile(K);
+    const int NT = SUP ? SUP / TS : 0;
+    int SUPL = 0, NTL = 0;
+    while (SUP && (1 << SUPL) < SUP) ++SUPL;
+    while (NT && (1 << NTL) < NT) ++NTL;
     const int PS = K.jit_part;
     const int PS2 = SQ ? frt_jit_sub_ps(PS, SQ) : 0;
     const int NM = K.jit_node_major ? K.jit_node_major : T.multi_row ? 4 : 1;
@@ -1199,20 +1204,35 @@
             const int c = p + 1 < T.parts[(size_t)l] ? PS : lights[l].num_samples - (int)p * PS;
             for (int x : frt_jit_sub_sizes(std::max(c, 0), SQ)) subn += (subn.empty() ? "" : ", ") + std::to_string(x);
         }
+    auto decode_sub = [&](const std::string& e3, const std::string& ind) {
+        if (SUP)
+            o << ind << "const uint32_t e4 = " << e3 << " >> " << NTL << ";\n"
+              << ind << "const uint32_t tp = e4 >> " << SQL << ";\n"
+              << ind << "q = e4 & " << std::max(SQ - 1, 0) << "u;\n"
+              << ind << "const uint32_t sup = tp / " << NP << ";\n"
+              << ind << "gp = tp - sup * " << NP << ";\n"
+              << ind << "tile = (sup << " << NTL << ") + (" << e3 << " & " << (NT - 1) << "u);\n";
+        else
+            o << ind << "const uint32_t tp = " << e3 << " >> " << SQL << ";\n"
+              << ind << "q = " << e3 << " & " << std::max(SQ - 1, 0) << "u;\n"
+              << ind << "tile = tp / " << NP << ";\n"
+              << ind << "gp = tp - tile * " << NP << ";\n";
+    };
     auto pair_kernel = [&](int mode) {
         const char* name = mode == 0 ? "frt_jit_beam" : mode == 1 ? "frt_jit_tile" : mode == 2 ? "frt_jit_beam_list"
-                         : mode == 3 ? "frt_jit_sub" : "frt_jit_subtile";
-        const bool boxed = mode == 1 || mode == 3 || mode == 4;
+                         : mode == 3 ? "frt_jit_sub" : mode == 4 ? "frt_jit_subtile" : "frt_jit_split";
+        const bool boxed = mode == 1 || mode == 3 || mode == 4 || mode == 5;
+        const std::string RL = SUP ? "runl" : std::to_string(TSL), RN = SUP ? "(1u << runl)" : std::to_string(TS) + "u";
         o << "extern \"C\" __global__ void __launch_bounds__(kTraceBlock)" << waves_attr(K.jit_beam_waves) << "\n"
           << name << "(DevScene S, Batch B, const HeadCols shead, uint32_t nlanes, uint32_t nnodes,\n"
              "             const float* __restrict__ tbox, const uint32_t* __restrict__ tlist, jit::SegTable seg,\n"
              "             uint32_t b0, uint32_t tsegcap,\n"
              "             const float* __restrict__ laabb, int32_t* __restrict__ counts, uint32_t* __restrict__ mixed,\n"
              "             unsigned* __restrict__ mcount, uint32_t segcap, unsigned* __restrict__ err,\n"
-             "             unsigned long long* __restrict__ jstats, const int32_t* __restrict__ psamp2) {\n"
+             "             unsigned long long* __restrict__ jstats, const int32_t* __restrict__ psamp2, uint32_t runl) {\n"
              "    const uint32_t tid = blockIdx.x * blockDim.x + threadIdx.x;\n";
         for (int k = 0; k < num_nodes; ++k) g.node32(k, "    ");
-        o << "    uint32_t node = 0, gp = 0, pp = 0, tile = 0;\n"
+        o << "    uint32_t node = 0, gp = 0, pp = 0, tile = 0, entry_w = 0;\n"
              "    bool live = false;\n"
              "    uint32_t START = 0, FLAGS = 0;  // (frt_jit_beam_list: the tile's resume point and flags)\n"
              "    bool START_ANY = false;\n"
@@ -1248,20 +1268,27 @@
                  "            START_ANY = (rsv >> 31) != 0;\n"
                  "            tile = entry / " << NP << ";\n"
                  "            gp = entry - tile * " << NP << ";\n"
-                 "            in = (tile << " << TSL << ") < nnodes && SUBN[gp * " << SQ << "u + q] > 0;\n"
+                 "            in = (tile << " << RL << ") < nnodes && SUBN[gp * " << SQ << "u + q] > 0;\n"
                  "        }\n"
                  "    }\n";
         } else {
-            const int LL = mode == 4 ? NSTL : ST ? STL : TSL;
+            const int LL = mode == 5 ? NTL : mode == 4 ? NSTL : ST ? STL : TSL;
             if (SQ) o << "    constexpr int32_t SUBN[] = {" << subn << "};\n";
             o << "    bool in = false;\n"
                  "    uint32_t q = 0, st = 0;\n"
                  "    {\n"
                  "        const uint32_t gb = b0 + blockIdx.x;\n"
                  "        const int sg = jit::seg_of_block(seg, gb);\n"
-                 "        const uint32_t u = (gb - seg.bstart[sg]) * blockDim.x + threadIdx.x;\n"
-                 "        const uint32_t mi = u >> " << LL << ";\n"
-                 "        if (mi < seg.count[sg]) {\n"
+                 "        const uint32_t u = (gb - seg.bstart[sg]) * blockDim.x + threadIdx.x;\n";
+            if (mode == 5 && NT < 64)
+                o << "        const uint32_t mi = ((u >> 6) << " << (6 - NTL) << ") + (u & " << ((64 >> NTL) - 1) << "u);\n"
+                     "        const uint32_t tsel = (u & 63u) >> " << (6 - NTL) << ";\n";
+            else if (mode == 5)
+                o << "        const uint32_t mi = u >> " << LL << ";\n"
+                     "        const uint32_t tsel = u & " << (NT - 1) << "u;\n";
+            else
+                o << "        const uint32_t mi = u >> " << LL << ";\n";
+            o << "        if (mi < seg.count[sg]) {\n"
                  "            const size_t slot = (size_t)sg * tsegcap + mi;\n"
                  "            const uint32_t entry = tlist[slot];\n"
                  "            const uint32_t rsv = tlist[(size_t)jit::kMixSegs * tsegcap + slot];\n"
@@ -1270,14 +1297,22 @@
                  "            START_ANY = (rsv >> 31) != 0;\n"
                  "            // (SQ: tile sub-pairs (tile pair) * SQ + q; mode 2 after the sub-tile kernel: times NST plus\n"
                  "            // the sub-tile; mode 4: its lanes' sub-tiles)\n"
+                 "            // (frt_jit_split: (super-tile pair) * SQ + q, its lanes' tiles of the run)\n"
+                 "            entry_w = entry;\n"
                  "            const uint32_t e2 = entry >> " << (mode == 2 ? NSTL : 0) << ";\n"
                  "            st = " << (mode == 4 ? "u & " + std::to_string(std::max(NST - 1, 0)) + "u"
-                                       : "entry & " + std::to_string(mode == 2 ? std::max(NST - 1, 0) : 0) + "u") << ";\n"
-                 "            const uint32_t tp = e2 >> " << SQL << ";\n"
-                 "            q = e2 & " << std::max(SQ - 1, 0) << "u;\n"
-                 "            tile = tp / " << NP << ";\n"
-                 "            gp = tp - tile * " << NP << ";\n";
-            if (mode == 4)
+                                       : "entry & " + std::to_string(mode == 2 ? std::max(NST - 1, 0) : 0) + "u") << ";\n";
+            if (mode == 5)
+                o << "            const uint32_t tp = e2 >> " << SQL << ";\n"
+                     "            q = e2 & " << std::max(SQ - 1, 0) << "u;\n"
+                     "            const uint32_t sup = tp / " << NP << ";\n"
+                     "            gp = tp - sup * " << NP << ";\n"
+                     "            tile = (sup << " << NTL << ") + tsel;\n";
+            else
+                decode_sub("e2", "            ");
+            if (mode == 5)
+                o << "            node = tile << " << TSL << ";  // (the tile's first)\n";
+            else if (mode == 4)
                 o << "            node = (tile << " << TSL << ") + (st << " << STL << ");  // (the sub-tile's first)\n";
             else if (ST)
                 o << "            node = (tile << " << TSL << ") + (st << " << STL << ") + (u & " << (ST - 1) << "u);\n";
@@ -1348,7 +1383,7 @@
         g.beam_stats = stats_on;
         g.stats = false;
         g.track_start = resume;
-        g.gate_start = (mode == 2 || mode == 3 || mode == 4) && resume;
+        g.gate_start = (mode == 2 || mode == 3 || mode == 4 || mode == 5) && resume;
         g.JS = boxed ? "jstats + 1024 + 6144" : "jstats + 1024";
         walk32(g, roots, num_roots);
         g.JS = "jstats + 1024";
@@ -1361,10 +1396,39 @@
         const std::string cnt = "(int32_t)min(" + std::to_string(PS) + "u, " + T.ns() + " - pp * " +
                                 std::to_string(PS) + "u)";
         const std::string rsv = "RS | FLAGS | (RS_ANY ? 0x80000000u : 0u)";
-        if (mode == 1 && K.jit_run_counts) {
+        const std::string pair_q = "(tile * " + NP + " + gp) * " + std::to_string(SQ) + "u + q";
+        const std::string sub_entry =
+            !SUP ? pair_q
+                 : "runl == " + std::to_string(SUPL) + "u ? " + pair_q + " : ((((tile >> " + std::to_string(NTL) + ") * " + NP +
+                       " + gp) * " + std::to_string(SQ) + "u + q) << " + std::to_string(NTL) + ") + (tile & " +
+                       std::to_string(NT - 1) + "u)";
+        const std::string st_entry = "(" + (SUP ? std::string("entry_w") : "(" + pair_q + ")") + " << " +
+                                     std::to_string(NSTL) + ") + st";
+        if (mode == 5) {
+            if (K.jit_run_counts)
+                o << "    // the sub-part's samples are unshadowed from every node of the tile (summed over the tile's lanes)\n"
+                     "    jit::add_run_counts(shead, counts, " << NL << ", live && !amb && result == 0, node, " << TS
+                  << "u, (uint32_t)lt, in ? SUBN[gp * " << SQ << "u + q] : 0, nnodes);\n";
+            else
+                o << "    if (live && !amb && result == 0) {  // the sub-part's samples are unshadowed from every node of the tile\n"
+                     "        for (uint32_t n = 0; n < " << TS << "u; ++n) {\n"
+                     "            const uint32_t nd = node + n;\n"
+                     "            if (nd < nnodes && shead.hit(nd)) atomicAdd(counts + nd * " << NL
+                  << " + (uint32_t)lt, SUBN[gp * " << SQ << "u + q]);\n"
+                     "        }\n"
+                     "    }\n";
+            o << "    jit::mix_append(live && amb, (entry_w << " << NTL << ") + (tile & " << (NT - 1) << "u), " << rsv
+              << ", mixed, mcount, segcap, err);\n"
+                 "    if (jstats != nullptr) {  // diagnostics (FRT_JIT_STATS): split pairs / mixed ones\n"
+                 "        unsigned long long* line = jstats + 32 * (blockIdx.x % 64);\n"
+                 "        wave_count(line + 10, live);\n"
+                 "        wave_count(line + 11, live && amb);\n"
+                 "    }\n"
+                 "}\n\n";
+        } else if (mode == 1 && K.jit_run_counts) {
             o << "    // the part's samples are unshadowed from every node of the tile (summed over the wave's lanes of the tile)\n"
-                 "    jit::add_run_counts(shead, counts, " << NL << ", live && !amb && result == 0, tile << " << TSL << ", "
-              << TS << "u, (uint32_t)lt, " << cnt << ", nnodes);\n"
+                 "    jit::add_run_counts(shead, counts, " << NL << ", live && !amb && result == 0, tile << " << RL << ", "
+              << RN << ", (uint32_t)lt, " << cnt << ", nnodes);\n"
                  "    jit::mix_append(live && amb, tile * " << NP << " + gp, " << rsv << ", mixed, mcount, segcap, err);\n"
                  "    if (jstats != nullptr) {  // diagnostics (FRT_JIT_STATS): tile pairs / mixed tile pairs\n"
                  "        unsigned long long* line = jstats + 32 * (blockIdx.x % 64);\n"
@@ -1374,10 +1438,9 @@
                  "}\n\n";
         } else if (mode == 3 && K.jit_run_counts) {
             o << "    // the sub-part's samples are unshadowed from every node of the tile (summed over the tile's lanes)\n"
-                 "    jit::add_run_counts(shead, counts, " << NL << ", live && !amb && result == 0, tile << " << TSL << ", "
-              << TS << "u, (uint32_t)lt, in ? SUBN[gp * " << SQ << "u + q] : 0, nnodes);\n"
-                 "    jit::mix_append(live && amb, (tile * " << NP << " + gp) * " << SQ << "u + q, " << rsv
-              << ", mixed, mcount, segcap, err);\n"
+                 "    jit::add_run_counts(shead, counts, " << NL << ", live && !amb && result == 0, tile << " << RL << ", "
+              << RN << ", (uint32_t)lt, in ? SUBN[gp * " << SQ << "u + q] : 0, nnodes);\n"
+                 "    jit::mix_append(live && amb, " << sub_entry << ", " << rsv << ", mixed, mcount, segcap, err);\n"
                  "    if (jstats != nullptr) {  // diagnostics (FRT_JIT_STATS): sub-part pairs / mixed ones\n"
                  "        unsigned long long* line = jstats + 32 * (blockIdx.x % 64);\n"
                  "        wave_count(line + 6, live);\n"
@@ -1388,8 +1451,7 @@
             o << "    // the sub-part's samples are unshadowed from every node of the sub-tile (summed over its lanes)\n"
                  "    jit::add_run_counts(shead, counts, " << NL << ", live && !amb && result == 0, node, " << ST
               << "u, (uint32_t)lt, in ? SUBN[gp * " << SQ << "u + q] : 0, nnodes);\n"
-                 "    jit::mix_append(live && amb, (((tile * " << NP << " + gp) * " << SQ << "u + q) << " << NSTL << ") + st, "
-              << rsv << ", mixed, mcount, segcap, err);\n"
+                 "    jit::mix_append(live && amb, " << st_entry << ", " << rsv << ", mixed, mcount, segcap, err);\n"
                  "    if (jstats != nullptr) {  // diagnostics (FRT_JIT_STATS): sub-tile pairs / mixed ones\n"
                  "        unsigned long long* line = jstats + 32 * (blockIdx.x % 64);\n"
                  "        wave_count(line + 8, live);\n"
@@ -1398,8 +1460,8 @@
                  "}\n\n";
         } else if (mode == 1) {
             o << "    if (live && !amb && result == 0) {  // the part's samples are unshadowed from every node of the tile\n"
-                 "        for (uint32_t n = 0; n < " << TS << "u; ++n) {\n"
-                 "            const uint32_t nd = (tile << " << TSL << ") + n;\n"
+                 "        for (uint32_t n = 0; n < " << RN << "; ++n) {\n"
+                 "            const uint32_t nd = (tile << " << RL << ") + n;\n"
                  "            if (nd < nnodes && shead.hit(nd)) atomicAdd(counts + nd * " << NL << " + (uint32_t)lt, " << cnt << ");\n"
                  "        }\n"
                  "    }\n"
@@ -1412,14 +1474,13 @@
                  "}\n\n";
         } else if (mode == 3) {
             o << "    if (live && !amb && result == 0) {  // the sub-part's samples are unshadowed from every node of the tile\n"
-                 "        for (uint32_t n = 0; n < " << TS << "u; ++n) {\n"
-                 "            const uint32_t nd = (tile << " << TSL << ") + n;\n"
+                 "        for (uint32_t n = 0; n < " << RN << "; ++n) {\n"
+                 "            const uint32_t nd = (tile << " << RL << ") + n;\n"
                  "            if (nd < nnodes && shead.hit(nd)) atomicAdd(counts + nd * " << NL
               << " + (uint32_t)lt, SUBN[gp * " << SQ << "u + q]);\n"
                  "        }\n"
                  "    }\n"
-                 "    jit::mix_append(live && amb, (tile * " << NP << " + gp) * " << SQ << "u + q, " << rsv
-              << ", mixed, mcount, segcap, err);\n"
+                 "    jit::mix_append(live && amb, " << sub_entry << ", " << rsv << ", mixed, mcount, segcap, err);\n"
                  "    if (jstats != nullptr) {  // diagnostics (FRT_JIT_STATS): sub-part pairs / mixed ones\n"
                  "        unsigned long long* line = jstats + 32 * (blockIdx.x % 64);\n"
                  "        wave_count(line + 6, live);\n"
@@ -1434,8 +1495,7 @@
               << " + (uint32_t)lt, SUBN[gp * " << SQ << "u + q]);\n"
                  "        }\n"
                  "    }\n"
-                 "    jit::mix_append(live && amb, (((tile * " << NP << " + gp) * " << SQ << "u + q) << " << NSTL << ") + st, "
-              << rsv << ", mixed, mcount, segcap, err);\n"
+                 "    jit::mix_append(live && amb, " << st_entry << ", " << rsv << ", mixed, mcount, segcap, err);\n"
                  "    if (jstats != nullptr) {  // diagnostics (FRT_JIT_STATS): sub-tile pairs / mixed ones\n"
                  "        unsigned long long* line = jstats + 32 * (blockIdx.x % 64);\n"
                  "        wave_count(line + 8, live);\n"
@@ -1472,6 +1532,7 @@
     }
     if (SQ > 0) pair_kernel(3);
     if (ST > 0) pair_kernel(4);
+    if (SUP > 0) pair_kernel(5);
     g.u32 = u32_mode >= 2;
 
     o << "extern \"C\" __global__ void __launch_bounds__(kTraceBlock)" << waves_attr(K.jit_waves) << "\n"
@@ -1536,11 +1597,20 @@
          "                const uint32_t nn = j / " << std::max(PS2, 1) << "u;\n"
          "                j -= nn * " << std::max(PS2, 1) << "u;\n"
          "                const uint32_t e2 = subq == 3 ? pair >> " << NSTL << " : pair;\n"
-         "                const uint32_t tp = e2 >> " << SQL << ";\n"
-         "                q = e2 & " << std::max(SQ - 1, 0) << "u;\n"
-         "                const uint32_t tile = tp / " << NP << ";\n"
-         "                gp = tp - tile * " << NP << ";\n"
-         "                L.node = (tile << " << TSL << ") + (subq == 3 ? (pair & " << std::max(NST - 1, 0) << "u) << " << STL
+         "                uint32_t tile = 0;\n";
+    if (SUP)
+        o << "                const uint32_t e4 = e2 >> " << NTL << ";\n"
+             "                const uint32_t tp = e4 >> " << SQL << ";\n"
+             "                q = e4 & " << std::max(SQ - 1, 0) << "u;\n"
+             "                const uint32_t sup = tp / " << NP << ";\n"
+             "                gp = tp - sup * " << NP << ";\n"
+             "                tile = (sup << " << NTL << ") + (e2 & " << (NT - 1) << "u);\n";
+    else
+        o << "                const uint32_t tp = e2 >> " << SQL << ";\n"
+             "                q = e2 & " << std::max(SQ - 1, 0) << "u;\n"
+             "                tile = tp / " << NP << ";\n"
+             "                gp = tp - tile * " << NP << ";\n";
+    o << "                L.node = (tile << " << TSL << ") + (subq == 3 ? (pair & " << std::max(NST - 1, 0) << "u) << " << STL
       << " : 0u) + nn;\n"
          "            } else {\n"
          "                const uint32_t npair = subq ? pair >> " << SQL << " : pair;\n"
@@ -1868,7 +1938,8 @@
         }
         return -1;
     }
-    hipFunction_t f = nullptr, fb = nullptr, ft = nullptr, fl = nullptr, fs = nullptr, fst = nullptr, ftr = nullptr;
+    hipFunction_t f = nullptr, fb = nullptr, ft = nullptr, fl = nullptr, fs = nullptr, fst = nullptr, ftr = nullptr,
+                  fsp = nullptr;
     if (hipModuleGetFunction(&f, ce.mod, "frt_jit_shadow") != hipSuccess ||
         hipModuleGetFunction(&fb, ce.mod, "frt_jit_beam") != hipSuccess) {
         log = "hipModuleGetFunction failed";
@@ -1890,12 +1961,18 @@
         log = "hipModuleGetFunction failed (sub-tile kernel)";
         return -1;
     }
+    if (src.find("frt_jit_split(") != std::string::npos &&
+        hipModuleGetFunction(&fsp, ce.mod, "frt_jit_split") != hipSuccess) {
+        log = "hipModuleGetFunction failed (split kernel)";
+        return -1;
+    }
     if (src.find("frt_jit_trace(") != std::string::npos && hipModuleGetFunction(&ftr, ce.mod, "frt_jit_trace") != hipSuccess) {
         log = "hipModuleGetFunction failed (closest-hit kernel)";
         return -1;
     }
     ce.fns.sub = (void*)fs;
     ce.fns.subtile = (void*)fst;
+    ce.fns.split = (void*)fsp;
     ce.fns.trace = (void*)ftr;
     ce.fns.shadow = (void*)f;
     ce.fns.beam = (void*)fb;
diff --git a/fast_ray_tracer_amd/csrc/frt_knobs.hpp b/fast_ray_tracer_amd/csrc/frt_knobs.hpp
--- a/fast_ray_tracer_amd/csrc/frt_knobs.hpp
+++ b/fast_ray_tracer_amd/csrc/frt_knobs.hpp
@@ -58,6 +58,7 @@
     int jit_subtile = 16;
     bool jit_subtile_set = false;
     int jit_sub = 16;
+    int jit_supertile = 512;
     bool jit_inside = true;
     int jit_u32 = 1;
     int jit_order = 1;
@@ -100,6 +101,8 @@
     k.jit_subtile_set = present("FRT_JIT_SUBTILE");
     const int sub = int_or("FRT_JIT_SUB", 16);
     k.jit_sub = sub == 2 || sub == 4 || sub == 8 || sub == 16 || sub == 32 ? sub : 0;
+    const int sup = int_or("FRT_JIT_SUPERTILE", 512);
+    k.jit_supertile = sup == 128 || sup == 256 || sup == 512 || sup == 1024 ? sup : 0;
     k.jit_inside = unless_int0("FRT_JIT_INSIDE");
     k.jit_u32 = int_or("FRT_JIT_U32", 1);
     k.jit_order = int_or("FRT_JIT_ORDER", 1);
@@ -138,6 +141,7 @@
     int64_t jit_max_pairs = 0;
     int64_t jit_min_pairs = (int64_t)1 << 18;
     bool jit_subtile_deep = true;
+    bool jit_supertile_deep = false;
     bool jit_trace = true;
     bool jit_trace_stats = false;
     std::string jit_trace_dump;
@@ -167,6 +171,7 @@
     k.jit_max_pairs = mp >= 1 && mp < (1ll << 31) ? (int64_t)mp : 0;
     k.jit_min_pairs = (int64_t)ll_or("FRT_JIT_MIN_PAIRS", 1ll << 18);
     k.jit_subtile_deep = unless_int0("FRT_JIT_SUBTILE_DEEP");
+    k.jit_supertile_deep = int_or("FRT_JIT_SUPERTILE_DEEP", 0) != 0;
     k.jit_trace = unless_int0("FRT_JIT_TRACE");
     k.jit_trace_stats = present("FRT_JIT_TRACE_STATS");
     if (const char* d = raw("FRT_JIT_TRACE_DUMP")) k.jit_trace_dump = d;
diff --git a/fast_ray_tracer_amd/runtime.py b/fast_ray_tracer_amd/runtime.py
--- a/fast_ray_tracer_amd/runtime.py
+++ b/fast_ray_tracer_amd/runtime.py
@@ -41,7 +41,7 @@
     def as_dict(self) -> dict:
         names = ["trace", "shadow", "shade", "combine", "resolve", "trace_primary", "prepare", "gi"]
         subs = ["frt_jit_beam", "frt_jit_shadow", "k_gather_est", "k_gather_hit", "frt_jit_tile", "frt_jit_sub",
-                "frt_jit_subtile", "k_shade_lit", "k_lit_sort", "k_shade_lit32", "k_feature_resolve"]
+                "frt_jit_subtile", "k_shade_lit", "k_lit_sort", "k_shade_lit32", "k_feature_resolve", "frt_jit_split"]
         return {
             "primary_rays": int(self.primary_rays), "secondary_rays": int(self.secondary_rays),
             "shadow_rays": int(self.shadow_rays), "pruned_secondary": int(self.pruned_secondary),
@@ -62,6 +62,15 @@
             "shadow_subtile_mixed": int(self.shadow_subtile_mixed), "lit_nodes": int(self.lit_nodes),
             "prepare_uniform_waves": int(self.prepare_uniform_waves),
         }
+
+
+class ShadowStageStats(ctypes.Structure):
+    _fields_ = [(n, ctypes.c_uint64) for n in
+                ("supertile", "tile_pairs", "tile_mixed", "sub_pairs", "sub_mixed", "split_pairs", "split_mixed",
+                 "subtile_pairs", "subtile_mixed", "rays_walked", "split_launches")] + [("split_ms", ctypes.c_double)]
+
+    def as_dict(self) -> dict:
+        return {n: (float if t is ctypes.c_double else int)(getattr(self, n)) for n, t in self._fields_}
 
 
 class FeatureBuffers(ctypes.Structure):
@@ -178,6 +187,10 @@
         lib.frt_render_rows_device.restype = ctypes.c_int
         lib.frt_render_rows_device.argtypes = [vp, ctypes.POINTER(FrameParams), vp, ctypes.POINTER(FrameStats)]
         lib.frt_scene_release.argtypes = [vp]
+        lib.frt_shadow_stages.restype = ctypes.c_size_t
+        lib.frt_shadow_stages.argtypes = [vp, ctypes.POINTER(ShadowStageStats)]
+        if lib.frt_shadow_stages(None, None) != ctypes.sizeof(ShadowStageStats):
+            raise RuntimeError("frt: frt_shadow_stage_stats does not match runtime.py ShadowStageStats: rebuild")
         lib.frt_encode_ppm.restype = ctypes.c_size_t
         lib.frt_encode_ppm.argtypes = [vp, ctypes.c_size_t, ctypes.c_size_t, ctypes.c_int, vp, ctypes.c_size_t]
         lib.frt_encode16.restype = ctypes.c_int
@@ -388,6 +401,11 @@
             raise RuntimeError("frt render_views failed: " + err)
         return (out, st) if stats else out
 
+    def shadow_stages(self) -> dict:
+        st = ShadowStageStats()
+        self.lib.frt_shadow_stages(self.handle, ctypes.byref(st))
+        return st.as_dict()
+
     def close(self) -> None:
         if getattr(self, "handle", None):
             self.lib.frt_scene_release(self.handle)
diff --git a/include/frt_device.h b/include/frt_device.h
--- a/include/frt_device.h
+++ b/include/frt_device.h
@@ -192,6 +192,21 @@
     uint64_t prepare_uniform_waves;
 } frt_frame_stats;
 
+typedef struct frt_shadow_stage_stats {
+    uint64_t supertile;
+    uint64_t tile_pairs;
+    uint64_t tile_mixed;
+    uint64_t sub_pairs;
+    uint64_t sub_mixed;
+    uint64_t split_pairs;
+    uint64_t split_mixed;
+    uint64_t subtile_pairs;
+    uint64_t subtile_mixed;
+    uint64_t rays_walked;
+    uint64_t split_launches;
+    double split_ms;
+} frt_shadow_stage_stats;
+
 int frt_device_count(void);
 
 int frt_device_warmup(int device);
@@ -202,6 +217,8 @@
 size_t frt_frame_stats_size(void);
 
 size_t frt_frame_params_size(void);
+
+size_t frt_shadow_stages(const frt_scene_handle *scene, frt_shadow_stage_stats *out);
 
 const char *frt_last_error(void);
 
```

Result: faster. 596,200, median of 6 (+11.9%).
